# adjacentlink/srsLTE-emane

Hardware: AMD Instinct MI355X
Metric: DL subframes/s (20 MHz, turbo 6-iter) (higher is better)
Workload: dtype f32 (OFDM/chest/eq) + i16 (LLR/turbo)

## Files before the change

include/srslte_hip/phy_hip.h:

```cpp
#ifndef SRSLTE_HIP_PHY_HIP_H
#define SRSLTE_HIP_PHY_HIP_H

#include <stddef.h>
#include <stdint.h>

#ifdef __cplusplus
extern "C" {
#endif

int   srslte_hip_device_count(void);
int   srslte_hip_set_device(int device);
void* srslte_hip_malloc(size_t nbytes);
void  srslte_hip_free(void* d_ptr);
int   srslte_hip_memcpy_h2d(void* d_dst, const void* h_src, size_t nbytes);
int   srslte_hip_memcpy_d2h(void* h_dst, const void* d_src, size_t nbytes);
int   srslte_hip_memset(void* d_dst, int value, size_t nbytes);
int   srslte_hip_sync(void);
void* srslte_hip_stream_create(void);
void  srslte_hip_stream_destroy(void* stream);
int   srslte_hip_stream_sync(void* stream);
void* srslte_hip_event_create(void);
int   srslte_hip_event_record(void* event, void* stream);
float srslte_hip_event_elapsed_ms(void* start, void* stop);
void  srslte_hip_event_destroy(void* event);
// ... 27 lines not shown
  int      filter_type;
  float    filter_coef[2];
  uint16_t mbsfn_area_id;
  uint8_t  interpolate_subframe;
  uint8_t  rsrp_neighbour;
  uint8_t  cfo_estimate_enable;
  uint32_t cfo_estimate_sf_mask;
  uint8_t  sync_error_enable;
} srslte_hip_chest_dl_cfg_t;
typedef struct {
  float noise_estimate, noise_estimate_dbm, snr_db, rsrp, rsrp_dbm, rsrq, rsrq_db, rssi_dbm, cfo, sync_error;
} srslte_hip_chest_dl_res_t;
srslte_hip_chest_dl_t* srslte_hip_chest_dl_create(uint32_t cell_id, uint32_t nof_prb, uint32_t nof_ports, int cp_is_norm);
int srslte_hip_chest_dl_set_tdd(srslte_hip_chest_dl_t* q, int sf_config, int ss_config);
void                   srslte_hip_chest_dl_destroy(srslte_hip_chest_dl_t* q);
int                    srslte_hip_chest_dl_set_symbol_sz(srslte_hip_chest_dl_t* q, int symbol_sz);
const void*            srslte_hip_chest_dl_pilots(const srslte_hip_chest_dl_t* q);
int srslte_hip_chest_dl_estimate_batch(srslte_hip_chest_dl_t* q, const srslte_hip_chest_dl_cfg_t* cfg, uint32_t tti0, const void* d_grid,
                                       void* d_ce, void* d_res, int nof_sf, void* stream);
int srslte_hip_chest_dl_estimate_batch_multi(srslte_hip_chest_dl_t* q, const srslte_hip_chest_dl_cfg_t* cfg, uint32_t tti0, const void* d_grid,
                                             void* d_ce, void* d_res, int nof_sf, int nof_rx, void* stream);
const float* srslte_hip_chest_dl_last_raw(const srslte_hip_chest_dl_t* q);
int         srslte_hip_chest_dl_set_mbsfn_area_id(srslte_hip_chest_dl_t* q, uint16_t mbsfn_area_id);
const void* srslte_hip_chest_dl_mbsfn_pilots(const srslte_hip_chest_dl_t* q, uint16_t mbsfn_area_id);
int srslte_hip_chest_dl_estimate_mbsfn_batch(srslte_hip_chest_dl_t* q, const srslte_hip_chest_dl_cfg_t* cfg, uint32_t tti0, const void* d_grid,
                                             void* d_ce, float* d_noise, int nof_sf, int nof_rx, void* stream);

typedef struct srslte_hip_chest_ul srslte_hip_chest_ul_t;
typedef struct {
  uint32_t cyclic_shift, delta_ss;
  int      group_hopping_en, sequence_hopping_en;
} srslte_hip_dmrs_pusch_cfg_t;
typedef struct {
  float noise_estimate, noise_estimate_dbm, snr, snr_db, cfo;
} srslte_hip_chest_ul_res_t;
srslte_hip_chest_ul_t* srslte_hip_chest_ul_create(uint32_t cell_id, uint32_t nof_prb, int cp_is_norm, const srslte_hip_dmrs_pusch_cfg_t* cfg);
void                   srslte_hip_chest_ul_destroy(srslte_hip_chest_ul_t* q);
int srslte_hip_refsignal_dmrs_pusch_gen(const srslte_hip_chest_ul_t* q, uint32_t L_prb, uint32_t sf_idx, uint32_t n_dmrs, void* r_host);
int srslte_hip_chest_ul_estimate_pusch_batch(srslte_hip_chest_ul_t* q, uint32_t tti0, uint32_t L_prb, uint32_t n_prb, uint32_t n_dmrs,
                                             const void* d_grid, void* d_ce, void* d_res, int nof_sf, void* stream);
int srslte_hip_chest_ul_estimate_pusch_batch_hop(srslte_hip_chest_ul_t* q, uint32_t tti0, uint32_t L_prb, uint32_t n_prb, uint32_t n_prb_slot1,
                                                 uint32_t n_dmrs, const void* d_grid, void* d_ce, void* d_res, int nof_sf, void* stream);

int srslte_hip_demod_soft_demodulate_batch(int mod, const void* d_symbols, float* d_llr, int nsymbols, int ncalls, void* stream);
int srslte_hip_demod_soft_demodulate_s_batch(int mod, const void* d_symbols, short* d_llr, int nsymbols, int ncalls, void* stream);
int srslte_hip_demod_soft_demodulate_b_batch(int mod, const void* d_symbols, int8_t* d_llr, int nsymbols, int ncalls, void* stream);

typedef struct srslte_hip_tdec srslte_hip_tdec_t;
srslte_hip_tdec_t* srslte_hip_tdec_create(uint32_t max_long_cb, uint32_t max_nof_cb);
void               srslte_hip_tdec_destroy(srslte_hip_tdec_t* q);
uint32_t           srslte_hip_tdec_autoimp_get_subblocks(uint32_t long_cb);
uint32_t           srslte_hip_tdec_input_len(uint32_t long_cb, int sb_layout);
int srslte_hip_tdec_run_batch(srslte_hip_tdec_t* q, const int16_t* d_input, uint32_t in_stride, int sb_layout, uint32_t long_cb,
                              uint32_t nof_cb, uint32_t nof_iterations, uint32_t crc_poly, uint32_t crc_nbits, uint8_t* d_output,
                              uint32_t out_stride, uint32_t* d_iters, uint8_t* d_crc_ok, void* stream);

int srslte_hip_tdec_run_batch_manual(srslte_hip_tdec_t* q, const int16_t* d_input, uint32_t in_stride, int sb_layout, uint32_t long_cb,
                                     uint32_t nof_subblocks, uint32_t nof_cb, uint32_t nof_iterations, uint32_t crc_poly, uint32_t crc_nbits,
                                     uint8_t* d_output, uint32_t out_stride, uint32_t* d_iters, uint8_t* d_crc_ok, void* stream);

uint32_t srslte_hip_tdec_autoimp_get_subblocks_8bit(uint32_t long_cb);
int srslte_hip_tdec_run_batch_8bit(srslte_hip_tdec_t* q, const int8_t* d_input, uint32_t in_stride, int sb_layout, uint32_t long_cb,
                                   uint32_t nof_cb, uint32_t nof_iterations, uint32_t crc_poly, uint32_t crc_nbits, uint8_t* d_output,
                                   uint32_t out_stride, uint32_t* d_iters, uint8_t* d_crc_ok, void* stream);

int srslte_hip_tcod_encode_batch(const uint8_t* d_input, uint8_t* d_output, uint32_t long_cb, uint32_t nof_cb, void* stream);
int srslte_hip_tcod_encode_bytes_batch(const uint8_t* d_input, uint32_t in_stride, uint8_t* d_parity, uint32_t par_stride, uint8_t* d_sys_tail,
                                       uint32_t long_cb, uint32_t nof_cb, void* stream);

typedef struct {
  uint32_t F, C, K1, K2, K1_idx, K2_idx, C1, C2, tbs;
} srslte_hip_cbsegm_t;
int srslte_hip_cbsegm(srslte_hip_cbsegm_t* s, uint32_t tbs);
int srslte_hip_cbsegm_cbindex(uint32_t long_cb);
int srslte_hip_cbsegm_cbsize(uint32_t index);
int srslte_hip_tc_interl_LTE_gen_interl(uint16_t* forward, uint16_t* reverse, uint32_t long_cb, uint32_t interl_win);

typedef struct srslte_hip_dl_rx srslte_hip_dl_rx_t;
typedef struct {
  uint32_t cell_id, nof_prb, cfi;
  uint16_t rnti;
  int      mod;
  uint32_t tbs;
  uint32_t max_iterations;
  uint32_t max_batch;
  int      mmse;
  srslte_hip_chest_dl_cfg_t chest_cfg;
  int      llr_8bit;
  uint32_t nof_rx_antennas;
  uint32_t nof_ports;
  int      csi_enable;
  int      power_scale;
  float    p_a;
  int      tx_scheme;
  uint32_t pmi;
  int      mod2;
  uint32_t tbs2;
  int      cp_ext;
  int      tdd;
  uint32_t tdd_sf_config, tdd_ss_config;
  int      mbsfn;
  uint32_t mbsfn_area_id, non_mbsfn_region;
} srslte_hip_dl_rx_cfg_t;
srslte_hip_dl_rx_t* srslte_hip_dl_rx_create(const srslte_hip_dl_rx_cfg_t* cfg);
void                srslte_hip_dl_rx_destroy(srslte_hip_dl_rx_t* q);
int                 srslte_hip_dl_rx_set_iq_format(srslte_hip_dl_rx_t* q, int format, float scale);
uint32_t            srslte_hip_dl_rx_nof_re(const srslte_hip_dl_rx_t* q, uint32_t sf_idx);
int srslte_hip_dl_rx_batch(srslte_hip_dl_rx_t* q, const void* d_iq, uint32_t tti0, uint32_t nof_sf, uint8_t* d_tb, uint32_t tb_stride,
                           uint8_t* d_tb_ok, void* stream);
int srslte_hip_dl_rx_batch_harq(srslte_hip_dl_rx_t* q, const void* d_iq, uint32_t tti0, uint32_t nof_sf, uint32_t rv, int new_data,
                                uint8_t* d_tb, uint32_t tb_stride, uint8_t* d_tb_ok, void* stream);
int srslte_hip_dl_rx_batch_harq2(srslte_hip_dl_rx_t* q, const void* d_iq, uint32_t tti0, uint32_t nof_sf, const uint32_t rv[2], const int new_data[2],
                                 uint8_t* d_tb, uint32_t tb_stride, uint8_t* d_tb_ok, void* stream);
int srslte_hip_dl_rx_grid_batch(srslte_hip_dl_rx_t* q, const void* d_grid, uint32_t tti0, uint32_t nof_sf, uint8_t* d_tb, uint32_t tb_stride,
                                uint8_t* d_tb_ok, void* stream);
typedef struct {
  uint32_t prb_mask[2][4];
  int      mod;
  uint32_t tbs;
  uint32_t rv;
  uint32_t cfi;
  uint16_t rnti;
  int      new_data;
} srslte_hip_dl_grant_t;
int srslte_hip_dl_rx_batch_grants(srslte_hip_dl_rx_t* q, const void* d_iq, uint32_t tti0, uint32_t nof_sf, const srslte_hip_dl_grant_t* grants,
                                  uint8_t* d_tb, uint32_t tb_stride, uint8_t* d_tb_ok, void* stream);
typedef struct {
  srslte_hip_dl_grant_t tb0;
  int      tx_scheme;
  uint32_t pmi;
  int      mod2;
  uint32_t tbs2, rv2;
  int      new_data2;
} srslte_hip_dl_grant2_t;
int srslte_hip_dl_rx_batch_grants2(srslte_hip_dl_rx_t* q, const void* d_iq, uint32_t tti0, uint32_t nof_sf, const srslte_hip_dl_grant2_t* grants,
                                   uint8_t* d_tb, uint32_t tb_stride, uint8_t* d_tb_ok, void* stream);
int srslte_hip_dl_rx_grid_batch_grants2(srslte_hip_dl_rx_t* q, const void* d_grid, uint32_t tti0, uint32_t nof_sf, const srslte_hip_dl_grant2_t* grants,
                                        uint8_t* d_tb, uint32_t tb_stride, uint8_t* d_tb_ok, void* stream);
typedef struct srslte_hip_dl_rx_pool srslte_hip_dl_rx_pool_t;
srslte_hip_dl_rx_pool_t* srslte_hip_dl_rx_pool_create(const srslte_hip_dl_rx_cfg_t* cfg, uint32_t depth);
void                     srslte_hip_dl_rx_pool_destroy(srslte_hip_dl_rx_pool_t* p);
int64_t srslte_hip_dl_rx_pool_submit(srslte_hip_dl_rx_pool_t* p, const void* d_iq, uint32_t tti0, uint32_t nof_sf, const srslte_hip_dl_grant_t* grants,
                                     uint8_t* d_tb, uint32_t tb_stride, uint8_t* d_tb_ok, void* h_record );
int     srslte_hip_dl_rx_pool_wait(srslte_hip_dl_rx_pool_t* p, int64_t ticket);
int     srslte_hip_dl_rx_pool_set_iq_format(srslte_hip_dl_rx_pool_t* p, int format, float scale);
int64_t srslte_hip_dl_rx_pool_submit_host(srslte_hip_dl_rx_pool_t* p, const void* h_iq, uint32_t tti0, uint32_t nof_sf, const srslte_hip_dl_grant_t* grants,
                                          uint8_t* d_tb, uint32_t tb_stride, uint8_t* d_tb_ok, void* h_record );

int srslte_hip_dl_rx_stage(srslte_hip_dl_rx_t* q, int stage, const void* d_iq, uint32_t tti0, uint32_t nof_sf, uint8_t* d_tb,
                           uint32_t tb_stride, uint8_t* d_tb_ok, void* stream);
const void* srslte_hip_dl_rx_debug_buffer(const srslte_hip_dl_rx_t* q, int which);
int         srslte_hip_dl_rx_keep_symbols(srslte_hip_dl_rx_t* q, int enable);
int      srslte_hip_dl_rx_parity_compact(const srslte_hip_dl_rx_t* q);
uint32_t srslte_hip_rm_parity_compact_limit(uint32_t K);

typedef struct srslte_hip_ul_rx srslte_hip_ul_rx_t;
typedef struct {
  uint32_t cell_id, nof_prb;
  uint16_t rnti;
  int      mod;
  uint32_t tbs;
  uint32_t L_prb, n_prb, n_dmrs;
  uint32_t max_iterations, max_batch;
  int      mmse;
  srslte_hip_dmrs_pusch_cfg_t dmrs_cfg;
  int      shortened;
  uint32_t ack_len;
  uint32_t I_offset_ack;
  uint32_t ri_len;
  uint32_t I_offset_ri;
  uint32_t cqi_len, I_offset_cqi;
  uint32_t hopping, n_prb_slot1;
  uint32_t max_grants;
  int      cp_ext;
} srslte_hip_ul_rx_cfg_t;
srslte_hip_ul_rx_t* srslte_hip_ul_rx_create(const srslte_hip_ul_rx_cfg_t* cfg);
void                srslte_hip_ul_rx_destroy(srslte_hip_ul_rx_t* q);
int                 srslte_hip_ul_rx_set_iq_format(srslte_hip_ul_rx_t* q, int format, float scale);
int srslte_hip_ul_rx_batch(srslte_hip_ul_rx_t* q, const void* d_iq, uint32_t tti0, uint32_t nof_sf, uint8_t* d_tb, uint32_t tb_stride,
                           uint8_t* d_tb_ok, void* stream);
int srslte_hip_ul_rx_batch_harq(srslte_hip_ul_rx_t* q, const void* d_iq, uint32_t tti0, uint32_t nof_sf, uint32_t rv, int new_data, uint8_t* d_tb,
                                uint32_t tb_stride, uint8_t* d_tb_ok, void* stream);
typedef struct {
  uint32_t sf;
  uint16_t rnti;
  uint32_t L_prb, n_prb, n_prb_slot1, n_dmrs;
  int      mod;
  uint32_t tbs, rv;
  int      new_data;
  uint32_t ack_len, I_offset_ack;
  uint32_t ri_len, I_offset_ri;
  uint32_t cqi_len, I_offset_cqi;
} srslte_hip_ul_grant_t;
int srslte_hip_ul_rx_batch_grants(srslte_hip_ul_rx_t* q, const void* d_iq, uint32_t tti0, uint32_t nof_sf, const srslte_hip_ul_grant_t* grants,
                                  uint32_t nof_grants, uint8_t* d_tb, uint32_t tb_stride, uint8_t* d_tb_ok, void* stream);
const uint8_t* srslte_hip_ul_rx_grants_ack(const srslte_hip_ul_rx_t* q);
const uint8_t* srslte_hip_ul_rx_grants_ri(const srslte_hip_ul_rx_t* q);
const uint8_t* srslte_hip_ul_rx_grants_cqi(const srslte_hip_ul_rx_t* q);
const uint8_t* srslte_hip_ul_rx_ack(const srslte_hip_ul_rx_t* q);
const uint8_t* srslte_hip_ul_rx_ri(const srslte_hip_ul_rx_t* q);
const uint8_t* srslte_hip_ul_rx_cqi(const srslte_hip_ul_rx_t* q);
const void* srslte_hip_ul_rx_debug_buffer(const srslte_hip_ul_rx_t* q, int which);

typedef struct srslte_hip_ul_tx srslte_hip_ul_tx_t;
typedef struct {
  uint32_t cell_id, nof_prb;
  uint16_t rnti;
  int      mod;
  uint32_t tbs;
  uint32_t L_prb, n_prb, n_dmrs;
  uint32_t max_batch;
  srslte_hip_dmrs_pusch_cfg_t dmrs_cfg;
  int      shortened;
  uint32_t ack_len, I_offset_ack;
  uint32_t ri_len, I_offset_ri;
  uint32_t cqi_len, I_offset_cqi;
  uint32_t hopping, n_prb_slot1;
  uint32_t max_grants;
  int      cp_ext;
} srslte_hip_ul_tx_cfg_t;
srslte_hip_ul_tx_t* srslte_hip_ul_tx_create(const srslte_hip_ul_tx_cfg_t* cfg);
void                srslte_hip_ul_tx_destroy(srslte_hip_ul_tx_t* q);
int                 srslte_hip_ul_tx_set_iq_format(srslte_hip_ul_tx_t* q, int format, float scale);
int srslte_hip_ul_tx_batch(srslte_hip_ul_tx_t* q, const uint8_t* d_tb, uint32_t tb_stride, uint32_t tti0, uint32_t nof_sf, void* d_iq,
                           void* stream);
int srslte_hip_ul_tx_batch_ack(srslte_hip_ul_tx_t* q, const uint8_t* d_tb, uint32_t tb_stride, const uint8_t* d_ack, uint32_t tti0,
                               uint32_t nof_sf, void* d_iq, void* stream);
int srslte_hip_ul_tx_batch_uci(srslte_hip_ul_tx_t* q, const uint8_t* d_tb, uint32_t tb_stride, const uint8_t* d_ack, const uint8_t* d_ri,
                               uint32_t tti0, uint32_t nof_sf, void* d_iq, void* stream);
int srslte_hip_ul_tx_batch_uci_cqi(srslte_hip_ul_tx_t* q, const uint8_t* d_tb, uint32_t tb_stride, const uint8_t* d_ack, const uint8_t* d_ri,
                                   const uint8_t* d_cqi, uint32_t tti0, uint32_t nof_sf, void* d_iq, void* stream);
int srslte_hip_ul_tx_batch_rv(srslte_hip_ul_tx_t* q, const uint8_t* d_tb, uint32_t tb_stride, const uint8_t* d_ack, const uint8_t* d_ri,
                              const uint8_t* d_cqi, uint32_t rv, uint32_t tti0, uint32_t nof_sf, void* d_iq, void* stream);
int srslte_hip_ul_tx_batch_grants(srslte_hip_ul_tx_t* q, const uint8_t* d_tb, uint32_t tb_stride, const uint8_t* d_ack, const uint8_t* d_ri,
                                  const uint8_t* d_cqi, uint32_t tti0, uint32_t nof_sf, const srslte_hip_ul_grant_t* grants, uint32_t nof_grants,
                                  void* d_iq, void* stream);
const void* srslte_hip_ul_tx_debug_buffer(const srslte_hip_ul_tx_t* q, int which);

typedef struct srslte_hip_dl_tx srslte_hip_dl_tx_t;
typedef struct {
  uint32_t cell_id, nof_prb, cfi;
  uint16_t rnti;
  int      mod;
  uint32_t tbs;
  uint32_t max_batch;
  uint32_t nof_ports;
  float    p_a;
  uint32_t max_grants;
  int      cp_ext;
  int      tdd;
  uint32_t tdd_sf_config, tdd_ss_config;
  int      mbsfn;
  uint32_t mbsfn_area_id, non_mbsfn_region;
} srslte_hip_dl_tx_cfg_t;
srslte_hip_dl_tx_t* srslte_hip_dl_tx_create(const srslte_hip_dl_tx_cfg_t* cfg);
void                srslte_hip_dl_tx_destroy(srslte_hip_dl_tx_t* q);
int                 srslte_hip_dl_tx_set_iq_format(srslte_hip_dl_tx_t* q, int format, float scale);
int srslte_hip_dl_tx_batch(srslte_hip_dl_tx_t* q, const uint8_t* d_tb, uint32_t tb_stride, uint32_t tti0, uint32_t nof_sf, uint32_t rv, void* d_iq,
                           void* stream);
typedef struct {
  uint32_t              sf;
  srslte_hip_dl_grant_t grant;
} srslte_hip_dl_tx_grant_t;
int srslte_hip_dl_tx_batch_grants(srslte_hip_dl_tx_t* q, const uint8_t* d_tb, uint32_t tb_stride, uint32_t tti0, uint32_t nof_sf,
                                  const srslte_hip_dl_tx_grant_t* grants, uint32_t nof_grants, void* d_iq, void* stream);
typedef struct {
  uint32_t               sf;
  srslte_hip_dl_grant2_t grant;
} srslte_hip_dl_tx_grant2_t;
int srslte_hip_dl_tx_batch_grants2(srslte_hip_dl_tx_t* q, const uint8_t* d_tb, uint32_t tb_stride, uint32_t tti0, uint32_t nof_sf,
                                   const srslte_hip_dl_tx_grant2_t* grants, uint32_t nof_grants, void* d_iq, void* stream);
const void* srslte_hip_dl_tx_debug_buffer(const srslte_hip_dl_tx_t* q, int which);

typedef struct srslte_hip_sch srslte_hip_sch_t;
srslte_hip_sch_t* srslte_hip_sch_create(uint32_t max_tbs, uint32_t max_e_bits, int llr_8bit);
void              srslte_hip_sch_destroy(srslte_hip_sch_t* q);
int srslte_hip_sch_decode(srslte_hip_sch_t* q, const void* e_bits, uint32_t nof_e_bits, uint32_t tbs, int mod, uint32_t Nl, uint32_t rv,
                          uint32_t max_iterations, int16_t** buffer_f, uint8_t* cb_crc, uint8_t* cb_bytes, uint32_t* sum_passes);
typedef struct {
  int      mod;
  uint32_t tbs, rv, nof_bits, L_prb, nof_symb, max_iterations;
  uint32_t ack_len, ri_len, cqi_len;
  uint32_t I_offset_ack, I_offset_ri, I_offset_cqi;
  uint32_t cqi_len_rank2, cqi_rank2;
} srslte_hip_ulsch_cfg_t;
typedef struct {
  uint8_t  ack[2], ri;
  uint8_t  cqi_bits[64], cqi_crc;
  uint32_t cqi_len;
  uint32_t Q_prime_ack, Q_prime_ri, Q_prime_cqi;
  uint32_t stream_waits;
} srslte_hip_ulsch_res_t;
int srslte_hip_ulsch_decode(srslte_hip_sch_t* q, const int16_t* q_bits, const uint8_t* c_seq, const srslte_hip_ulsch_cfg_t* cfg, int16_t** buffer_f,
                            uint8_t* cb_crc, uint8_t* cb_bytes, uint32_t* sum_passes, srslte_hip_ulsch_res_t* res);
int srslte_hip_ulsch_debug_g(srslte_hip_sch_t* q, int16_t* out, uint32_t n);
typedef struct {
  srslte_hip_ulsch_cfg_t sch;
  uint32_t nof_prb, cell_id, cp_ext;
  uint32_t rnti, sf_idx;
  uint32_t n_prb_tilde[2];
  uint32_t shortened;
  uint32_t nof_re;
} srslte_hip_pusch_cfg_t;
int srslte_hip_pusch_decode(srslte_hip_sch_t* q, const void* sf_symbols, const void* ce, float noise_estimate, const srslte_hip_pusch_cfg_t* cfg,
                            int16_t** buffer_f, uint8_t* cb_crc, uint8_t* cb_bytes, uint32_t* sum_passes, srslte_hip_ulsch_res_t* res);
int srslte_hip_pusch_rows(const srslte_hip_pusch_cfg_t* cfg, uint32_t* rows);
// ... 615 lines not shown
```

srslte-emane_amd/csrc/pdsch_kernels.inc:

```
#include <vector>

namespace {

struct ChestResDev {
  float noise_estimate, noise_estimate_dbm, snr_db, rsrp, rsrp_dbm, rsrq, rsrq_db, rssi_dbm, cfo, sync_error;
};

struct SfClass {
  const uint32_t* idx;
  int             nof_re;
};

struct SfDesc {
  const uint32_t* idx;
  const uint32_t* scr;
  int             nof_re, mod, Qm;
  int             C, K, tbs, rlen;
  const uint32_t* crc_fac;
  int             scheme, codebook, nof_tb;
};
struct CbDesc {
  int             sf, cb;
  int             C, K, Qm, nof_re;
  int             combine;
  int             w_len;
  const uint32_t* tbl;
  int             Nl;
  int             e_off;
};
struct GrantDev {
  uint32_t mask[2][4];
  int      sf_idx, lstart, q_off, rnti;
  int      cw;
  int      tdd;
  int      nss[2];
};

struct PdschGeom {
  const SfDesc* desc;
  SfClass cls[3];
  int     grid_len;
  int      ce_len, ce_nre;
  uint32_t ce_magic;
  int     max_re, max_bits, mod, Qm, mmse, scr_words, tti0, nof_rx, nof_ports;
  float     inv_scaling;
  float*    csi;
  uint32_t* csi_max;
  int             tx_scheme, codebook_idx, nof_tb, mod1, Qm1, max_bits1, scr_words1;
  const uint32_t* scr1;
  float*          csi1;
  uint32_t*       csi_max1;
  int             cw1_off;
};

__device__ __forceinline__ void csi_note_max(uint32_t* dst, float v)
{
  for (int o = 32; o > 0; o >>= 1) v = fmaxf(v, __shfl_xor(v, o, 64));
  if ((threadIdx.x & 63) == 0) atomicMax(dst, __float_as_uint(v));
}

__device__ __forceinline__ int sf_class(int sf_idx) { return sf_idx == 0 ? 0 : (sf_idx == 5 ? 1 : 2); }

template <typename LLR>
__global__ __launch_bounds__(256) void pdsch_demod_kernel(const cf32* __restrict__ grid, const cf32* __restrict__ ce,
                                                          const ChestResDev* __restrict__ res, const uint32_t* __restrict__ scr,
                                                          cf32* __restrict__ d_out, LLR* __restrict__ e_out, PdschGeom g)
{
  __shared__ __attribute__((aligned(16))) LLR stage[256 * 8];
  const int       sf = blockIdx.y, sf_idx = (g.tti0 + sf) % 10;
  SfClass         c  = g.cls[sf_class(sf_idx)];
  int             mod = g.mod, Qm = g.Qm;
  const uint32_t* cs = scr + (size_t)sf_idx * g.scr_words;
  if (g.desc) {
    const SfDesc d = g.desc[sf];
    if (d.scheme >= 2) return;
    c.idx = d.idx; c.nof_re = d.nof_re; mod = d.mod; Qm = d.Qm; cs = d.scr;
  }
  const int     base = blockIdx.x * blockDim.x, i = base + threadIdx.x;
  if (base >= c.nof_re) return;
  const bool     live = i < c.nof_re;
  const uint32_t k  = c.idx[live ? i : c.nof_re - 1];
  const float    n0 = g.mmse ? res[sf].noise_estimate : 0.f;
  cf32           x;
  float          gain;
  const uint32_t kh = g.ce_nre ? k - __umulhi(k, g.ce_magic) * (uint32_t)g.ce_nre : k;
  if (g.nof_rx == 1) {
    const cf32 y = grid[(size_t)sf * g.grid_len + k], h = ce[(size_t)sf * g.ce_len + kh];
    const float re = y.x * h.x + y.y * h.y, im = y.y * h.x - y.x * h.y, csi = h.x * h.x + h.y * h.y + n0;
    x = make_float2(re * g.inv_scaling / csi, im * g.inv_scaling / csi);
    gain = csi;
  } else {
    float re = 0.f, im = 0.f, hh = 0.f;
    for (int a = 0; a < g.nof_rx; a++) {
      const size_t o = ((size_t)sf * g.nof_rx + a) * g.grid_len + k;
      const cf32   y = grid[o], h = ce[((size_t)sf * g.nof_rx + a) * g.ce_len + kh];
      const float  pr = y.x * h.x + y.y * h.y, pi = y.y * h.x - y.x * h.y, ph = h.x * h.x + h.y * h.y;
      re = a ? re + pr : pr;
      im = a ? im + pi : pi;
      hh = a ? hh + ph : ph;
    }
    if (n0 > 0.f) hh += n0;
    x = make_float2(re / hh * g.inv_scaling, im / hh * g.inv_scaling);
    gain = hh;
  }
  if (g.csi) {
    if (live) g.csi[(size_t)sf * g.max_re + i] = gain;
    csi_note_max(g.csi_max + sf, live ? gain : 0.f);
  }
  if (d_out && live) d_out[(size_t)sf * g.max_re + i] = x;
  LLR o[8];
  if constexpr (sizeof(LLR) == 1) {
    demod_dev::demod_b(mod, x, i, c.nof_re, o);
  } else {
    demod_dev::demod_s(mod, x, i, c.nof_re, o);
  }
  const int       bit0 = (live ? i : 0) * Qm;
  const uint32_t  c2   = (uint32_t)((((uint64_t)cs[(bit0 >> 5) + 1] << 32) | cs[bit0 >> 5]) >> (bit0 & 31));
  for (int j = 0; j < Qm; j++) {
    LLR v = o[j];
    if ((c2 >> j) & 1) v = (LLR)-v;
    stage[threadIdx.x * Qm + j] = v;
  }
  __syncthreads();
  const int   nbytes = min(256, c.nof_re - base) * Qm * (int)sizeof(LLR);
  char*       dst    = reinterpret_cast<char*>(e_out + (size_t)sf * g.max_bits + (size_t)base * Qm);
  const char* src    = reinterpret_cast<const char*>(stage);
  for (int o16 = threadIdx.x * 16; o16 + 16 <= nbytes; o16 += 256 * 16) *reinterpret_cast<uint4*>(dst + o16) = *reinterpret_cast<const uint4*>(src + o16);
  const int rem = nbytes & 15;
  if ((int)threadIdx.x < rem) dst[nbytes - rem + threadIdx.x] = src[nbytes - rem + threadIdx.x];
}

template <typename LLR>
__global__ __launch_bounds__(256) void pdsch_demod_div_kernel(const cf32* __restrict__ grid, const cf32* __restrict__ ce,
                                                              const uint32_t* __restrict__ scr, cf32* __restrict__ d_out, LLR* __restrict__ e_out,
                                                              PdschGeom g)
{
  __shared__ __attribute__((aligned(16))) LLR stage[512 * 8];
  const int       sf = blockIdx.y, sf_idx = (g.tti0 + sf) % 10;
  SfClass         c  = g.cls[sf_class(sf_idx)];
  const uint32_t* cs = scr + (size_t)sf_idx * g.scr_words;
  int             mod = g.mod, Qm = g.Qm;
  if (g.desc) {
    const SfDesc d = g.desc[sf];
    if (d.scheme >= 2) return;
    c.idx = d.idx; c.nof_re = d.nof_re; mod = d.mod; Qm = d.Qm; cs = d.scr;
  }
  const int     base = blockIdx.x * 512, i0 = base + 2 * threadIdx.x;
  if (base >= c.nof_re) return;
  const bool     live = i0 < c.nof_re;
  const uint32_t k0 = c.idx[live ? i0 : c.nof_re - 2], k1 = c.idx[live ? i0 + 1 : c.nof_re - 1];
  float          hh = 0.f, x0r = 0.f, x0i = 0.f, x1r = 0.f, x1i = 0.f;
  for (int a = 0; a < g.nof_rx; a++) {
    const cf32* y  = grid + ((size_t)sf * g.nof_rx + a) * g.grid_len;
    const cf32* h0 = ce + (((size_t)sf * 2 + 0) * g.nof_rx + a) * g.grid_len;
    const cf32* h1 = ce + (((size_t)sf * 2 + 1) * g.nof_rx + a) * g.grid_len;
    const cf32  r0 = y[k0], r1 = y[k1], h00 = h0[k0], h01 = h0[k1], h10 = h1[k0], h11 = h1[k1];
    hh += h00.x * h00.x + h00.y * h00.y + h11.x * h11.x + h11.y * h11.y;
    if (hh == 0.f) hh = 1e-4f;
    x0r += h00.x * r0.x + h00.y * r0.y + h11.x * r1.x + h11.y * r1.y;
    x0i += h00.x * r0.y - h00.y * r0.x + h11.y * r1.x - h11.x * r1.y;
    x1r += -(h10.x * r0.x + h10.y * r0.y) + h01.x * r1.x + h01.y * r1.y;
    x1i += -(h10.y * r0.x - h10.x * r0.y) + h01.x * r1.y - h01.y * r1.x;
  }
  if (g.csi) {
    if (live) *reinterpret_cast<float2*>(g.csi + (size_t)sf * g.max_re + i0) = make_float2(hh, hh);
    csi_note_max(g.csi_max + sf, live ? hh : 0.f);
  }
  hh *= 1.0f / g.inv_scaling;
  const cf32 x[2] = {make_float2((float)((double)(x0r / hh) * 1.4142135623730951), (float)((double)(x0i / hh) * 1.4142135623730951)),
                     make_float2((float)((double)(x1r / hh) * 1.4142135623730951), (float)((double)(x1i / hh) * 1.4142135623730951))};
#pragma unroll
  for (int t = 0; t < 2; t++) {
    const int i = (live ? i0 : 0) + t;
    if (d_out && live) d_out[(size_t)sf * g.max_re + i] = x[t];
    LLR o[8];
    if constexpr (sizeof(LLR) == 1) {
      demod_dev::demod_b(mod, x[t], i, c.nof_re, o);
    } else {
      demod_dev::demod_s(mod, x[t], i, c.nof_re, o);
    }
    const int      bit0 = i * Qm;
    const uint32_t c2   = (uint32_t)((((uint64_t)cs[(bit0 >> 5) + 1] << 32) | cs[bit0 >> 5]) >> (bit0 & 31));
    for (int j = 0; j < Qm; j++) stage[(2 * threadIdx.x + t) * Qm + j] = ((c2 >> j) & 1) ? (LLR)-o[j] : o[j];
  }
  __syncthreads();
  const int   nbytes = min(512, c.nof_re - base) * Qm * (int)sizeof(LLR);
  char*       dst    = reinterpret_cast<char*>(e_out + (size_t)sf * g.max_bits + (size_t)base * Qm);
  const char* src    = reinterpret_cast<const char*>(stage);
  for (int o16 = threadIdx.x * 16; o16 + 16 <= nbytes; o16 += 256 * 16) *reinterpret_cast<uint4*>(dst + o16) = *reinterpret_cast<const uint4*>(src + o16);
  const int rem = nbytes & 15;
  if ((int)threadIdx.x < rem) dst[nbytes - rem + threadIdx.x] = src[nbytes - rem + threadIdx.x];
}

template <typename LLR>
__global__ __launch_bounds__(256) void pdsch_demod_div4_kernel(const cf32* __restrict__ grid, const cf32* __restrict__ ce,
                                                               const uint32_t* __restrict__ scr, cf32* __restrict__ d_out, LLR* __restrict__ e_out,
                                                               PdschGeom g)
{
  __shared__ __attribute__((aligned(16))) LLR stage[1024 * 8];
  const int       sf = blockIdx.y, sf_idx = (g.tti0 + sf) % 10;
  SfClass         c  = g.cls[sf_class(sf_idx)];
  const uint32_t* cs = scr + (size_t)sf_idx * g.scr_words;
  int             mod = g.mod, Qm = g.Qm;
  if (g.desc) {
    const SfDesc d = g.desc[sf];
    if (d.scheme >= 2) return;
    c.idx = d.idx; c.nof_re = d.nof_re; mod = d.mod; Qm = d.Qm; cs = d.scr;
  }
  const int     base = blockIdx.x * 1024, i0 = base + 4 * threadIdx.x;
  if (base >= c.nof_re) return;
  const bool live = i0 < c.nof_re;
  uint32_t   k[4];
#pragma unroll
  for (int t = 0; t < 4; t++) k[t] = c.idx[live ? i0 + t : c.nof_re - 4 + t];
  float a[4] = {0.f, 0.f, 0.f, 0.f}, xr[4] = {0.f, 0.f, 0.f, 0.f}, xi[4] = {0.f, 0.f, 0.f, 0.f};
  for (int an = 0; an < g.nof_rx; an++) {
    const cf32* y = grid + ((size_t)sf * g.nof_rx + an) * g.grid_len;
#pragma unroll
    for (int half = 0; half < 2; half++) {
      const cf32* hA = ce + (((size_t)sf * 4 + half) * g.nof_rx + an) * g.grid_len;
      const cf32* hB = ce + (((size_t)sf * 4 + 2 + half) * g.nof_rx + an) * g.grid_len;
      const uint32_t k0 = k[2 * half], k1 = k[2 * half + 1];
      const cf32     h00 = hA[k0], h01 = hB[k0], h10 = hA[k1], h11 = hB[k1], r0 = y[k0], r1 = y[k1];
      a[2 * half] += h00.x * h00.x + h00.y * h00.y + h11.x * h11.x + h11.y * h11.y;
      a[2 * half + 1] += h10.x * h10.x + h10.y * h10.y + h01.x * h01.x + h01.y * h01.y;
      xr[2 * half] += h00.x * r0.x + h00.y * r0.y + h11.x * r1.x + h11.y * r1.y;
      xi[2 * half] += h00.x * r0.y - h00.y * r0.x + h11.y * r1.x - h11.x * r1.y;
      xr[2 * half + 1] += -(h01.x * r0.x + h01.y * r0.y) + h10.x * r1.x + h10.y * r1.y;
      xi[2 * half + 1] += -(h01.y * r0.x - h01.x * r0.y) + h10.x * r1.y - h10.y * r1.x;
    }
  }
  float           gmax = 0.f;
#pragma unroll
  for (int t = 0; t < 4; t++) {
    const int   i  = (live ? i0 : 0) + t;
    const float at = a[t] * (1.0f / g.inv_scaling);
    const cf32  x  = make_float2(xr[t] / at * 1.41421356f, xi[t] / at * 1.41421356f);
    if (g.csi && live) g.csi[(size_t)sf * g.max_re + i] = at / g.nof_rx;
    gmax = fmaxf(gmax, live ? at / g.nof_rx : 0.f);
    if (d_out && live) d_out[(size_t)sf * g.max_re + i] = x;
    LLR o[8];
    if constexpr (sizeof(LLR) == 1) {
      demod_dev::demod_b(mod, x, i, c.nof_re, o);
    } else {
      demod_dev::demod_s(mod, x, i, c.nof_re, o);
    }
    const int      bit0 = i * Qm;
    const uint32_t c2   = (uint32_t)((((uint64_t)cs[(bit0 >> 5) + 1] << 32) | cs[bit0 >> 5]) >> (bit0 & 31));
    for (int j = 0; j < Qm; j++) stage[(4 * threadIdx.x + t) * Qm + j] = ((c2 >> j) & 1) ? (LLR)-o[j] : o[j];
  }
  if (g.csi) csi_note_max(g.csi_max + sf, gmax);
  __syncthreads();
  const int   nbytes = min(1024, c.nof_re - base) * Qm * (int)sizeof(LLR);
  char*       dst    = reinterpret_cast<char*>(e_out + (size_t)sf * g.max_bits + (size_t)base * Qm);
  const char* src    = reinterpret_cast<const char*>(stage);
  for (int o16 = threadIdx.x * 16; o16 + 16 <= nbytes; o16 += 256 * 16) *reinterpret_cast<uint4*>(dst + o16) = *reinterpret_cast<const uint4*>(src + o16);
  const int rem = nbytes & 15;
  if ((int)threadIdx.x < rem) dst[nbytes - rem + threadIdx.x] = src[nbytes - rem + threadIdx.x];
}

__device__ __forceinline__ cf32 cmulc(cf32 a, cf32 b) { return make_float2(a.x * b.x + a.y * b.y, a.y * b.x - a.x * b.y); }

template <typename LLR>
__global__ __launch_bounds__(256) void pdsch_demod_mimo_kernel(const cf32* __restrict__ grid, const cf32* __restrict__ ce,
                                                               const ChestResDev* __restrict__ res, const uint32_t* __restrict__ scr,
                                                               cf32* __restrict__ d_out0, cf32* __restrict__ d_out1, LLR* __restrict__ e_out0,
                                                               LLR* __restrict__ e_out1, PdschGeom g)
{
  __shared__ __attribute__((aligned(16))) LLR stage[2][256 * 8];
  const int       sf = blockIdx.y, sf_idx = (g.tti0 + sf) % 10;
  SfClass         c  = g.cls[sf_class(sf_idx)];
  int             tx_scheme = g.tx_scheme, codebook_idx = g.codebook_idx, nof_tb = g.nof_tb, mods[2] = {g.mod, g.mod1}, Qms[2] = {g.Qm, g.Qm1};
  const uint32_t* css[2] = {scr + (size_t)sf_idx * g.scr_words, g.scr1 ? g.scr1 + (size_t)sf_idx * g.scr_words1 : nullptr};
  if (g.desc) {
    const SfDesc d0 = g.desc[sf];
    if (d0.scheme < 2) return;
    const SfDesc d1 = g.desc[g.cw1_off + sf];
    c.idx = d0.idx; c.nof_re = d0.nof_re; tx_scheme = d0.scheme; codebook_idx = d0.codebook; nof_tb = d0.nof_tb;
    mods[0] = d0.mod; Qms[0] = d0.Qm; css[0] = d0.scr;
    mods[1] = d1.mod; Qms[1] = d1.Qm; css[1] = d1.scr;
  }
  const int     base = blockIdx.x * blockDim.x, i = base + threadIdx.x;
  if (base >= c.nof_re) return;
  const bool     live = i < c.nof_re;
// ... 53 lines not shown
    x[1]   = cadd(cmul(y0, w10), cmul(y1, w11));
    csi[0] = 1.0f / b00.x;
    csi[1] = 1.0f / b11.x;
  }
#pragma unroll
  for (int cw = 0; cw < 2; cw++) {
    if (cw >= nof_tb) break;
    const int       mod = mods[cw], Qm = Qms[cw];
    float*          csi_o = cw ? g.csi1 : g.csi;
    cf32*           d_out = cw ? d_out1 : d_out0;
    if (csi_o) {
      if (live) csi_o[(size_t)sf * g.max_re + i] = csi[cw];
      csi_note_max((cw ? g.csi_max1 : g.csi_max) + sf, live ? csi[cw] : 0.f);
    }
    if (d_out && live) d_out[(size_t)sf * g.max_re + i] = x[cw];
    LLR o[8];
    if constexpr (sizeof(LLR) == 1) {
      demod_dev::demod_b(mod, x[cw], i, c.nof_re, o);
    } else {
      demod_dev::demod_s(mod, x[cw], i, c.nof_re, o);
    }
    const uint32_t* cs   = css[cw];
    const int       bit0 = (live ? i : 0) * Qm;
    const uint32_t  c2   = (uint32_t)((((uint64_t)cs[(bit0 >> 5) + 1] << 32) | cs[bit0 >> 5]) >> (bit0 & 31));
    for (int j = 0; j < Qm; j++) stage[cw][threadIdx.x * Qm + j] = ((c2 >> j) & 1) ? (LLR)-o[j] : o[j];
  }
  __syncthreads();
#pragma unroll
  for (int cw = 0; cw < 2; cw++) {
    if (cw >= nof_tb) break;
    const int   Qm = Qms[cw], nbytes = min(256, c.nof_re - base) * Qm * (int)sizeof(LLR);
    char*       dst = reinterpret_cast<char*>((cw ? e_out1 : e_out0) + (size_t)sf * (cw ? g.max_bits1 : g.max_bits) + (size_t)base * Qm);
    const char* src = reinterpret_cast<const char*>(stage[cw]);
    for (int o16 = threadIdx.x * 16; o16 + 16 <= nbytes; o16 += 256 * 16) *reinterpret_cast<uint4*>(dst + o16) = *reinterpret_cast<const uint4*>(src + o16);
    const int rem = nbytes & 15;
    if ((int)threadIdx.x < rem) dst[nbytes - rem + threadIdx.x] = src[nbytes - rem + threadIdx.x];
  }
}

struct RmGeom {
  const CbDesc* cbd;
  uint8_t*      cb_ok_rst;
  int C, K, Qm, tti0, max_bits, w_stride, out_len;
  int nof_re[3];
  int             max_re, mod;
  int             Nl;
  const float*    csi;
  const uint32_t* csi_max;
  int             combine;
  const uint8_t*  skip;
  int             e_off;
  int             w_len;
};

template <typename LLR>
__device__ __forceinline__ uint32_t add_wrap(uint32_t a, uint32_t b)
{
  if constexpr (sizeof(LLR) == 2) {
    return (((a & 0xffffu) + (b & 0xffffu)) & 0xffffu) | (((a >> 16) + (b >> 16)) << 16);
  } else {
    const uint32_t lo = ((a & 0x00ff00ffu) + (b & 0x00ff00ffu)) & 0x00ff00ffu, hi = ((a & 0xff00ff00u) >> 8) + ((b & 0xff00ff00u) >> 8);
    return lo | ((hi & 0x00ff00ffu) << 8);
  }
}

struct CsiW {
  const float* csi;
  float        scale, inv;
  int          Qm, mod, body_bits, nsym;
};
__device__ __forceinline__ CsiW csi_setup(const RmGeom& g, int sf, int nsym, int Qm)
{
  CsiW c;
  c.csi = g.csi + (size_t)sf * g.max_re;
  const float mx = nsym > 0 ? __uint_as_float(g.csi_max[sf]) : 1.0f;
  c.scale = 32767.0f / mx;
  c.inv   = 1.0f / mx;
  c.Qm = Qm; c.mod = Qm / 2; c.nsym = nsym;
  const int G = c.mod == 3 ? 12 : (c.mod == 4 ? 8 : 4);
  c.body_bits = (nsym * Qm / G) * G;
  return c;
}
template <typename LLR>
__device__ __forceinline__ LLR csi_apply(const CsiW& c, LLR v, int b)
{
  if constexpr (sizeof(LLR) == 1) {
    const int s = min(b / c.Qm, c.nsym - 1);
    return (LLR)demod_dev::trunc_i((float)v * (c.csi[s] * c.inv));
  } else {
    if (b >= c.body_bits) {
      const int s = min(b / c.Qm, c.nsym - 1);
      return (LLR)demod_dev::trunc_i((float)v * (c.csi[s] * c.inv));
    }
    int s;
    if (c.mod == 1) {
      s = 2 * (b >> 2) + (((b & 3) < 2) ? 1 : 0);
    } else if (c.mod == 3) {
      const int r = b % 12;
      s = 2 * (b / 12) + ((r < 4 || r == 6 || r == 7) ? 0 : 1);
    } else {
      s = b / c.Qm;
    }
    const int w = demod_dev::sat16(demod_dev::rne(c.csi[s] * c.scale));
    return (LLR)(((int)v * w) >> 16);
  }
}


template <typename LLR>
__global__ __launch_bounds__(256) void rm_rx_kernel(const LLR* __restrict__ e, LLR* __restrict__ w, const uint32_t* __restrict__ inv, RmGeom g)
{
  constexpr int PER = 4 / (int)sizeof(LLR);
  int             cbg = blockIdx.y, sf = cbg / g.C, cb = cbg - sf * g.C, C = g.C, Qm = g.Qm, out_len = g.out_len, w_len = g.w_len ? g.w_len : g.w_stride, combine = g.combine;
  int             nre = g.nof_re[sf_class((g.tti0 + sf) % 10)], Nl = g.Nl, e_off = g.e_off;
  const uint32_t* tbl = inv;
  if (g.cbd) {
    const CbDesc d = g.cbd[blockIdx.y];
    sf = d.sf; cb = d.cb; cbg = sf * g.C + cb; C = d.C; Qm = d.Qm; out_len = 3 * d.K + 12; w_len = d.w_len; combine = d.combine; nre = d.nof_re; tbl = d.tbl;
    Nl = d.Nl; e_off = d.e_off;
  }
  const int j = PER * (blockIdx.x * blockDim.x + threadIdx.x);
  if (j >= w_len || (g.skip && combine && g.skip[cbg])) return;
  if (g.cb_ok_rst && !combine && j == 0) g.cb_ok_rst[cbg] = 0;
  const int QmL = Qm * Nl, Gp = nre / Nl;
  const int gamma = Gp % C, n_e = QmL * (Gp / C);
  int       rp = cb * n_e, n_e2 = n_e;
  if (cb > C - gamma) {
    n_e2 = n_e + QmL;
    rp   = (C - gamma) * n_e + (cb - (C - gamma)) * n_e2;
  }
  const LLR* src = e + (size_t)sf * g.max_bits + e_off + rp;
  CsiW       cw;
  if (g.csi) cw = csi_setup(g, sf, nre, Qm);
  uint32_t   n[PER], word = 0;
  if constexpr (PER == 2) {
    const uint2 t = *reinterpret_cast<const uint2*>(tbl + j);
    n[0] = t.x; n[1] = t.y;
  } else {
    const uint4 t = *reinterpret_cast<const uint4*>(tbl + j);
    n[0] = t.x; n[1] = t.y; n[2] = t.z; n[3] = t.w;
  }
#pragma unroll
  for (int s = 0; s < PER; s++) {
    int acc = 0;
    if (n[s] != 0xffffffffu) {
      for (int i = (int)n[s]; i < n_e2; i += out_len) acc += g.csi ? csi_apply<LLR>(cw, src[i], rp + i) : src[i];
    }
    word |= ((uint32_t)acc & ((1u << (8 * sizeof(LLR))) - 1u)) << (8 * sizeof(LLR) * s);
  }
  uint32_t* dst = reinterpret_cast<uint32_t*>(w + (size_t)cbg * g.w_stride + j);
  *dst          = combine ? add_wrap<LLR>(*dst, word) : word;
}

template <typename LLR>
__global__ __launch_bounds__(256) void rm_rx_lds_kernel(const LLR* __restrict__ e, LLR* __restrict__ w, const uint32_t* __restrict__ inv, RmGeom g)
{
  extern __shared__ __attribute__((aligned(16))) char seg_raw[];
  constexpr int PER = 16 / (int)sizeof(LLR), NV = PER / 8;
  LLR*          seg = reinterpret_cast<LLR*>(seg_raw);
  int             cbg = blockIdx.x, sf = cbg / g.C, cb = cbg - sf * g.C, C = g.C, Qm = g.Qm, out_len = g.out_len, w_len = g.w_len ? g.w_len : g.w_stride, combine = g.combine;
  int             nre = g.nof_re[sf_class((g.tti0 + sf) % 10)], Nl = g.Nl, e_off = g.e_off;
  const uint32_t* tbl = inv;
  if (g.cbd) {
    const CbDesc d = g.cbd[blockIdx.x];
    sf = d.sf; cb = d.cb; cbg = sf * g.C + cb; C = d.C; Qm = d.Qm; out_len = 3 * d.K + 12; w_len = d.w_len; combine = d.combine; nre = d.nof_re; tbl = d.tbl;
    Nl = d.Nl; e_off = d.e_off;
  }
  if (g.skip && combine && g.skip[cbg]) return;
  if (g.cb_ok_rst && !combine && threadIdx.x == 0) g.cb_ok_rst[cbg] = 0;
  const int QmL = Qm * Nl, Gp = nre / Nl;
  const int gamma = Gp % C, n_e = QmL * (Gp / C);
  int       rp = cb * n_e, n_e2 = n_e;
  if (cb > C - gamma) {
    n_e2 = n_e + QmL;
    rp   = (C - gamma) * n_e + (cb - (C - gamma)) * n_e2;
  }
  const LLR* src = e + (size_t)sf * g.max_bits + e_off + rp;
  const int mis = (int)((reinterpret_cast<uintptr_t>(src) & 15) / sizeof(LLR));
  const int4* s4 = reinterpret_cast<const int4*>(src - mis);
  const int   n16 = (n_e2 + mis + PER - 1) / PER;
  if (g.csi) {
    const CsiW cw = csi_setup(g, sf, nre, Qm);
    for (int i = threadIdx.x; i < n16; i += 256) {
      union {
        int4 v;
        LLR  h[PER];
      } u;
      u.v = s4[i];
#pragma unroll
      for (int j = 0; j < PER; j++) u.h[j] = csi_apply<LLR>(cw, u.h[j], rp - mis + PER * i + j);
      reinterpret_cast<int4*>(seg)[i] = u.v;
    }
  } else {
#pragma unroll 4
    for (int i = threadIdx.x; i < n16; i += 256) reinterpret_cast<int4*>(seg)[i] = s4[i];
  }
  __syncthreads();
  const LLR*   ls    = seg + mis;
  const uint4* inv16 = reinterpret_cast<const uint4*>(reinterpret_cast<const uint16_t*>(tbl + w_len));
  uint4*       dst   = reinterpret_cast<uint4*>(w + (size_t)cbg * g.w_stride);
  const int    ngroups = w_len / PER;
  for (int j0 = threadIdx.x; j0 < ngroups; j0 += 4 * 256) {
    uint4 tt[4][NV];
#pragma unroll
    for (int u = 0; u < 4; u++) {
      const int j = j0 + 256 * u;
#pragma unroll
      for (int v = 0; v < NV; v++) tt[u][v] = j < ngroups ? inv16[j * NV + v] : make_uint4(~0u, ~0u, ~0u, ~0u);
    }
#pragma unroll
    for (int u = 0; u < 4; u++) {
      const int j = j0 + 256 * u;
      if (j >= ngroups) break;
      uint32_t o[4] = {0, 0, 0, 0};
#pragma unroll
      for (int s = 0; s < PER; s++) {
        const uint32_t pair = (&tt[u][s / 8].x)[(s / 2) & 3], n = (s & 1) ? pair >> 16 : pair & 0xffffu;
        int            acc  = 0;
        if (n != 0xffffu) {
          for (int i = (int)n; i < n_e2; i += out_len) acc += ls[i];
        }
        constexpr int BITS = 8 * (int)sizeof(LLR);
        o[s * BITS / 32] |= ((uint32_t)acc & ((1u << BITS) - 1u)) << ((s * BITS) & 31);
      }
      if (combine) {
        const uint4 old = dst[j];
        dst[j] = make_uint4(add_wrap<LLR>(old.x, o[0]), add_wrap<LLR>(old.y, o[1]), add_wrap<LLR>(old.z, o[2]), add_wrap<LLR>(old.w, o[3]));
      } else {
        dst[j] = make_uint4(o[0], o[1], o[2], o[3]);
      }
    }
  }
}

__device__ __forceinline__ uint32_t gf24_mul(uint32_t a, uint32_t b, uint32_t poly)
{
  uint32_t r = 0;
  for (int i = 23; i >= 0; i--) {
    r <<= 1;
    if (r & 0x1000000u) r ^= poly;
    if ((b >> i) & 1) r ^= a;
  }
  return r;
}

template <typename Byte>
__device__ uint32_t block_crc24(Byte byte_at, int nbytes, uint32_t poly, uint32_t* tab, uint32_t* red)
{
  const int t = threadIdx.x;
  {
    uint32_t v = (uint32_t)t << 16;
    for (int i = 0; i < 8; i++) {
      v <<= 1;
      if (v & 0x1000000u) v ^= poly;
    }
    tab[t] = v;
  }
  __syncthreads();
  const int cB = (nbytes + 255) / 256, pad = 256 * cB - nbytes;
  uint32_t  crc = 0;
  for (int i = 0; i < cB; i++) {
    const int v = t * cB + i - pad;
    if (v >= 0) crc = ((crc << 8) & 0xffffffu) ^ tab[((crc >> 16) & 0xff) ^ byte_at(v)];
  }
  uint32_t m = 1;
  for (int i = 0; i < 8 * cB; i++) {
    m <<= 1;
    if (m & 0x1000000u) m ^= poly;
  }
  red[t] = crc;
  __syncthreads();
  for (int s = 1; s < 256; s <<= 1) {
    uint32_t v = 0;
    if ((t & (2 * s - 1)) == 0) v = gf24_mul(red[t], m, poly) ^ red[t + s];
    __syncthreads();
    if ((t & (2 * s - 1)) == 0) red[t] = v;
    m = gf24_mul(m, m, poly);
    __syncthreads();
  }
  return red[0];
}

struct TbGeom {
  const SfDesc* desc;
  int C, K, tbs, rlen, cb_stride, tb_stride;
  int nof_sf, cw1_off;
  const uint32_t* iters;
};
__device__ __forceinline__ bool tb_any_block_decoded(const uint32_t* iters, int first, int C)
{
  if (!iters) return true;
  bool any = false;
  for (int c = 0; c < C; c++) any = any || iters[first + c] != 0;
  return any;
}

__global__ __launch_bounds__(512) void tb_crc_kernel(const uint8_t* __restrict__ cb_bytes, const uint8_t* __restrict__ cb_ok,
                                                     const uint32_t* __restrict__ crc_rem, uint8_t* __restrict__ tb, uint8_t* __restrict__ tb_ok,
                                                     TbGeom g)
{
  __shared__ uint32_t red[8];
  const int C = g.C, K = g.K, tbs = g.tbs, rlen = g.rlen;
  const int sf = blockIdx.x, nbytes = tbs / 8 + 3, rb = rlen / 8;
  uint8_t*  dst = tb + (size_t)sf * g.tb_stride;
  uint32_t  syn = 0;
  for (int b0 = threadIdx.x * 4; b0 < nbytes + 3; b0 += blockDim.x * 4) {
    uint32_t word = 0;
#pragma unroll
    for (int t = 0; t < 4; t++) {
      const int b = b0 + t;
      int       cb = b / rb;
      if (cb > C - 1) cb = C - 1;
      const int     off = b - cb * rb;
      const uint8_t v   = (b < nbytes + 3 && off < K / 8) ? cb_bytes[((size_t)sf * g.C + cb) * g.cb_stride + off] : 0;
      if (b < nbytes + 3) dst[b] = v;
      word |= (uint32_t)(b < nbytes ? v : 0) << (8 * t);
    }
#pragma unroll
    for (int j = 0; j < 32; j++) {
      const int      t = j >> 3, bit = 8 * (b0 + t) + 7 - (j & 7);
      const uint32_t m = 0u - ((word >> j) & 1u);
      syn ^= (bit < 8 * nbytes ? crc_rem[bit] : 0u) & m;
    }
  }
  for (int o = 32; o > 0; o >>= 1) syn ^= __shfl_xor(syn, o, 64);
  if ((threadIdx.x & 63) == 0) red[threadIdx.x >> 6] = syn;
  __syncthreads();
  if (threadIdx.x == 0) {
    syn = 0;
    for (int i = 0; i < (int)blockDim.x / 64; i++) syn ^= red[i];
    bool ok = syn == 0;
    for (int c = 0; c < C; c++) ok = ok && cb_ok[sf * g.C + c];
    const uint8_t* p = dst + tbs / 8;
    ok               = ok && (p[0] | p[1] | p[2]) && tb_any_block_decoded(g.iters, sf * g.C, C);
    tb_ok[sf]        = ok ? 1 : 0;
  }
}

constexpr int TB_MAX_BITS = 105528;
__global__ __launch_bounds__(256) void tb_crc_bytes_kernel(const uint8_t* __restrict__ cb_bytes, const uint8_t* __restrict__ cb_ok, uint8_t* __restrict__ tb,
                                                           uint8_t* __restrict__ tb_ok, TbGeom g)
{
  __shared__ uint32_t tab[256], red[4];
  __shared__ uint8_t  bytes[TB_MAX_BITS / 8 + 8];
  const int    row = blockIdx.x, sf = row < g.nof_sf ? row : g.cw1_off + row - g.nof_sf;
  const SfDesc d   = g.desc[sf];
  const int    C = d.C, K = d.K, nbytes = d.tbs / 8 + 3, rb = d.rlen / 8, t = threadIdx.x;
  uint8_t*     dst = tb + (size_t)row * g.tb_stride;
  if (C == 0) {
    if (t == 0) tb_ok[row] = 0;
    return;
  }
  {
    uint32_t v = (uint32_t)t << 16;
    for (int i = 0; i < 8; i++) {
      v <<= 1;
      if (v & 0x1000000u) v ^= 0x1864CFBu;
    }
    tab[t] = v;
  }
  for (int cb = 0; cb < C; cb++) {
    const uint8_t* src = cb_bytes + ((size_t)sf * g.C + cb) * g.cb_stride;
    const int      n   = cb == C - 1 ? nbytes + 3 - cb * rb : rb;
    for (int i = t; i < n; i += 256) {
      const uint8_t v = i < K / 8 ? src[i] : 0;
      dst[cb * rb + i] = v;
      if (cb * rb + i < nbytes) bytes[cb * rb + i] = v;
    }
  }
  __syncthreads();
  const int cB = (nbytes + 255) / 256, pad = 256 * cB - nbytes;
  uint32_t  crc = 0;
// ... 46 lines not shown
  pdsch_relist_body(gr, idx_out, P, cell_id, max_re, nof_ports, nsl, (int)blockIdx.x);
}
__device__ __forceinline__ void pdsch_relist_body(const GrantDev* __restrict__ gr, uint32_t* __restrict__ idx_out, int P, int cell_id, int max_re,
                                                  int nof_ports, int nsl, int sf)
{
  __shared__ int cnt[14 * 21 + 1];
  const int      nre = 12 * P, cps = (nre + 63) / 64, nsym = 2 * nsl, nchunks = nsym * cps;
  const int      wave = threadIdx.x >> 6, lane = threadIdx.x & 63, nwaves = RELIST_THREADS / 64;
  const GrantDev g  = gr[sf];
  auto           used = [&](int sym, int kc) {
    const int k = kc * 64 + lane, s = sym >= nsl ? 1 : 0, l = sym - nsl * s, p = k / 12;
    if (k >= nre || !((g.mask[s][p >> 5] >> (p & 31)) & 1u)) return false;
    if (g.nss[0] && l >= g.nss[s]) return false;
    return pdsch_re_used(P, cell_id, g.sf_idx, g.q_off, s, l, k, nof_ports, nsl, g.tdd, g.nss[1]);
  };
  __shared__ unsigned long long msk[14 * 21];
  for (int sym = 0; sym < nsym; sym++) {
    const bool on = sym >= nsl || sym >= g.lstart;
    for (int kc = wave; kc < cps; kc += nwaves) {
      const unsigned long long b = on ? __ballot(used(sym, kc)) : 0ull;
      if (lane == 0) {
        cnt[sym * cps + kc] = __popcll(b);
        msk[sym * cps + kc] = b;
      }
    }
  }
  __syncthreads();
  if (wave == 0) {
    constexpr int PL = (14 * 21 + 63) / 64;
    int           v[PL], sum = 0;
#pragma unroll
    for (int j = 0; j < PL; j++) {
      const int c = lane * PL + j;
      v[j]        = c < nchunks ? cnt[c] : 0;
      sum += v[j];
    }
    int incl = sum;
    for (int o = 1; o < 64; o <<= 1) {
      const int t = __shfl_up(incl, o, 64);
      if (lane >= o) incl += t;
    }
    int acc = incl - sum;
#pragma unroll
    for (int j = 0; j < PL; j++) {
      const int c = lane * PL + j;
      if (c < nchunks) cnt[c] = acc;
      acc += v[j];
    }
  }
  __syncthreads();
  uint32_t* o = idx_out + (size_t)sf * max_re;
  for (int sym = (g.lstart < nsl ? g.lstart : nsl); sym < nsym; sym++) {
    for (int kc = wave; kc < cps; kc += nwaves) {
      const unsigned long long b = msk[sym * cps + kc];
      if ((b >> lane) & 1ull) o[cnt[sym * cps + kc] + __popcll(b & ((1ull << lane) - 1ull))] = (uint32_t)(sym * nre + kc * 64 + lane);
    }
  }
}
__device__ __forceinline__ void scr_gen_body(const GrantDev* __restrict__ gr, const uint32_t* __restrict__ basis, uint32_t* __restrict__ out, int words,
                                             int cell_id, int sf, int w)
{
  if (w >= words) return;
  const GrantDev g = gr[sf];
  uint32_t       c_init = ((uint32_t)g.rnti << 14) + ((uint32_t)g.cw << 13) + ((uint32_t)g.sf_idx << 9) + (uint32_t)cell_id, v = basis[w];
  for (int j = 0; j < 31; j++) {
    if ((c_init >> j) & 1u) v ^= basis[(size_t)(1 + j) * words + w];
  }
  out[(size_t)sf * words + w] = v;
}
__global__ __launch_bounds__(256) void scr_gen_kernel(const GrantDev* __restrict__ gr, const uint32_t* __restrict__ basis, uint32_t* __restrict__ out,
                                                      int words, int cell_id)
{
  scr_gen_body(gr, basis, out, words, cell_id, (int)blockIdx.y, (int)(blockIdx.x * 256 + threadIdx.x));
}
__global__ __launch_bounds__(256) void desc_copy_kernel(const uint4* __restrict__ src, uint4* __restrict__ dst, int n16)
{
  const int i = (int)(blockIdx.x * 256 + threadIdx.x);
  if (i < n16) dst[i] = src[i];
}

__global__ __launch_bounds__(RELIST_THREADS) void grants_prep_kernel(const GrantDev* __restrict__ gr, uint32_t* __restrict__ idx_out, int P, int cell_id,
                                                                     int max_re, int nof_ports, int nsl, int nof_sf, const uint32_t* __restrict__ basis,
                                                                     uint32_t* __restrict__ scr0, const GrantDev* __restrict__ gr1,
                                                                     uint32_t* __restrict__ scr1, int words, uint8_t* __restrict__ tb_ok, int nrows,
                                                                     const uint4* __restrict__ desc_src, uint4* __restrict__ desc_dst, int desc_n16,
                                                                     int copy_first)
{
  if ((int)blockIdx.x >= copy_first) {
    const int i = ((int)blockIdx.x - copy_first) * RELIST_THREADS + (int)threadIdx.x;
    if (i < desc_n16) desc_dst[i] = desc_src[i];
    return;
  }
  if ((int)blockIdx.x < nof_sf) {
    if (threadIdx.x == 0) {
      tb_ok[blockIdx.x] = 0;
      if ((int)blockIdx.x + nof_sf < nrows) tb_ok[blockIdx.x + nof_sf] = 0;
    }
    pdsch_relist_body(gr, idx_out, P, cell_id, max_re, nof_ports, nsl, (int)blockIdx.x);
    return;
  }
  const int per = (words + RELIST_THREADS - 1) / RELIST_THREADS;
  int       b = (int)blockIdx.x - nof_sf;
  const int cw = b / (nof_sf * per);
  b -= cw * nof_sf * per;
  const int sf = b / per, w = (b - sf * per) * RELIST_THREADS + (int)threadIdx.x;
  scr_gen_body(cw ? gr1 : gr, basis, cw ? scr1 : scr0, words, cell_id, sf, w);
}

__global__ __launch_bounds__(256) void tb_asm_kernel(const uint8_t* __restrict__ cb_bytes, const uint8_t* __restrict__ cb_ok,
                                                     const uint32_t* __restrict__ cb_syn, uint8_t* __restrict__ tb, uint8_t* __restrict__ tb_ok,
                                                     TbGeom g)
{
  __shared__ __attribute__((aligned(8))) uint8_t cbb[32 * 768];
  const int      sf = blockIdx.x, nbytes = g.tbs / 8 + 3, rb = g.rlen / 8, tot = g.C * g.cb_stride;
  const uint8_t* src0 = cb_bytes + (size_t)sf * tot;
  uint8_t*       dst = tb + (size_t)sf * g.tb_stride;
  if ((reinterpret_cast<uintptr_t>(src0) & 7) == 0) {
    for (int i = threadIdx.x; i < tot / 8; i += blockDim.x) reinterpret_cast<uint64_t*>(cbb)[i] = reinterpret_cast<const uint64_t*>(src0)[i];
    for (int i = tot / 8 * 8 + threadIdx.x; i < tot; i += blockDim.x) cbb[i] = src0[i];
  } else {
    for (int i = threadIdx.x; i < tot; i += blockDim.x) cbb[i] = src0[i];
  }
  __syncthreads();
  auto src = [&](int b) -> uint32_t {
    int cb = b / rb;
    if (cb > g.C - 1) cb = g.C - 1;
    const int off = b - cb * rb;
    return off < g.K / 8 ? cbb[cb * g.cb_stride + off] : 0u;
  };
  const bool a4 = ((reinterpret_cast<uintptr_t>(dst) | (uintptr_t)g.tb_stride) & 3) == 0;
  const int  n  = nbytes + 3, n4 = a4 ? n / 4 : 0;
  for (int w = threadIdx.x; w < n4; w += blockDim.x)
    reinterpret_cast<uint32_t*>(dst)[w] = src(4 * w) | (src(4 * w + 1) << 8) | (src(4 * w + 2) << 16) | (src(4 * w + 3) << 24);
  for (int b = 4 * n4 + threadIdx.x; b < n; b += blockDim.x) dst[b] = (uint8_t)src(b);
  if (threadIdx.x == 0) {
    uint32_t syn = 0;
    bool     ok  = true;
    for (int c = 0; c < g.C; c++) {
      syn ^= cb_syn[sf * g.C + c];
      ok = ok && cb_ok[sf * g.C + c];
    }
    ok        = ok && syn == 0 && (src(g.tbs / 8) | src(g.tbs / 8 + 1) | src(g.tbs / 8 + 2)) && tb_any_block_decoded(g.iters, sf * g.C, g.C);
    tb_ok[sf] = ok ? 1 : 0;
  }
}

int rm_lds_bytes(const RmGeom& g, int llr_bytes)
{
  int mx = g.nof_re[0] > g.nof_re[1] ? g.nof_re[0] : g.nof_re[1];
  mx     = mx > g.nof_re[2] ? mx : g.nof_re[2];
  return ((g.Qm * (mx / g.C) + 2 * g.Qm) * llr_bytes + 32 + 15) & ~15;
}

template <typename T>
int rm_rx_launch(int lds, uint32_t nblk, const void* e, void* w, const uint32_t* tbl, const RmGeom& g, hipStream_t st)
{
  if (lds <= 64 * 1024) {
    hipLaunchKernelGGL(rm_rx_lds_kernel<T>, dim3(nblk), dim3(256), lds, st, (const T*)e, (T*)w, tbl, g);
  } else {
    hipLaunchKernelGGL(rm_rx_kernel<T>, dim3(ceil_div(g.w_stride, 1024 / (int)sizeof(T)), nblk), dim3(256), 0, st, (const T*)e, (T*)w, tbl, g);
  }
  LAUNCH_CHECK();
  return SRSLTE_SUCCESS;
}

std::vector<uint32_t> rm_slot_table(const std::vector<uint32_t>& t, uint32_t w_stride)
{
  std::vector<uint32_t> inv(w_stride + w_stride / 2, 0xffffffffu);
  uint16_t*             inv16 = reinterpret_cast<uint16_t*>(inv.data() + w_stride);
  for (uint32_t n = 0; n < t.size(); n++) {
    if (t[n] == 0xffffffffu) continue;
    inv[t[n]]   = n;
    inv16[t[n]] = (uint16_t)n;
  }
  return inv;
}

void pmch_re_indices(uint32_t nof_prb, uint32_t lstart, std::vector<uint32_t>& idx)
{
  idx.clear();
  for (uint32_t s = 0; s < 2; s++) {
    for (uint32_t l = (s == 0 ? lstart : 0); l < 6; l++) {
      const bool     has_ref = (l == 2 && s == 0) || (l == 0 && s == 1) || (l == 4 && s == 1);
      const uint32_t keep    = (l == 0 && s == 1) ? 0 : 1;
      for (uint32_t k = 0; k < 12 * nof_prb; k++) {
        if (!has_ref || (k & 1) == keep) idx.push_back((6 * s + l) * 12 * nof_prb + k);
      }
    }
  }
}

void pdsch_re_indices(uint32_t cell_id, uint32_t nof_prb, uint32_t nof_ports, uint32_t sf_idx, uint32_t lstart, std::vector<uint32_t>& idx,
                      uint32_t nsl = 7)
{
  const uint32_t nre = 12 * nof_prb, step = nof_ports == 1 ? 6 : 3;
  idx.clear();
  for (uint32_t s = 0; s < 2; s++) {
    for (uint32_t l = (s == 0 ? lstart : 0); l < nsl; l++) {
      const bool     has_ref = l == 0 || l == nsl - 3 || (l == 1 && nof_ports == 4);
      const uint32_t offset  = l == 0 ? cell_id % 6 : (cell_id + 3) % 6;
      const bool     sync    = (s == 0 && (sf_idx == 0 || sf_idx == 5) && l >= nsl - 2) || (s == 1 && sf_idx == 0 && l < 4);
      for (uint32_t k = 0; k < nre; k++) {
        if (sync && k + 36 >= nre / 2 && k < nre / 2 + 36) continue;
        if (has_ref && (k % step) == offset % step) continue;
        idx.push_back((s * nsl + l) * nre + k);
      }
    }
  }
}

template <typename T>
int upload(DevBuf<T>& d, const std::vector<T>& h)
{
  if (h.empty() ? d.alloc(1) : d.upload(h)) {
    hip_log("[srslte_hip] upload of a %zu-byte table to the device failed\n", sizeof(T) * h.size());
    return SRSLTE_ERROR;
  }
  return SRSLTE_SUCCESS;
}

int rm_rx_table_upload(uint32_t K, uint32_t rv, uint32_t W, uint32_t w_stride, DevBuf<uint32_t>& d_tbl)
{
  std::vector<uint32_t> t;
  lte_rm_rx_table(K, rv, t);
  if (W) {
    for (auto& v : t) v = v < 3 * K ? (v % 3) * (K + 32) + ((v / 3) % (K / W)) * W + (v / 3) / (K / W) : (v - 3 * K) + 3 * (K + 32);
  }
  return upload(d_tbl, rm_slot_table(t, w_stride));
}

struct RmParityCompact {
  uint32_t phase[2], len, e_lim;
};
bool rm_parity_compact(uint32_t K, RmParityCompact& c, std::vector<uint32_t>* t_out = nullptr)
{
  if (K % 64 || K / 16 < 4) return false;
  std::vector<uint32_t> t;
  lte_rm_rx_table(K, 0, t);
  const uint32_t Lw = K / 16;
  bool           seen[2] = {false, false};
  c.phase[0] = c.phase[1] = 0;
  c.len   = (K + 32 + K / 2 + 12 + 31) & ~31u;
  c.e_lim = (uint32_t)t.size();
  for (uint32_t n = 0; n < t.size(); n++) {
    const uint32_t v = t[n], s = v % 3, i = v / 3;
    if (v >= 3 * K) {
      t[n] = (v - 3 * K) + K + 32 + K / 2;
    } else if (s == 0) {
      t[n] = (i % Lw) * 16 + i / Lw;
    } else {
      const uint32_t r = i % Lw;
      if (!seen[s - 1]) {
        seen[s - 1]    = true;
        c.phase[s - 1] = r % 4;
      }
      if (r % 4 == c.phase[s - 1]) {
        t[n] = K + 32 + (s - 1) * (K / 4) + (r / 4) * 16 + i / Lw;
      } else {
        if (c.e_lim == t.size()) c.e_lim = n;
        t[n] = 0xffffffffu;
      }
    }
  }
  if (t_out) t_out->swap(t);
  return true;
}
int rm_rx_table_upload_compact(uint32_t K, RmParityCompact& c, DevBuf<uint32_t>& d_tbl)
{
  std::vector<uint32_t> t;
  if (!rm_parity_compact(K, c, &t)) return SRSLTE_ERROR_INVALID_INPUTS;
  return upload(d_tbl, rm_slot_table(t, c.len));
}

__global__ __launch_bounds__(256) void rm_parity_expand_kernel(int16_t* __restrict__ w, int w_stride, int K, int phase0, int phase1)
{
  __shared__ __attribute__((aligned(16))) int16_t cp[6144 / 2 + 16];
  int16_t*  p  = w + (size_t)blockIdx.x * w_stride;
  const int nc = K / 2 + 12, base = K + 32;
  for (int i = threadIdx.x; i < (nc + 7) / 8; i += 256) reinterpret_cast<uint4*>(cp)[i] = reinterpret_cast<const uint4*>(p + base)[i];
  __syncthreads();
  const int per = (K + 32) / 8;
  for (int j = threadIdx.x; j < 2 * per; j += 256) {
    const int s = j >= per, h = j - s * per, r = h >> 1;
    uint4     v = make_uint4(0, 0, 0, 0);
    if (r < K / 16 && (r & 3) == (s ? phase1 : phase0)) v = *reinterpret_cast<const uint4*>(cp + s * (K / 4) + (r >> 2) * 16 + (h & 1) * 8);
    *reinterpret_cast<uint4*>(p + (1 + s) * (K + 32) + h * 8) = v;
  }
  for (int i = 3 * (K + 32) + threadIdx.x; i < w_stride; i += 256) p[i] = i < 3 * (K + 32) + 12 ? cp[K / 2 + i - 3 * (K + 32)] : (int16_t)0;
}

int rm_tx_table_upload(uint32_t K, uint32_t rv, DevBuf<uint32_t>& d_tbl)
{
  std::vector<uint32_t> t;
  lte_rm_rx_table(K, rv, t);
  for (auto& v : t) {
    const uint32_t p = v / 3, s = v % 3;
    v = s == 0 ? (p < K ? p : (1u << 30) | (p - K)) : (2u << 30) | (s == 1 ? p : K + 4 + p);
  }
  return upload(d_tbl, t);
}

void constellation_levels(int mod, float* lvl)
{
  for (uint32_t idx = 0; idx < (1u << mod); idx++) {
    double v = 1.0;
    for (int i = mod - 1; i >= 1; i--) v = (double)(1 << (mod - i)) - (1 - 2 * (int)((idx >> (mod - 1 - i)) & 1)) * v;
    const double norm = mod == 1 ? sqrt(2.0) : (mod == 2 ? sqrt(10.0) : (mod == 3 ? sqrt(42.0) : sqrt(170.0)));
    lvl[idx]          = (float)((1 - 2 * (int)((idx >> (mod - 1)) & 1)) * v / norm);
  }
}
// ... 27 lines not shown
```

srslte-emane_amd/csrc/pdsch_rx.inc:

```
struct GrantsState {
  srslte_hip_tdec_t* tdec = nullptr;
  uint32_t           Cmax = 0, stride = 0, max_re = 0, max_bits = 0, words = 0;
  uint32_t           V = 0;
  DevBuf<uint32_t>   d_relist, d_scr, d_basis, d_cb_iters;
  DevBuf<int16_t>    d_e, d_w;
  DevBuf<uint8_t>    d_cb_bytes, d_cb_ok;
  DevBuf<float>      d_csi;
  DevBuf<uint32_t>   d_csi_max;
  size_t             desc_bytes = 0;
  DescStage          desc;
  bool               tb_direct = false;
  std::map<std::pair<uint32_t, uint32_t>, DevBuf<uint32_t>> rm_tbl;
  std::map<uint32_t, DevBuf<uint32_t>>                      crc_fac;
  ~GrantsState() { srslte_hip_tdec_destroy(tdec); }
};

struct srslte_hip_dl_rx {
  srslte_hip_dl_rx_cfg_t cfg   = {};
  srslte_hip_ofdm_t*     ofdm  = nullptr;
  srslte_hip_chest_dl_t* chest = nullptr;
  PdschGeom              pg    = {};
  DevBuf<uint32_t>       d_idx[3];
  struct Codeword {
    DevBuf<uint32_t> d_scr;
    DevBuf<int16_t>  d_e;
    DevBuf<cf32>     d_d;
    DevBuf<float>    d_csi;
    DevBuf<uint32_t> d_csi_max;
    SchRxFixed       sch;
  } cw[2];
  int                    ncw = 1;
  DevBuf<cf32>           d_grid, d_ce;
  DevBuf<cf32>           d_ce_full;
  DevBuf<ChestResDev>    d_res;
  std::unique_ptr<GrantsState> gs;
  srslte_hip_csi_t*      csi = nullptr;
  uint32_t               est_nof_sf = 0;
  float                  csi_offset = 0.f;
  ~srslte_hip_dl_rx()
  {
    srslte_hip_ofdm_destroy(ofdm);
    srslte_hip_chest_dl_destroy(chest);
    srslte_hip_csi_destroy(csi);
  }
};

struct DlRxCall {
  const cf32* grid = nullptr;
  SchHarq     harq[2];
};

extern "C" void srslte_hip_dl_rx_destroy(srslte_hip_dl_rx_t* q) { delete q; }

extern "C" int srslte_hip_dl_rx_set_iq_format(srslte_hip_dl_rx_t* q, int format, float scale)
{
  return q ? srslte_hip_ofdm_set_sample_format(q->ofdm, format, scale) : SRSLTE_ERROR_INVALID_INPUTS;
}

extern "C" srslte_hip_dl_rx_t* srslte_hip_dl_rx_create(const srslte_hip_dl_rx_cfg_t* cfg)
{
  if (!cfg || cfg->max_batch == 0 || cfg->mod < 1 || cfg->mod > 4 || cfg->max_iterations == 0 || cfg->nof_rx_antennas > 4 || cfg->nof_ports > 4 ||
      cfg->nof_ports == 3) {
    hip_log("[srslte_hip] dl_rx: invalid configuration\n");
    return nullptr;
  }
  const bool mimo = cfg->tx_scheme != 0, two = mimo && cfg->tbs2 != 0;
  if (mimo) {
    const bool ok = (cfg->tx_scheme == 2 || cfg->tx_scheme == 3) && cfg->nof_ports == 2 && cfg->nof_rx_antennas == 2 &&
                    (cfg->tx_scheme == 2 || two) && (two ? cfg->pmi < 2 : cfg->pmi < 4) && (!two || (cfg->mod2 >= 1 && cfg->mod2 <= 4));
    if (!ok) {
      hip_log("[srslte_hip] dl_rx: two-layer modes need a 2-port cell and 2 receive antennas; CDD with two transport blocks, "
              "multiplexing with two (pmi 0-1) or one (pmi 0-3)\n");
      return nullptr;
    }
  }
  std::unique_ptr<srslte_hip_dl_rx> q(new srslte_hip_dl_rx());
  q->cfg = *cfg;
  q->ncw = two ? 2 : 1;
  srslte_hip_cbsegm_t seg;
  if (fixed_grant_segmentation("dl_rx", cfg->tbs, &seg) || (two && fixed_grant_segmentation("dl_rx", cfg->tbs2, &seg))) return nullptr;
  const uint32_t P = cfg->nof_prb, nre = 12 * P, B = cfg->max_batch;
  const uint32_t lstart = cfg->cfi + (P < 10 ? 1 : 0);
  const uint32_t nrx    = cfg->nof_rx_antennas ? cfg->nof_rx_antennas : 1;
  const uint32_t npt    = cfg->nof_ports ? cfg->nof_ports : 1;
  const uint32_t nsl    = (cfg->cp_ext || cfg->mbsfn) ? 6 : 7;
  if (cfg->mbsfn && (npt != 1 || mimo || cfg->tdd || cfg->llr_8bit || cfg->csi_enable || cfg->power_scale || cfg->mbsfn_area_id > 255 ||
                     cfg->non_mbsfn_region < 1 || cfg->non_mbsfn_region > 2)) {
    hip_log("[srslte_hip] dl_rx: an MBSFN pipeline is single-port FDD with 16-bit LLRs, area id 0-255, a non-MBSFN region of 1 or 2 symbols\n");
    return nullptr;
  }
  if (cfg->mbsfn) q->cfg.chest_cfg.interpolate_subframe = 1;
  if (cfg->tdd && (cfg->tdd_sf_config > 6 || cfg->tdd_ss_config > 9)) {
    hip_log("[srslte_hip] dl_rx: TDD uplink-downlink configuration %u / special-subframe configuration %u\n", cfg->tdd_sf_config, cfg->tdd_ss_config);
    return nullptr;
  }
  q->ofdm  = srslte_hip_ofdm_create((int)P, nsl == 6 ? 0 : 1, 1);
  q->chest = srslte_hip_chest_dl_create(cfg->cell_id, P, npt, cfg->cp_ext ? 0 : 1);
  if (q->chest && cfg->tdd) srslte_hip_chest_dl_set_tdd(q->chest, (int)cfg->tdd_sf_config, (int)cfg->tdd_ss_config);
  if (cfg->mbsfn && q->ofdm && q->chest &&
      (srslte_hip_ofdm_set_mbsfn(q->ofdm, 1, (int)cfg->non_mbsfn_region) || srslte_hip_chest_dl_set_mbsfn_area_id(q->chest, (uint16_t)cfg->mbsfn_area_id))) {
    srslte_hip_chest_dl_destroy(q->chest);
    q->chest = nullptr;
  }
  bool ok = q->ofdm && q->chest;
  SchRxFixed::Cfg sc = {};
  const uint32_t  rep_sf[3] = {0, 5, 1};
  for (int c = 0; c < 3 && ok; c++) {
    std::vector<uint32_t> idx;
    if (cfg->mbsfn) pmch_re_indices(P, lstart, idx);
    else pdsch_re_indices(cfg->cell_id, P, npt, rep_sf[c], lstart, idx, nsl);
    q->pg.cls[c].nof_re = (int)idx.size();
    sc.nof_re[c]        = (uint32_t)idx.size();
    sc.max_re           = idx.size() > sc.max_re ? (uint32_t)idx.size() : sc.max_re;
    ok                  = upload(q->d_idx[c], idx) == SRSLTE_SUCCESS;
    q->pg.cls[c].idx    = q->d_idx[c];
  }
  const uint32_t max_re = sc.max_re;
  const size_t   glen   = (size_t)2 * nsl * nre;
  ok = ok && !q->d_grid.alloc(glen * B * nrx) && !q->d_ce.alloc(glen * B * nrx * npt) &&
       hipMemset(q->d_ce, 0, sizeof(cf32) * glen * B * nrx * npt) == hipSuccess &&
       !q->d_res.alloc(B);
  sc.max_batch = B; sc.max_iterations = cfg->max_iterations; sc.llr_8bit = cfg->llr_8bit != 0;
  sc.Nl = (npt > 1 && !mimo) ? 2 : 1;
  uint32_t scr_words[2] = {0, 0};
  for (int c = 0; c < q->ncw && ok; c++) {
    srslte_hip_dl_rx::Codeword& w = q->cw[c];
    sc.mod = c ? cfg->mod2 : cfg->mod; sc.tbs = c ? cfg->tbs2 : cfg->tbs; sc.Qm = 2 * (uint32_t)sc.mod;
    sc.max_bits  = (max_re * sc.Qm + 15) & ~15u;
    scr_words[c] = (max_re * sc.Qm + 31) / 32 + 1;
    std::vector<uint32_t> scr;
    const uint32_t        c_init0 = cfg->mbsfn ? cfg->mbsfn_area_id : ((uint32_t)cfg->rnti << 14) + ((uint32_t)c << 13) + cfg->cell_id;
    lte_scr_table([&](uint32_t sf) { return c_init0 + (sf << 9); }, max_re * sc.Qm, scr_words[c], scr);
    ok = upload(w.d_scr, scr) == SRSLTE_SUCCESS && !w.d_e.alloc((size_t)sc.max_bits * B + 16);
    if (ok && cfg->csi_enable) ok = !w.d_csi.alloc((size_t)max_re * B) && !w.d_csi_max.alloc(B);
    sc.csi = w.d_csi; sc.csi_max = w.d_csi_max;
    sc.may_compact = c == 0; sc.may_direct = !two && !mimo;
    ok = ok && w.sch.init(sc) == SRSLTE_SUCCESS;
  }
  if (!ok) {
    hip_log("[srslte_hip] dl_rx: initialisation failed\n");
    return nullptr;
  }
  const SchRxFixed& s0 = q->cw[0].sch;
  q->pg.grid_len = (int)glen; q->pg.max_re = (int)max_re; q->pg.max_bits = s0.rg.max_bits; q->pg.mod = cfg->mod; q->pg.Qm = s0.rg.Qm;
  q->pg.mmse = cfg->mmse; q->pg.scr_words = (int)scr_words[0]; q->pg.nof_rx = (int)nrx; q->pg.nof_ports = (int)npt;
  q->pg.csi = q->cw[0].d_csi; q->pg.csi_max = q->cw[0].d_csi_max;
  const bool compact = npt == 1 && !q->cfg.chest_cfg.interpolate_subframe;
  q->pg.ce_len = compact ? (int)(12 * P) : (int)glen; q->pg.ce_nre = compact ? (int)(12 * P) : 0;
  q->pg.ce_magic = compact ? (uint32_t)((0x100000000ull + 12 * P - 1) / (12 * P)) : 0;
  q->pg.inv_scaling = cfg->power_scale ? 1.0f / (powf(10.0f, cfg->p_a / 20.0f) * (npt == 1 ? 1.0f : sqrtf(2.0f))) : 1.0f;
  if (mimo) {
    q->pg.tx_scheme = cfg->tx_scheme; q->pg.nof_tb = two ? 2 : 1;
    q->pg.codebook_idx = (int)(two ? cfg->pmi + 1 : cfg->pmi);
    if (two) {
      const SchRxFixed& s1 = q->cw[1].sch;
      q->pg.mod1 = cfg->mod2; q->pg.Qm1 = s1.rg.Qm; q->pg.max_bits1 = s1.rg.max_bits; q->pg.scr_words1 = (int)scr_words[1];
      q->pg.scr1 = q->cw[1].d_scr; q->pg.csi1 = q->cw[1].d_csi; q->pg.csi_max1 = q->cw[1].d_csi_max;
    }
  }
  return q.release();
}

extern "C" int srslte_hip_dl_rx_keep_symbols(srslte_hip_dl_rx_t* q, int enable)
{
  if (!q) return SRSLTE_ERROR_INVALID_INPUTS;
  for (int c = q->ncw - 1; c >= 0; c--) {
    DevBuf<cf32>& d_d = q->cw[c].d_d;
    if (enable && !d_d && d_d.alloc((size_t)q->pg.max_re * q->cfg.max_batch)) {
      hip_log("[srslte_hip] dl_rx: no device memory for the equalised symbols\n");
      return SRSLTE_ERROR;
    }
    if (!enable) d_d = DevBuf<cf32>();
  }
  return SRSLTE_SUCCESS;
}

extern "C" uint32_t srslte_hip_dl_rx_nof_re(const srslte_hip_dl_rx_t* q, uint32_t sf_idx)
{
  return q ? (uint32_t)q->pg.cls[sf_idx % 10 == 0 ? 0 : (sf_idx % 10 == 5 ? 1 : 2)].nof_re : 0;
}

__global__ void ce_expand_kernel(const cf32* __restrict__ row, cf32* __restrict__ full, int nre, int nsym)
{
  const int plane = blockIdx.y;
  for (int k = blockIdx.x * blockDim.x + threadIdx.x; k < nre; k += gridDim.x * blockDim.x) {
    const cf32 v = row[(size_t)plane * nre + k];
    for (int l = 0; l < nsym; l++) full[((size_t)plane * nsym + l) * nre + k] = v;
  }
}
static const void* dl_rx_ce_full(srslte_hip_dl_rx_t* q)
{
  const size_t planes = (size_t)q->cfg.max_batch * q->pg.nof_rx;
  if (hipDeviceSynchronize() != hipSuccess) return nullptr;
  if (!q->d_ce_full && q->d_ce_full.alloc(planes * q->pg.grid_len)) return nullptr;
  hipLaunchKernelGGL(ce_expand_kernel, dim3(ceil_div(q->pg.ce_nre, 256), (unsigned)planes), dim3(256), 0, 0, (const cf32*)q->d_ce, q->d_ce_full, q->pg.ce_nre,
                     q->pg.grid_len / q->pg.ce_nre);
  return hipDeviceSynchronize() == hipSuccess ? q->d_ce_full : nullptr;
}

extern "C" int srslte_hip_dl_rx_parity_compact(const srslte_hip_dl_rx_t* q) { return q ? q->cw[0].sch.last_compact : 0; }

extern "C" uint32_t srslte_hip_rm_parity_compact_limit(uint32_t K)
{
  RmParityCompact c;
  return lte_cb_index(K) >= 0 && lte_qpp_table[lte_cb_index(K)].K == K && rm_parity_compact(K, c) ? c.e_lim : 0;
}

extern "C" const void* srslte_hip_dl_rx_debug_buffer(const srslte_hip_dl_rx_t* q, int which)
{
  if (!q) return nullptr;
  const int c = which >= 100 ? 1 : 0;
  which -= 100 * c;
  if (c && (q->ncw < 2 || which < 3 || which > 10)) return nullptr;
  srslte_hip_dl_rx_t*         m = const_cast<srslte_hip_dl_rx_t*>(q);
  srslte_hip_dl_rx::Codeword& w = m->cw[c];
  switch (which) {
    case 0: return q->d_grid;
    case 1: return q->pg.ce_nre ? dl_rx_ce_full(m) : q->d_ce;
    case 2: return q->d_res;
    case 3: return w.d_d;
    case 4: return w.d_e;
    case 5:
      if (hipDeviceSynchronize() != hipSuccess || w.sch.w_whole(0) || hipDeviceSynchronize() != hipSuccess) return nullptr;
      return w.sch.d_w;
    case 6: return w.sch.d_cb_iters;
    case 7: return w.sch.d_cb_ok;
    case 8: return w.sch.d_cb_bytes;
    case 9: return w.d_csi;
    case 10: return w.d_csi_max;
    case 11: return q->gs ? q->gs->d_e : nullptr;
    case 12: return q->gs ? q->gs->d_w : nullptr;
    case 13: return q->gs ? q->gs->d_cb_iters : nullptr;
    case 14: return q->gs ? q->gs->d_cb_ok : nullptr;
    case 15: return q->gs ? q->gs->d_relist : nullptr;
    case 16: return q->gs ? q->gs->d_scr : nullptr;
    case 17: return q->gs ? q->gs->d_csi : nullptr;
  }
  return nullptr;
}

template <typename LLR>
static void dl_rx_demod_launch(srslte_hip_dl_rx_t* q, const PdschGeom& g, const cf32* grid, uint32_t nof_sf, hipStream_t st)
{
  const cf32*        ce  = q->d_ce;
  const ChestResDev* res = q->d_res;
  const uint32_t*    scr = q->cw[0].d_scr;
  cf32*              d   = q->cw[0].d_d;
  LLR*               e   = reinterpret_cast<LLR*>(q->cw[0].d_e.get());
  if (g.tx_scheme) {
    hipLaunchKernelGGL(pdsch_demod_mimo_kernel<LLR>, dim3(ceil_div(g.max_re, 256), nof_sf), dim3(256), 0, st, grid, ce, res, scr, d, q->cw[1].d_d.get(), e,
                       reinterpret_cast<LLR*>(q->cw[1].d_e.get()), g);
  } else if (g.nof_ports == 4) {
    hipLaunchKernelGGL(pdsch_demod_div4_kernel<LLR>, dim3(ceil_div(g.max_re, 1024), nof_sf), dim3(256), 0, st, grid, ce, scr, d, e, g);
  } else if (g.nof_ports == 2) {
    hipLaunchKernelGGL(pdsch_demod_div_kernel<LLR>, dim3(ceil_div(g.max_re, 512), nof_sf), dim3(256), 0, st, grid, ce, scr, d, e, g);
  } else {
    hipLaunchKernelGGL(pdsch_demod_kernel<LLR>, dim3(ceil_div(g.max_re, 256), nof_sf), dim3(256), 0, st, grid, ce, res, scr, d, e, g);
  }
}

static int dl_rx_stage(srslte_hip_dl_rx_t* q, int stage, const void* d_iq, uint32_t tti0, uint32_t nof_sf, uint8_t* d_tb, uint32_t tb_stride, uint8_t* d_tb_ok,
                       void* stream, const DlRxCall& call)
{
  if (!q || nof_sf > q->cfg.max_batch) return SRSLTE_ERROR_INVALID_INPUTS;
  if (nof_sf == 0) return SRSLTE_SUCCESS;
  hipStream_t st   = (hipStream_t)stream;
  const cf32* grid = call.grid ? call.grid : q->d_grid;
  if (q->cfg.tdd && stage >= 2) {
    hip_log("[srslte_hip] dl_rx: a TDD cell is received through the per-subframe-grant entry points (srslte_hip_dl_rx_batch_grants*)\n");
    return SRSLTE_ERROR;
  }
  uint8_t* const tb[2] = {d_tb, d_tb ? d_tb + (size_t)nof_sf * tb_stride : nullptr};
  uint8_t* const tb_ok[2] = {d_tb_ok, d_tb_ok ? d_tb_ok + nof_sf : nullptr};
  switch (stage) {
    case 0: return srslte_hip_ofdm_rx_sf_batch(q->ofdm, d_iq, q->d_grid, (int)nof_sf * q->pg.nof_rx, stream);
    case 1: {
      q->est_nof_sf = 0;
      int r;
      if (q->cfg.mbsfn) {
        srslte_hip_chest_dl_cfg_t mc = q->cfg.chest_cfg;
        mc.mbsfn_area_id             = (uint16_t)q->cfg.mbsfn_area_id;
        r = chest_dl_estimate_mbsfn_rows(q->chest, &mc, tti0, grid, q->d_ce, (int)nof_sf, q->pg.nof_rx, 6, q->d_res, stream);
      } else {
        r = chest_dl_estimate_batch_rows(q->chest, &q->cfg.chest_cfg, tti0, grid, q->d_ce, q->d_res, (int)nof_sf, q->pg.nof_rx, q->pg.ce_nre != 0, stream);
      }
      if (r == SRSLTE_SUCCESS) q->est_nof_sf = nof_sf;
      return r;
    }
    case 2: {
      PdschGeom g = q->pg;
      g.tti0      = (int)tti0;
      if (g.csi_max) HIP_TRY(hipMemsetAsync(g.csi_max, 0, sizeof(uint32_t) * nof_sf, st));
      if (g.tx_scheme && g.csi_max1) HIP_TRY(hipMemsetAsync(g.csi_max1, 0, sizeof(uint32_t) * nof_sf, st));
      if (q->cfg.llr_8bit) dl_rx_demod_launch<int8_t>(q, g, grid, nof_sf, st);
      else dl_rx_demod_launch<int16_t>(q, g, grid, nof_sf, st);
      LAUNCH_CHECK();
      return SRSLTE_SUCCESS;
    }
    case 3:
    case 4:
    case 5:
      for (int c = 0; c < q->ncw && stage == 5; c++) {
        if (!d_tb || !d_tb_ok || tb_stride < q->cw[c].sch.cfg.tbs / 8 + 6) return SRSLTE_ERROR_INVALID_INPUTS;
      }
      for (int c = q->ncw - 1; c >= 0; c--) {
        SchRxFixed& s = q->cw[c].sch;
        const int   r = stage == 3 ? s.dematch(q->cw[c].d_e, tti0, nof_sf, call.harq[c], st)
                                   : (stage == 4 ? s.decode(nof_sf, call.harq[c], tb[c], tb_stride, tb_ok[c], st) : s.assemble(nof_sf, tb[c], tb_stride, tb_ok[c], st));
        if (r) return r;
      }
      return SRSLTE_SUCCESS;
  }
  return SRSLTE_ERROR_INVALID_INPUTS;
}

extern "C" int srslte_hip_dl_rx_stage(srslte_hip_dl_rx_t* q, int stage, const void* d_iq, uint32_t tti0, uint32_t nof_sf, uint8_t* d_tb,
                                      uint32_t tb_stride, uint8_t* d_tb_ok, void* stream)
{
  return dl_rx_stage(q, stage, d_iq, tti0, nof_sf, d_tb, tb_stride, d_tb_ok, stream, DlRxCall());
}

extern "C" int srslte_hip_dl_rx_batch(srslte_hip_dl_rx_t* q, const void* d_iq, uint32_t tti0, uint32_t nof_sf, uint8_t* d_tb,
                                      uint32_t tb_stride, uint8_t* d_tb_ok, void* stream)
{
  return srslte_hip_dl_rx_batch_harq(q, d_iq, tti0, nof_sf, 0, 1, d_tb, tb_stride, d_tb_ok, stream);
}

extern "C" int srslte_hip_dl_rx_batch_harq(srslte_hip_dl_rx_t* q, const void* d_iq, uint32_t tti0, uint32_t nof_sf, uint32_t rv, int new_data,
                                           uint8_t* d_tb, uint32_t tb_stride, uint8_t* d_tb_ok, void* stream)
{
  if (!q || !d_iq || !d_tb || !d_tb_ok || rv > 3) return SRSLTE_ERROR_INVALID_INPUTS;
  const uint32_t rv2[2] = {rv, rv};
  const int      nd2[2] = {new_data, new_data};
  return srslte_hip_dl_rx_batch_harq2(q, d_iq, tti0, nof_sf, rv2, nd2, d_tb, tb_stride, d_tb_ok, stream);
}

extern "C" int srslte_hip_dl_rx_batch_harq2(srslte_hip_dl_rx_t* q, const void* d_iq, uint32_t tti0, uint32_t nof_sf, const uint32_t rv[2],
                                            const int new_data[2], uint8_t* d_tb, uint32_t tb_stride, uint8_t* d_tb_ok, void* stream)
{
  if (!q || !d_iq || !d_tb || !d_tb_ok || !rv || !new_data || rv[0] > 3 || rv[1] > 3) return SRSLTE_ERROR_INVALID_INPUTS;
  DlRxCall call;
  for (int c = 0; c < q->ncw; c++) {
    call.harq[c] = {rv[c], new_data[c] ? 0 : 1};
    if (int r = q->cw[c].sch.ensure_rv(rv[c])) return r;
  }
  int r = SRSLTE_SUCCESS;
  for (int s = 0; s < 6 && !r; s++) r = dl_rx_stage(q, s, d_iq, tti0, nof_sf, d_tb, tb_stride, d_tb_ok, stream, call);
  return r;
}

extern "C" int srslte_hip_dl_rx_csi_batch(srslte_hip_dl_rx_t* q, uint32_t nof_sf, srslte_hip_csi_res_t* d_out, void* stream)
{
  if (!q || !d_out || nof_sf == 0 || q->est_nof_sf == 0 || nof_sf > q->est_nof_sf) return SRSLTE_ERROR_INVALID_INPUTS;
  if (!q->csi) {
    q->csi = srslte_hip_csi_create(q->cfg.nof_prb, (uint32_t)q->pg.nof_ports, (uint32_t)q->pg.nof_rx, (q->cfg.cp_ext || q->cfg.mbsfn) ? 0 : 1);
    if (!q->csi) return SRSLTE_ERROR_INVALID_INPUTS;
  }
  if (int r = srslte_hip_csi_set_snr_to_cqi_offset(q->csi, q->csi_offset)) return r;
  return srslte_hip_csi_batch(q->csi, q->d_ce, q->d_res, nof_sf, d_out, stream);
}

extern "C" int srslte_hip_dl_rx_set_snr_to_cqi_offset(srslte_hip_dl_rx_t* q, float offset)
{
  if (!q || !(offset == offset)) return SRSLTE_ERROR_INVALID_INPUTS;
  q->csi_offset = offset;
  return SRSLTE_SUCCESS;
}

extern "C" int srslte_hip_dl_rx_grid_batch(srslte_hip_dl_rx_t* q, const void* d_grid, uint32_t tti0, uint32_t nof_sf, uint8_t* d_tb,
                                           uint32_t tb_stride, uint8_t* d_tb_ok, void* stream)
{
  if (!q || !d_grid || !d_tb || !d_tb_ok) return SRSLTE_ERROR_INVALID_INPUTS;
  DlRxCall call;
  call.grid = (const cf32*)d_grid;
  int r     = SRSLTE_SUCCESS;
  for (int s = 1; s < 6 && r == SRSLTE_SUCCESS; s++) r = dl_rx_stage(q, s, nullptr, tti0, nof_sf, d_tb, tb_stride, d_tb_ok, stream, call);
  return r;
}
```

srslte-emane_amd/csrc/pdsch_rx_grants.inc:

```
static int gold_basis_upload(uint32_t words, DevBuf<uint32_t>& d_basis)
{
  const uint32_t         nbits = words * 32, Nc = 1600, tot = nbits + Nc + 31;
  std::vector<uint8_t>   x1(tot);
  std::vector<uint32_t>  x2(tot);
  for (uint32_t n = 0; n < 31; n++) {
    x1[n] = n == 0;
    x2[n] = 1u << n;
  }
  for (uint32_t n = 0; n + 31 < tot; n++) {
    x1[n + 31] = x1[n + 3] ^ x1[n];
    x2[n + 31] = x2[n + 3] ^ x2[n + 2] ^ x2[n + 1] ^ x2[n];
  }
  std::vector<uint32_t> basis((size_t)32 * words, 0);
  for (uint32_t n = 0; n < nbits; n++) {
    const uint32_t w = n >> 5, b = n & 31, v2 = x2[n + Nc];
    basis[w] |= (uint32_t)x1[n + Nc] << b;
    for (uint32_t j = 0; j < 31; j++) basis[(size_t)(1 + j) * words + w] |= ((v2 >> j) & 1u) << b;
  }
  return upload(d_basis, basis);
}

static int grants_alloc(GrantsState* g, uint32_t max_re, uint32_t V, uint32_t Cmax, uint32_t relist_rows, bool csi, size_t extra_desc_bytes)
{
  g->Cmax     = Cmax;
  g->stride   = (srslte_hip_tdec_input_len(6144, 1) + 31) & ~31u;
  g->max_re   = max_re;
  g->max_bits = (g->max_re * 8 + 15) & ~15u;
  g->words    = (g->max_re * 8 + 31) / 32 + 2;
  g->V        = V;
  {
    const char* e = getenv("SRSLTE_HIP_GRANTS_TB_DIRECT");
    g->tb_direct  = !(e && e[0] == '0');
  }
  g->tdec     = srslte_hip_tdec_create(6144, g->V * g->Cmax);
  if (!g->tdec) return SRSLTE_ERROR;
  if (gold_basis_upload(g->words, g->d_basis)) return SRSLTE_ERROR;
  const size_t nblk = (size_t)g->V * g->Cmax;
  g->desc_bytes     = sizeof(GrantDev) * g->V + sizeof(SfDesc) * g->V + sizeof(CbDesc) * nblk + sizeof(uint32_t) * nblk + extra_desc_bytes + ((g->V + 15) & ~15u);
  if (g->desc.init(g->desc_bytes + 16)) return SRSLTE_ERROR;
  if (relist_rows && g->d_relist.alloc((size_t)g->max_re * relist_rows)) return SRSLTE_ERROR;
  if (g->d_scr.alloc((size_t)g->words * g->V) || g->d_e.alloc((size_t)g->max_bits * g->V + 16) || g->d_w.alloc((size_t)g->stride * nblk) ||
      g->d_cb_bytes.alloc((size_t)768 * nblk) || g->d_cb_ok.alloc(nblk) || g->d_cb_iters.alloc(nblk))
    return SRSLTE_ERROR;
  if (csi && (g->d_csi.alloc((size_t)g->max_re * g->V) || g->d_csi_max.alloc(g->V))) return SRSLTE_ERROR;
  HIP_TRY(hipMemset(g->d_cb_ok, 0, nblk));
  HIP_TRY(hipMemset(g->d_w, 0, sizeof(int16_t) * (size_t)g->stride * nblk));
  HIP_TRY(hipMemset(g->d_cb_bytes, 0, (size_t)768 * nblk));
  HIP_TRY(hipDeviceSynchronize());
  return SRSLTE_SUCCESS;
}

struct GrantsDesc {
  GrantDev* gr;
  SfDesc*   sf;
  CbDesc*   cb;
  uint32_t* map;
  uint8_t * extra, *cof;
  GrantsDesc(const GrantsState* g, uint8_t* base)
  {
    const size_t nblk = (size_t)g->V * g->Cmax;
    gr    = reinterpret_cast<GrantDev*>(base);
    sf    = reinterpret_cast<SfDesc*>(gr + g->V);
    cb    = reinterpret_cast<CbDesc*>(sf + g->V);
    map   = reinterpret_cast<uint32_t*>(cb + nblk);
    extra = reinterpret_cast<uint8_t*>(map + nblk);
    cof   = base + g->desc_bytes - ((g->V + 15) & ~15u);
  }
};

template <typename Counts>
static const uint8_t* grants_direct_cof(const GrantsState* g, const GrantsDesc& h, const GrantsDesc& d, uint32_t n, bool l8, Counts counts)
{
  uint32_t max_C = 0;
  for (uint32_t v = 0; v < n; v++) {
    h.cof[v] = (uint8_t)h.sf[v].C;
    if (counts(v)) max_C = std::max(max_C, (uint32_t)h.sf[v].C);
  }
  return !l8 && g->tb_direct && max_C <= TDEC_TB_MAX_C_DIRECT ? d.cof : nullptr;
}

static int grants_init(srslte_hip_dl_rx_t* q)
{
  const uint32_t P = q->cfg.nof_prb, B = q->cfg.max_batch;
  q->gs.reset(new GrantsState());
  return grants_alloc(q->gs.get(), 14 * 12 * P, (q->pg.nof_ports == 2 && q->pg.nof_rx == 2) ? 2 * B : B, q->cw[0].sch.seg.C, B, q->cfg.csi_enable != 0, 0);
}

static int grants_rm_table(GrantsState* g, uint32_t K, uint32_t rv, uint32_t W, uint32_t w_len, const uint32_t** d_tbl)
{
  auto it = g->rm_tbl.find({K, rv});
  if (it == g->rm_tbl.end()) {
    DevBuf<uint32_t> d;
    if (rm_rx_table_upload(K, rv, W, w_len, d)) return SRSLTE_ERROR;
    it = g->rm_tbl.emplace(std::make_pair(K, rv), std::move(d)).first;
  }
  *d_tbl = it->second;
  return SRSLTE_SUCCESS;
}

static int grants_crc_factors(GrantsState* g, uint32_t tbs, const uint32_t** d_fac)
{
  auto it = g->crc_fac.find(tbs);
  if (it == g->crc_fac.end()) {
    const uint32_t poly = 0x1864CFBu, nbytes = tbs / 8 + 3, cB = (nbytes + 255) / 256;
    auto           mul  = [&](uint32_t a, uint32_t b) {
      uint32_t r = 0;
      for (int i = 23; i >= 0; i--) {
        r <<= 1;
        if (r & 0x1000000u) r ^= poly;
        if ((b >> i) & 1) r ^= a;
      }
      return r;
    };
    uint32_t m = 1;
    for (uint32_t i = 0; i < 8 * cB; i++) {
      m <<= 1;
      if (m & 0x1000000u) m ^= poly;
    }
    std::vector<uint32_t> w(256);
    w[255] = 1;
    for (int t = 254; t >= 0; t--) w[t] = mul(w[t + 1], m);
    DevBuf<uint32_t> d;
    if (upload(d, w)) return SRSLTE_ERROR;
    it = g->crc_fac.emplace(tbs, std::move(d)).first;
  }
  *d_fac = it->second;
  return SRSLTE_SUCCESS;
}

static void tdd_grant_symbols(int tdd, uint32_t sf_config, uint32_t ss_config, int nsl, uint32_t sf_idx, GrantDev& gd)
{
  static const int dw[10] = {3, 9, 10, 11, 12, 3, 9, 10, 11, 6};
  gd.tdd = tdd ? 1 : 0;
  gd.nss[0] = gd.nss[1] = 0;
  if (!tdd) return;
  const bool special = sf_idx == 1 || (sf_idx == 6 && (sf_config <= 2 || sf_config == 6));
  const int  n = special ? dw[ss_config % 10] : 2 * nsl;
  gd.nss[0] = n < nsl ? n : nsl;
  gd.nss[1] = n < nsl ? 0 : n - nsl;
}

static uint32_t pdsch_grant_dev(const srslte_hip_dl_grant_t& gr, uint32_t P, uint32_t cell_id, int npt, GrantDev& gd, int nsl = 7)
{
  const uint32_t sf_idx = (uint32_t)gd.sf_idx, lstart = (uint32_t)gd.lstart;
  bool any0 = false, below1 = false;
  for (uint32_t n = 0; n < P; n++) {
    for (int s_ = 0; s_ < 2; s_++) {
      if ((gr.prb_mask[s_][n >> 5] >> (n & 31)) & 1u) {
        gd.mask[s_][n >> 5] |= 1u << (n & 31);
        if (s_ == 0 && nsl - 3 >= (int)lstart) any0 = true;
        if (s_ == 1 && n + 3 < P / 2) below1 = true;
      }
    }
  }
  bool any1_whole = false;
  for (uint32_t n = 0; n < P; n++) {
    if (((gr.prb_mask[1][n >> 5] >> (n & 31)) & 1u) && !(n >= P / 2 - 3 && n < P / 2 + 3 + (P % 2))) any1_whole = true;
  }
  const int q0 = npt == 1 ? (below1 ? (int)(cell_id % 6) : (any0 ? (int)((cell_id + 3) % 6) : 0)) : ((below1 || any0) ? (int)(cell_id % 3) : 0);
  const int q1 = npt == 1 ? 0 : ((below1 || any0 || any1_whole) ? (int)(cell_id % 3) : 0);
  const int q3 = npt == 1 ? (below1 ? (int)((cell_id + 3) % 6) : (any1_whole ? (int)(cell_id % 6) : (any0 ? (int)((cell_id + 3) % 6) : 0)))
                          : ((below1 || any0 || any1_whole) ? (int)(cell_id % 3) : 0);
  gd.q_off = q0 | (q1 << 8) | (q3 << 16);
  auto pop = [](const uint32_t* m, const uint32_t* f) {
    return __builtin_popcount(m[0] & f[0]) + __builtin_popcount(m[1] & f[1]) + __builtin_popcount(m[2] & f[2]) + __builtin_popcount(m[3] & f[3]);
  };
  uint32_t centre[4] = {0, 0, 0, 0}, half[4] = {0, 0, 0, 0}, all[4] = {~0u, ~0u, ~0u, ~0u};
  for (uint32_t n = P / 2 - 3; n < P / 2 + 3 + (P % 2); n++) centre[n >> 5] |= 1u << (n & 31);
  if (P % 2) {
    half[(P / 2 - 3) >> 5] |= 1u << ((P / 2 - 3) & 31);
    half[(P / 2 + 3) >> 5] |= 1u << ((P / 2 + 3) & 31);
  }
  uint32_t nre = 0;
  const int nss[2] = {gd.nss[0] ? gd.nss[0] : nsl, gd.nss[0] ? gd.nss[1] : nsl};
  for (int sym = 0; sym < 2 * nsl; sym++) {
    const int s_ = sym / nsl, l = sym % nsl;
    if ((s_ == 0 && l < (int)lstart) || l >= nss[s_]) continue;
    const bool ref = l == 0 || l == nsl - 3 || (l == 1 && npt == 4);
    const bool ss  = gd.tdd ? ((s_ == 1 && (sf_idx == 0 || sf_idx == 5) && l >= nss[1] - 1) || (s_ == 0 && (sf_idx == 1 || sf_idx == 6) && l == 2))
                            : (s_ == 0 && (sf_idx == 0 || sf_idx == 5) && l >= nsl - 2);
    const bool sync = ss || (s_ == 1 && sf_idx == 0 && l < 4);
    const int  per = ref ? (npt == 1 ? 10 : 8) : 12;
    nre += per * pop(gd.mask[s_], all);
    if (sync) nre += (per / 2) * pop(gd.mask[s_], half) - per * pop(gd.mask[s_], centre);
  }
  return nre;
}

struct GrantsBuild {
  struct Group { uint32_t K, single; std::vector<uint32_t> slots; };
  GrantsState*       g;
  SfDesc*            h_sf;
  CbDesc*            h_cb;
  bool               l8;
  uint32_t           max_tbs;
  int                npt, max_mod;
  const char*        who;
  std::vector<Group> groups;
  uint32_t           ncb = 0, max_seg = 0;
  int add_tb(uint32_t b, uint32_t v, int mod, uint32_t tbs, uint32_t rv, int new_data, uint32_t nre, uint32_t Nl, uint32_t e_off = 0)
  {
    SfDesc& sd = h_sf[v];
    srslte_hip_cbsegm_t seg;
    if (mod < 1 || mod > max_mod || rv > 3 || tbs > max_tbs || tbs > (uint32_t)TB_MAX_BITS || (tbs % 8) || srslte_hip_cbsegm(&seg, tbs) || seg.F || seg.C2 ||
        seg.C == 0  || seg.C > g->Cmax) {
      hip_log("[srslte_hip] %s grants: entry %u: unsupported transport block (mod %d, tbs %u, rv %u)\n", who, b, mod, tbs, rv);
      return SRSLTE_ERROR_INVALID_INPUTS;
    }
    const uint32_t Qm = 2 * (uint32_t)mod, K = seg.K1, C = seg.C;
    if (nre == 0 || nre < C * Nl) {
      hip_log("[srslte_hip] %s grants: entry %u: empty allocation\n", who, b);
      return SRSLTE_ERROR_INVALID_INPUTS;
    }
    sd.nof_re = (int)nre; sd.mod = mod; sd.Qm = (int)Qm; sd.C = (int)C; sd.K = (int)K; sd.tbs = (int)tbs; sd.rlen = (int)(C == 1 ? K : K - 24);
    if (grants_crc_factors(g, tbs, &sd.crc_fac)) return SRSLTE_ERROR;
    const uint32_t W = l8 ? srslte_hip_tdec_autoimp_get_subblocks_8bit(K) : srslte_hip_tdec_autoimp_get_subblocks(K);
    const uint32_t w_len = (srslte_hip_tdec_input_len(K, W != 0) + 31) & ~31u;
    const uint32_t* tbl = nullptr;
    if (grants_rm_table(g, K, rv, W, w_len, &tbl)) return SRSLTE_ERROR;
    Group* grp = nullptr;
    for (auto& x : groups) {
      if (x.K == K && x.single == (C == 1 ? tbs : 0)) grp = &x;
    }
    if (!grp) {
      groups.push_back(Group{K, C == 1 ? tbs : 0, {}});
      grp = &groups.back();
    }
    for (uint32_t c = 0; c < C; c++) {
      CbDesc& cd = h_cb[ncb++];
      cd.sf = (int)v; cd.cb = (int)c; cd.C = (int)C; cd.K = (int)K; cd.Qm = (int)Qm; cd.nof_re = (int)nre; cd.combine = new_data ? 0 : 1;
      cd.w_len = (int)w_len; cd.tbl = tbl; cd.Nl = (int)Nl; cd.e_off = (int)e_off;
      grp->slots.push_back(v * g->Cmax + c);
    }
    const uint32_t seg_bytes = (Qm * (nre / C) + 2 * Qm * (uint32_t)npt) * (l8 ? 1 : 2) + 32;
    max_seg = seg_bytes > max_seg ? seg_bytes : max_seg;
    return SRSLTE_SUCCESS;
  }
  uint32_t fill_map(uint32_t* h_map) const
  {
    uint32_t n = 0;
    for (auto& x : groups) {
      for (uint32_t v : x.slots) h_map[n++] = v;
    }
    return n;
  }
};

static int grants_back_end(GrantsState* g, const GrantsBuild& bd, const SfDesc* d_sf, const CbDesc* d_cb, const uint32_t* d_map, uint32_t tti0,
                           uint32_t max_iterations, uint32_t nrows, uint32_t nof_rows0, uint32_t cw1_off, uint8_t* d_tb, uint32_t tb_stride,
                           uint8_t* d_tb_ok, hipStream_t st, const uint8_t* d_cof = nullptr)
{
  const bool l8 = bd.l8;
  const bool direct = d_cof != nullptr && !l8;
  if (bd.ncb) {
    RmGeom rg;
    memset(&rg, 0, sizeof(rg));
    rg.cbd = d_cb; rg.cb_ok_rst = g->d_cb_ok; rg.C = (int)g->Cmax; rg.tti0 = (int)tti0; rg.max_bits = (int)g->max_bits; rg.w_stride = (int)g->stride;
    rg.Nl = 1; rg.skip = g->d_cb_ok; rg.max_re = (int)g->max_re; rg.csi = g->d_csi; rg.csi_max = g->d_csi_max;
    const int lds = (int)((bd.max_seg + 15) & ~15u);
    if (int r = l8 ? rm_rx_launch<int8_t>(lds, bd.ncb, g->d_e, g->d_w, nullptr, rg, st) : rm_rx_launch<int16_t>(lds, bd.ncb, g->d_e, g->d_w, nullptr, rg, st))
      return r;
    TdecOpts o;
    o.skip = g->d_cb_ok;
    if (direct) {
      o.tb_out = d_tb; o.tb_out_stride = tb_stride; o.tb_ok_out = d_tb_ok;
      o.tb_Cof = d_cof; o.tb_width = g->Cmax; o.tb_B = cw1_off; o.tb_rows0 = nof_rows0;
    }
    std::vector<srslte_hip_tdec_group_t> gv;
    gv.reserve(bd.groups.size());
    for (auto& x : bd.groups) gv.push_back({x.K, (uint32_t)x.slots.size(), x.single ? 0x1864CFBu : 0x1800063u, x.single ? x.single + 24 : x.K});
    int rc = SRSLTE_SUCCESS;
    for (size_t first = 0, off = 0; first < gv.size() && rc == SRSLTE_SUCCESS;) {
      const size_t cnt = gv.size() - first < 24 ? gv.size() - first : 24;
      o.cb_map = d_map + off;
      rc = tdec_run_groups(g->tdec, g->d_w, l8 ? 1 : 0, g->stride, gv.data() + first, (uint32_t)cnt, max_iterations, g->d_cb_bytes, 768, g->d_cb_iters, g->d_cb_ok, st, o);
      for (size_t i = first; i < first + cnt; i++) off += gv[i].nof_cb;
      first += cnt;
    }
    if (rc) return rc;
  }
  if (direct || !d_tb) return SRSLTE_SUCCESS;
  TbGeom tg;
  memset(&tg, 0, sizeof(tg));
  tg.desc = d_sf; tg.C = (int)g->Cmax; tg.cb_stride = 768; tg.tb_stride = (int)tb_stride; tg.nof_sf = (int)nof_rows0; tg.cw1_off = (int)cw1_off;
  tg.iters = g->d_cb_iters;
  hipLaunchKernelGGL(tb_crc_bytes_kernel, dim3(nrows), dim3(256), 0, st, (const uint8_t*)g->d_cb_bytes, (const uint8_t*)g->d_cb_ok, d_tb, d_tb_ok, tg);
  LAUNCH_CHECK();
  return SRSLTE_SUCCESS;
}

static int grants_run(srslte_hip_dl_rx_t* q, const void* d_iq, uint32_t tti0, uint32_t nof_sf, const srslte_hip_dl_grant2_t* grants, uint8_t* d_tb,
                      uint32_t tb_stride, uint8_t* d_tb_ok, void* stream, bool second_rows, const cf32* grid_in = nullptr);

extern "C" int srslte_hip_dl_rx_batch_grants(srslte_hip_dl_rx_t* q, const void* d_iq, uint32_t tti0, uint32_t nof_sf, const srslte_hip_dl_grant_t* grants,
                                             uint8_t* d_tb, uint32_t tb_stride, uint8_t* d_tb_ok, void* stream)
{
  if (!q || !grants || nof_sf > q->cfg.max_batch) return SRSLTE_ERROR_INVALID_INPUTS;
  std::vector<srslte_hip_dl_grant2_t> g2(nof_sf);
  for (uint32_t b = 0; b < nof_sf; b++) {
    memset(&g2[b], 0, sizeof(g2[b]));
    g2[b].tb0 = grants[b];
  }
  return grants_run(q, d_iq, tti0, nof_sf, g2.data(), d_tb, tb_stride, d_tb_ok, stream, false);
}

extern "C" int srslte_hip_dl_rx_batch_grants2(srslte_hip_dl_rx_t* q, const void* d_iq, uint32_t tti0, uint32_t nof_sf, const srslte_hip_dl_grant2_t* grants,
                                              uint8_t* d_tb, uint32_t tb_stride, uint8_t* d_tb_ok, void* stream)
{
  return grants_run(q, d_iq, tti0, nof_sf, grants, d_tb, tb_stride, d_tb_ok, stream, true);
}

extern "C" int srslte_hip_dl_rx_grid_batch_grants2(srslte_hip_dl_rx_t* q, const void* d_grid, uint32_t tti0, uint32_t nof_sf, const srslte_hip_dl_grant2_t* grants,
                                                   uint8_t* d_tb, uint32_t tb_stride, uint8_t* d_tb_ok, void* stream)
{
  if (!q || !d_grid) return SRSLTE_ERROR_INVALID_INPUTS;
  return grants_run(q, d_grid, tti0, nof_sf, grants, d_tb, tb_stride, d_tb_ok, stream, true, (const cf32*)d_grid);
}

static int grants_run(srslte_hip_dl_rx_t* q, const void* d_iq, uint32_t tti0, uint32_t nof_sf, const srslte_hip_dl_grant2_t* grants, uint8_t* d_tb,
                      uint32_t tb_stride, uint8_t* d_tb_ok, void* stream, bool second_rows, const cf32* grid_in)
{
  if (!q || !d_iq || !grants || !d_tb || !d_tb_ok || nof_sf > q->cfg.max_batch || tb_stride < q->cfg.tbs / 8 + 6) return SRSLTE_ERROR_INVALID_INPUTS;
  if (q->cfg.tx_scheme) {
    hip_log("[srslte_hip] dl_rx grants mode: create the object without a fixed two-layer scheme; the grants carry it\n");
    return SRSLTE_ERROR;
  }
  if (q->cfg.mbsfn) {
    hip_log("[srslte_hip] dl_rx grants mode: an MBSFN pipeline has one PMCH configuration, no per-subframe grants\n");
    return SRSLTE_ERROR;
  }
  if (nof_sf == 0) return SRSLTE_SUCCESS;
  if (!q->gs && grants_init(q)) {
    hip_log("[srslte_hip] dl_rx grants: initialisation failed\n");
    q->gs.reset();
    return SRSLTE_ERROR;
  }
  GrantsState*   g  = q->gs.get();
  hipStream_t    st = (hipStream_t)stream;
  const uint32_t P = q->cfg.nof_prb, cell_id = q->cfg.cell_id, B = q->cfg.max_batch, V = g->V;
  const int      npt = q->pg.nof_ports;
  uint8_t*       h_pin = nullptr;
  if (int r = g->desc.begin(&h_pin)) return r;
  const GrantsDesc h(g, h_pin), d(g, g->desc.dev_bytes());
  GrantDev*        h_gr = h.gr;
  SfDesc*          h_sf = h.sf;
  const bool         l8 = q->cfg.llr_8bit != 0;
  bool               any_mimo = false;
  GrantsBuild        bd;
  bd.g = g; bd.h_sf = h_sf; bd.h_cb = h.cb; bd.l8 = l8; bd.max_tbs = q->cfg.tbs; bd.npt = npt; bd.max_mod = 4; bd.who = "dl_rx";
  auto add_tb = [&](uint32_t b, uint32_t v, int mod, uint32_t tbs, uint32_t rv, int new_data, uint32_t nre, uint32_t Nl) -> int {
    return bd.add_tb(b, v, mod, tbs, rv, new_data, nre, Nl);
  };
  for (uint32_t b = 0; b < nof_sf; b++) {
    const srslte_hip_dl_grant2_t& g2 = grants[b];
    const srslte_hip_dl_grant_t&  gr = g2.tb0;
    GrantDev&                     gd = h_gr[b];
    SfDesc&                       sd = h_sf[b];
    memset(&gd, 0, sizeof(gd));
    memset(&sd, 0, sizeof(sd));
    if (V > B) {
      memset(&h_gr[B + b], 0, sizeof(gd));
      memset(&h_sf[B + b], 0, sizeof(sd));
    }
    const uint32_t sf_idx = (tti0 + b) % 10, lstart = gr.cfi + (P < 10 ? 1 : 0);
    gd.sf_idx = (int)sf_idx; gd.lstart = (int)lstart; gd.rnti = gr.rnti;
    tdd_grant_symbols(q->cfg.tdd, q->cfg.tdd_sf_config, q->cfg.tdd_ss_config, q->cfg.cp_ext ? 6 : 7, sf_idx, gd);
    sd.idx = g->d_relist + (size_t)b * g->max_re;
    sd.scr = g->d_scr + (size_t)b * g->words;
    if (gr.tbs == 0) continue;
    const bool two_layer = g2.tx_scheme >= 2;
    if (gr.cfi < 1 || gr.cfi > 3 || g2.tx_scheme < 0 || g2.tx_scheme > 3 ||
        (two_layer && (V == B || (g2.tx_scheme == 3 && g2.tbs2 == 0) || (g2.tbs2 ? g2.pmi > 1 : g2.pmi > 3))) || (!two_layer && g2.tbs2)) {
      hip_log("[srslte_hip] dl_rx grants: subframe %u: unsupported grant (cfi %u, tx_scheme %d, pmi %u, second transport block %u bits)\n", b, gr.cfi, g2.tx_scheme,
              g2.pmi, g2.tbs2);
      return SRSLTE_ERROR_INVALID_INPUTS;
    }
    const uint32_t nre = pdsch_grant_dev(gr, P, cell_id, npt, gd, q->cfg.cp_ext ? 6 : 7);
    if (!two_layer && (nre % (uint32_t)npt)) {
      hip_log("[srslte_hip] dl_rx grants: subframe %u: %u REs are not a multiple of the %d ports\n", b, nre, npt);
      return SRSLTE_ERROR_INVALID_INPUTS;
    }
    if (int r = add_tb(b, b, gr.mod, gr.tbs, gr.rv, gr.new_data, nre, (!two_layer && npt > 1) ? 2 : 1)) return r;
    sd.scheme = g2.tx_scheme; sd.nof_tb = g2.tbs2 ? 2 : 1; sd.codebook = (int)(g2.tbs2 ? g2.pmi + 1 : g2.pmi);
    if (two_layer) any_mimo = true;
    if (g2.tbs2) {
      GrantDev& gd1 = h_gr[B + b];
      SfDesc&   sd1 = h_sf[B + b];
      gd1 = gd; gd1.cw = 1;
      sd1.idx = sd.idx;
      sd1.scr = g->d_scr + (size_t)(B + b) * g->words;
      if (int r = add_tb(b, B + b, g2.mod2, g2.tbs2, g2.rv2, g2.new_data2, nre, 1)) return r;
      sd1.scheme = g2.tx_scheme; sd1.nof_tb = 2; sd1.codebook = sd.codebook;
    }
  }
  bd.fill_map(h.map);
  const uint8_t* d_cof = grants_direct_cof(g, h, d, V, l8, [&](uint32_t v) { return v % B < nof_sf; });
  const DlRxCall call = {grid_in, {}};
  int r = grid_in ? SRSLTE_SUCCESS : dl_rx_stage(q, 0, d_iq, tti0, nof_sf, d_tb, tb_stride, d_tb_ok, stream, call);
  if (!r) r = dl_rx_stage(q, 1, d_iq, tti0, nof_sf, d_tb, tb_stride, d_tb_ok, stream, call);
  if (r) return r;
  const uint32_t nrows = (second_rows && V > B) ? 2 * nof_sf : nof_sf;
  {
    const int       per = ceil_div((int)g->words, RELIST_THREADS), work = (int)(nof_sf + (any_mimo ? 2 : 1) * nof_sf * per);
    const int       n16 = (int)((g->desc_bytes + 15) / 16);
    const GrantDev* src = h_gr;
    hipLaunchKernelGGL(grants_prep_kernel, dim3(work + ceil_div(n16, RELIST_THREADS)), dim3(RELIST_THREADS), 0, st, src, g->d_relist, (int)P,
                       (int)cell_id, (int)g->max_re, q->pg.nof_ports, q->cfg.cp_ext ? 6 : 7, (int)nof_sf, (const uint32_t*)g->d_basis, g->d_scr,
                       any_mimo ? src + B : nullptr, g->d_scr + (size_t)B * g->words, (int)g->words, d_tb_ok,
                       (int)nrows, (const uint4*)h_pin, (uint4*)g->desc.dev_bytes(), n16, work);
  }
  LAUNCH_CHECK();
  if (int r = g->desc.committed(st)) return r;
  {
    PdschGeom pg = q->pg;
    pg.desc = d.sf; pg.tti0 = (int)tti0; pg.max_re = (int)g->max_re; pg.max_bits = (int)g->max_bits; pg.csi = g->d_csi; pg.csi_max = g->d_csi_max;
    if (g->d_csi_max) HIP_TRY(hipMemsetAsync(g->d_csi_max, 0, sizeof(uint32_t) * V, st));
    const cf32* grid = grid_in ? grid_in : q->d_grid;
    if (pg.nof_ports == 4) {
      if (l8) {
        hipLaunchKernelGGL(pdsch_demod_div4_kernel<int8_t>, dim3(ceil_div((int)g->max_re, 1024), nof_sf), dim3(256), 0, st, grid, (const cf32*)q->d_ce,
                           (const uint32_t*)g->d_scr, (cf32*)nullptr, (int8_t*)g->d_e.get(), pg);
      } else {
        hipLaunchKernelGGL(pdsch_demod_div4_kernel<int16_t>, dim3(ceil_div((int)g->max_re, 1024), nof_sf), dim3(256), 0, st, grid, (const cf32*)q->d_ce,
                           (const uint32_t*)g->d_scr, (cf32*)nullptr, g->d_e, pg);
      }
    } else if (pg.nof_ports == 2) {
      if (l8) {
        hipLaunchKernelGGL(pdsch_demod_div_kernel<int8_t>, dim3(ceil_div((int)g->max_re, 512), nof_sf), dim3(256), 0, st, grid, (const cf32*)q->d_ce,
                           (const uint32_t*)g->d_scr, (cf32*)nullptr, (int8_t*)g->d_e.get(), pg);
      } else {
        hipLaunchKernelGGL(pdsch_demod_div_kernel<int16_t>, dim3(ceil_div((int)g->max_re, 512), nof_sf), dim3(256), 0, st, grid, (const cf32*)q->d_ce,
                           (const uint32_t*)g->d_scr, (cf32*)nullptr, g->d_e, pg);
      }
      if (any_mimo) {
        pg.cw1_off  = (int)B;
        pg.max_bits1 = pg.max_bits;
        pg.csi1     = g->d_csi ? g->d_csi + (size_t)B * g->max_re : nullptr;
        pg.csi_max1 = g->d_csi_max ? g->d_csi_max + B : nullptr;
        if (l8) {
          hipLaunchKernelGGL(pdsch_demod_mimo_kernel<int8_t>, dim3(ceil_div((int)g->max_re, 256), nof_sf), dim3(256), 0, st, grid, (const cf32*)q->d_ce,
                             (const ChestResDev*)q->d_res, (const uint32_t*)g->d_scr, (cf32*)nullptr, (cf32*)nullptr, (int8_t*)g->d_e.get(),
                             (int8_t*)g->d_e.get() + (size_t)B * g->max_bits, pg);
        } else {
          hipLaunchKernelGGL(pdsch_demod_mimo_kernel<int16_t>, dim3(ceil_div((int)g->max_re, 256), nof_sf), dim3(256), 0, st, grid, (const cf32*)q->d_ce,
                             (const ChestResDev*)q->d_res, (const uint32_t*)g->d_scr, (cf32*)nullptr, (cf32*)nullptr, g->d_e, g->d_e + (size_t)B * g->max_bits, pg);
        }
      }
    } else if (l8) {
      hipLaunchKernelGGL(pdsch_demod_kernel<int8_t>, dim3(ceil_div((int)g->max_re, 256), nof_sf), dim3(256), 0, st, grid, (const cf32*)q->d_ce,
                         (const ChestResDev*)q->d_res, (const uint32_t*)g->d_scr, (cf32*)nullptr, (int8_t*)g->d_e.get(), pg);
    } else {
      hipLaunchKernelGGL(pdsch_demod_kernel<int16_t>, dim3(ceil_div((int)g->max_re, 256), nof_sf), dim3(256), 0, st, grid, (const cf32*)q->d_ce,
                         (const ChestResDev*)q->d_res, (const uint32_t*)g->d_scr, (cf32*)nullptr, g->d_e, pg);
    }
    LAUNCH_CHECK();
  }
  return grants_back_end(g, bd, d.sf, d.cb, d.map, tti0, q->cfg.max_iterations, nrows, nof_sf, B, d_tb, tb_stride, d_tb_ok, st, d_cof);
}

struct srslte_hip_dl_rx_pool {
  std::vector<srslte_hip_dl_rx_t*> rx;
  std::vector<hipStream_t>         st;
  std::vector<hipEvent_t>          ev;
  std::vector<int64_t>             last;
  std::vector<DevBuf<uint8_t>>     iq;
  int64_t                          next = 0;
  ~srslte_hip_dl_rx_pool()
  {
    for (size_t i = 0; i < rx.size(); i++) {
      if (st[i]) (void)hipStreamSynchronize(st[i]);
      srslte_hip_dl_rx_destroy(rx[i]);
      if (ev[i]) (void)hipEventDestroy(ev[i]);
      if (st[i]) (void)hipStreamDestroy(st[i]);
    }
  }
};

extern "C" void srslte_hip_dl_rx_pool_destroy(srslte_hip_dl_rx_pool_t* p) { delete p; }

extern "C" srslte_hip_dl_rx_pool_t* srslte_hip_dl_rx_pool_create(const srslte_hip_dl_rx_cfg_t* cfg, uint32_t depth)
{
  if (!cfg || depth == 0 || depth > 16) return nullptr;
  std::unique_ptr<srslte_hip_dl_rx_pool> p(new srslte_hip_dl_rx_pool());
  p->rx.assign(depth, nullptr);
  p->st.assign(depth, nullptr);
  p->ev.assign(depth, nullptr);
  p->last.assign(depth, -1);
  p->iq.resize(depth);
  for (uint32_t i = 0; i < depth; i++) {
    p->rx[i] = srslte_hip_dl_rx_create(cfg);
    if (!p->rx[i] || hipStreamCreateWithFlags(&p->st[i], hipStreamNonBlocking) != hipSuccess ||
        hipEventCreateWithFlags(&p->ev[i], hipEventDisableTiming) != hipSuccess)
      return nullptr;
  }
  return p.release();
}

extern "C" int64_t srslte_hip_dl_rx_pool_submit(srslte_hip_dl_rx_pool_t* p, const void* d_iq, uint32_t tti0, uint32_t nof_sf, const srslte_hip_dl_grant_t* grants,
                                                uint8_t* d_tb, uint32_t tb_stride, uint8_t* d_tb_ok, void* h_record)
{
  if (!p || !d_iq || !d_tb || !d_tb_ok) return SRSLTE_ERROR_INVALID_INPUTS;
  const size_t i = (size_t)(p->next % (int64_t)p->rx.size());
  if (p->last[i] >= 0 && hipEventSynchronize(p->ev[i]) != hipSuccess) return SRSLTE_ERROR;
  const int r = grants ? srslte_hip_dl_rx_batch_grants(p->rx[i], d_iq, tti0, nof_sf, grants, d_tb, tb_stride, d_tb_ok, p->st[i])
                       : srslte_hip_dl_rx_batch(p->rx[i], d_iq, tti0, nof_sf, d_tb, tb_stride, d_tb_ok, p->st[i]);
  if (r) return r < 0 ? r : SRSLTE_ERROR;
  if (h_record) {
    if (hipMemcpyAsync(h_record, d_tb, (size_t)nof_sf * tb_stride, hipMemcpyDeviceToHost, p->st[i]) != hipSuccess ||
        hipMemcpyAsync((uint8_t*)h_record + (size_t)nof_sf * tb_stride, d_tb_ok, nof_sf, hipMemcpyDeviceToHost, p->st[i]) != hipSuccess)
      return SRSLTE_ERROR;
  }
  if (hipEventRecord(p->ev[i], p->st[i]) != hipSuccess) return SRSLTE_ERROR;
  p->last[i] = p->next;
  return p->next++;
}

extern "C" int srslte_hip_dl_rx_pool_set_iq_format(srslte_hip_dl_rx_pool_t* p, int format, float scale)
{
  if (!p || p->next != 0) return SRSLTE_ERROR_INVALID_INPUTS;
  for (auto* rx : p->rx)
    if (int r = srslte_hip_dl_rx_set_iq_format(rx, format, scale)) return r;
  return SRSLTE_SUCCESS;
}

extern "C" int64_t srslte_hip_dl_rx_pool_submit_host(srslte_hip_dl_rx_pool_t* p, const void* h_iq, uint32_t tti0, uint32_t nof_sf, const srslte_hip_dl_grant_t* grants,
                                                     uint8_t* d_tb, uint32_t tb_stride, uint8_t* d_tb_ok, void* h_record)
{
  if (!p || !h_iq || !d_tb || !d_tb_ok || nof_sf > p->rx[0]->cfg.max_batch) return SRSLTE_ERROR_INVALID_INPUTS;
  const size_t          i  = (size_t)(p->next % (int64_t)p->rx.size());
  srslte_hip_dl_rx_t*   rx = p->rx[i];
  const size_t          sf_bytes = ofdm_sample_bytes(rx->ofdm) * (size_t)rx->pg.nof_rx * (size_t)srslte_hip_ofdm_sf_len(rx->ofdm);
  if (!p->iq[0]) {
    for (auto& b : p->iq)
      if (b.alloc(sizeof(cf32) * (size_t)rx->pg.nof_rx * (size_t)srslte_hip_ofdm_sf_len(rx->ofdm) * rx->cfg.max_batch)) {
        for (auto& c : p->iq) c = DevBuf<uint8_t>();
        hip_log("[srslte_hip] dl_rx_pool: device allocation failed\n");
        return SRSLTE_ERROR;
      }
  }
  if (p->last[i] >= 0 && hipEventSynchronize(p->ev[i]) != hipSuccess) return SRSLTE_ERROR;
  if (nof_sf && hipMemcpyAsync(p->iq[i], h_iq, sf_bytes * nof_sf, hipMemcpyHostToDevice, p->st[i]) != hipSuccess) return SRSLTE_ERROR;
  return srslte_hip_dl_rx_pool_submit(p, p->iq[i], tti0, nof_sf, grants, d_tb, tb_stride, d_tb_ok, h_record);
}

extern "C" int srslte_hip_dl_rx_pool_wait(srslte_hip_dl_rx_pool_t* p, int64_t ticket)
{
  if (!p || ticket < 0 || ticket >= p->next) return SRSLTE_ERROR_INVALID_INPUTS;
  const size_t i = (size_t)(ticket % (int64_t)p->rx.size());
  if (p->last[i] > ticket) return SRSLTE_SUCCESS;
  return hipEventSynchronize(p->ev[i]) == hipSuccess ? SRSLTE_SUCCESS : SRSLTE_ERROR;
}
```

srslte-emane_amd/csrc/sch_fixed.inc:

```

static int fixed_grant_segmentation(const char* who, uint32_t tbs, srslte_hip_cbsegm_t* seg)
{
  if (srslte_hip_cbsegm(seg, tbs) == 0 && !seg->F && !seg->C2 && (tbs % 8) == 0) return SRSLTE_SUCCESS;
  hip_log("[srslte_hip] %s: TBS %u needs filler bits or two code-block sizes; not supported on device yet\n", who, tbs);
  return SRSLTE_ERROR;
}

struct SchHarq { uint32_t rv = 0; int combine = 0; };

struct SchRxFixed {
  struct Cfg {
    uint32_t        tbs, max_batch, max_iterations;
    bool            llr_8bit;
    uint32_t        nof_re[3], Qm, Nl, e_off, max_bits, max_re;
    int             mod;
    const float*    csi;
    const uint32_t* csi_max;
    bool            may_compact, may_direct;
  };
  Cfg                 cfg = {};
  srslte_hip_tdec_t*  tdec = nullptr;
  srslte_hip_cbsegm_t seg  = {};
  RmGeom              rg   = {};
  TbGeom              tg   = {};
  uint32_t            W = 0, in_stride = 0;
  DevBuf<uint32_t>    d_rm_tbl_rv[4];
  bool                pc_ok = false;
  RmParityCompact     pc    = {};
  DevBuf<uint32_t>    d_rm_tbl_pc;
  uint32_t            w_compact_n  = 0;
  int                 last_compact = 0;
  const uint8_t*      direct_tb = nullptr;
  const uint8_t*      direct_ok = nullptr;
  uint32_t            direct_stride = 0, direct_nof_sf = 0;
  DevBuf<int16_t>     d_w;
  DevBuf<uint8_t>     d_cb_bytes, d_cb_ok;
  DevBuf<uint32_t>    d_cb_iters, d_tbcrc;
  DevBuf<uint32_t>    d_tb_rem, d_cb_syn;
  ~SchRxFixed() { srslte_hip_tdec_destroy(tdec); }

  int init(const Cfg& c)
  {
    cfg = c;
    if (srslte_hip_cbsegm(&seg, c.tbs)) return SRSLTE_ERROR;
    const uint32_t B = c.max_batch, C = seg.C, K = seg.K1;
    if (!(tdec = srslte_hip_tdec_create(K, B * C))) return SRSLTE_ERROR;
    W         = c.llr_8bit ? srslte_hip_tdec_autoimp_get_subblocks_8bit(K) : srslte_hip_tdec_autoimp_get_subblocks(K);
    in_stride = (srslte_hip_tdec_input_len(K, W != 0) + 31) & ~31u;
    if (rm_rx_table_upload(K, 0, W, in_stride, d_rm_tbl_rv[0])) return SRSLTE_ERROR;
    std::vector<uint32_t> rem, t;
    lte_tbcrc_rem_table(c.tbs, rem);
    if (upload(d_tbcrc, rem)) return SRSLTE_ERROR;
    if (W) {
      lte_tbcrc_win_table(rem, C, K, W, t);
      if (upload(d_tb_rem, t) || d_cb_syn.alloc((size_t)B * C)) return SRSLTE_ERROR;
    }
    if (d_w.alloc((size_t)in_stride * B * C) || d_cb_bytes.alloc((size_t)(K / 8) * B * C) || d_cb_ok.alloc((size_t)B * C) || d_cb_iters.alloc((size_t)B * C))
      return SRSLTE_ERROR;
    HIP_TRY(hipMemset(d_cb_ok, 0, (size_t)B * C));
    HIP_TRY(hipMemset(d_w, 0, sizeof(int16_t) * (size_t)in_stride * B * C));
    HIP_TRY(hipMemset(d_cb_bytes, 0, (size_t)(K / 8) * B * C));
    HIP_TRY(hipDeviceSynchronize());
    rg.csi = c.csi; rg.csi_max = c.csi_max; rg.max_re = (int)c.max_re; rg.mod = c.mod; rg.Nl = (int)c.Nl; rg.e_off = (int)c.e_off;
    rg.C = (int)C; rg.K = (int)K; rg.Qm = (int)c.Qm; rg.max_bits = (int)c.max_bits; rg.w_stride = (int)in_stride; rg.out_len = (int)(3 * K + 12);
    for (int i = 0; i < 3; i++) rg.nof_re[i] = (int)c.nof_re[i];
    tg.C = (int)C; tg.K = (int)K; tg.tbs = (int)c.tbs; tg.rlen = (int)(C == 1 ? K : K - 24); tg.cb_stride = (int)(K / 8);
    if (c.may_compact && !c.llr_8bit && W == 16 && K % 64 == 0 && ((reinterpret_cast<uintptr_t>(d_w.get()) | (in_stride * sizeof(int16_t))) & 15) == 0) {
      const char*     e = getenv("SRSLTE_HIP_PARITY_COMPACT");
      RmParityCompact lim;
      if (!(e && atoi(e) == 0) && rm_parity_compact(K, lim)) {
        uint32_t mx = 0;
        for (int i = 0; i < 3; i++) {
          const uint32_t Gp = c.nof_re[i] / c.Nl, n_e = c.Qm * c.Nl * (Gp / C) + (Gp % C > 1 ? c.Qm * c.Nl : 0);
          mx = n_e > mx ? n_e : mx;
        }
        if (mx <= lim.e_lim) {
          if (rm_rx_table_upload_compact(K, pc, d_rm_tbl_pc)) return SRSLTE_ERROR;
          pc_ok = true;
        }
      }
    }
    return SRSLTE_SUCCESS;
  }

  int w_whole(hipStream_t st)
  {
    if (!w_compact_n) return SRSLTE_SUCCESS;
    hipLaunchKernelGGL(rm_parity_expand_kernel, dim3(w_compact_n * seg.C), dim3(256), 0, st, d_w.get(), (int)in_stride, (int)seg.K1, (int)pc.phase[0],
                       (int)pc.phase[1]);
    LAUNCH_CHECK();
    w_compact_n = 0;
    return SRSLTE_SUCCESS;
  }

  int ensure_rv(uint32_t rv) { return d_rm_tbl_rv[rv] ? SRSLTE_SUCCESS : rm_rx_table_upload(seg.K1, rv, W, in_stride, d_rm_tbl_rv[rv]); }

  int dematch(const void* d_e, uint32_t tti0, uint32_t nof_sf, SchHarq h, hipStream_t st)
  {
    RmGeom g  = rg;
    g.tti0    = (int)tti0;
    g.combine = h.combine;
    g.skip    = h.combine ? d_cb_ok : nullptr;
    const uint32_t* tbl = d_rm_tbl_rv[h.rv];
    last_compact = pc_ok && h.rv == 0 && !h.combine;
    if (last_compact) {
      tbl         = d_rm_tbl_pc;
      g.w_len     = (int)pc.len;
      w_compact_n = nof_sf > w_compact_n ? nof_sf : w_compact_n;
    } else if (h.combine || nof_sf < w_compact_n) {
      if (int r = w_whole(st)) return r;
    } else {
      w_compact_n = 0;
    }
    if (cfg.llr_8bit) return rm_rx_launch<int8_t>(rm_lds_bytes(g, 1), nof_sf * seg.C, d_e, d_w, tbl, g, st);
    return rm_rx_launch<int16_t>(rm_lds_bytes(g, 2), nof_sf * seg.C, d_e, d_w, tbl, g, st);
  }

  int decode(uint32_t nof_sf, SchHarq h, uint8_t* d_tb, uint32_t tb_stride, uint8_t* d_tb_ok, hipStream_t st)
  {
    const uint32_t C = seg.C, K = seg.K1;
    TdecOpts       o;
    o.tb_rem = d_tb_rem; o.tb_C = C; o.tb_syn = d_cb_syn;
    o.skip   = h.combine ? d_cb_ok.get() : nullptr;
    if (w_compact_n && w_compact_n < nof_sf) {
      if (int r = w_whole(st)) return r;
    }
    if (w_compact_n) {
      o.pc = 1; o.pc_phase[0] = pc.phase[0]; o.pc_phase[1] = pc.phase[1];
    }
    direct_tb = nullptr;
    if (cfg.may_direct && d_tb_rem && (cfg.llr_8bit ? W >= 16 : W == 16) && !h.combine && d_tb && d_tb_ok && tb_stride >= cfg.tbs / 8 + 6) {
      o.tb_out = d_tb; o.tb_out_stride = tb_stride; o.tb_rb = tg.rlen / 8; o.tb_ok_out = d_tb_ok;
      direct_tb = d_tb; direct_ok = d_tb_ok; direct_stride = tb_stride; direct_nof_sf = nof_sf;
    }
    return tdec_run_batch_w(tdec, d_w, cfg.llr_8bit ? 1 : 0, in_stride, W != 0, K, -1, nof_sf * C, cfg.max_iterations, C > 1 ? 0x1800063u : 0x1864CFBu,
                            C > 1 ? K : cfg.tbs + 24, d_cb_bytes, K / 8, d_cb_iters, d_cb_ok, st, o);
  }

  int assemble(uint32_t nof_sf, uint8_t* d_tb, uint32_t tb_stride, uint8_t* d_tb_ok, hipStream_t st)
  {
    if (direct_tb && direct_tb == d_tb && direct_ok == d_tb_ok && direct_stride == tb_stride && direct_nof_sf == nof_sf) return SRSLTE_SUCCESS;
    TbGeom g    = tg;
    g.tb_stride = (int)tb_stride;
    g.iters     = d_cb_iters;
    if (d_tb_rem) {
      hipLaunchKernelGGL(tb_asm_kernel, dim3(nof_sf), dim3(256), 0, st, (const uint8_t*)d_cb_bytes, (const uint8_t*)d_cb_ok, (const uint32_t*)d_cb_syn, d_tb,
                         d_tb_ok, g);
    } else {
      hipLaunchKernelGGL(tb_crc_kernel, dim3(nof_sf), dim3(512), 0, st, (const uint8_t*)d_cb_bytes, (const uint8_t*)d_cb_ok, (const uint32_t*)d_tbcrc, d_tb,
                         d_tb_ok, g);
    }
    LAUNCH_CHECK();
    return SRSLTE_SUCCESS;
  }
};
```

srslte-emane_amd/pipelines.py:

```python
import ctypes as C

import numpy as np

from ._native import (IQ_CF32, IQ_SC16, SRSLTE_SUCCESS, DevBuf, DevView, Handle, P, _check, cint, f32, host_copy, i64, lib, read_structs,
                      result_structs, struct_array, symbol_sz, sync, u32, void, vp)
from .core import ChestDlCfg, DmrsPuschCfg
from .csi import CsiRes
from .dl_ctrl import _ctrl_tx_in
from .ul_ctrl import SRS_MAX_CE, PucchReq, PucchRes, Srs, SrsRes, SrsUe


class DlRxCfg(C.Structure):
    C_TYPE = "srslte_hip_dl_rx_cfg_t"
    _fields_ = [("cell_id", C.c_uint32), ("nof_prb", C.c_uint32), ("cfi", C.c_uint32), ("rnti", C.c_uint16), ("mod", C.c_int),
                ("tbs", C.c_uint32), ("max_iterations", C.c_uint32), ("max_batch", C.c_uint32), ("mmse", C.c_int), ("chest_cfg", ChestDlCfg),
                ("llr_8bit", C.c_int), ("nof_rx_antennas", C.c_uint32), ("nof_ports", C.c_uint32), ("csi_enable", C.c_int), ("power_scale", C.c_int), ("p_a", C.c_float),
                ("tx_scheme", C.c_int), ("pmi", C.c_uint32), ("mod2", C.c_int), ("tbs2", C.c_uint32), ("cp_ext", C.c_int),
                ("tdd", C.c_int), ("tdd_sf_config", C.c_uint32), ("tdd_ss_config", C.c_uint32),
                ("mbsfn", C.c_int), ("mbsfn_area_id", C.c_uint32), ("non_mbsfn_region", C.c_uint32)]


class DlGrant(C.Structure):
    C_TYPE = "srslte_hip_dl_grant_t"
    _fields_ = [("prb_mask", (C.c_uint32 * 4) * 2), ("mod", C.c_int), ("tbs", C.c_uint32), ("rv", C.c_uint32), ("cfi", C.c_uint32), ("rnti", C.c_uint16),
                ("new_data", C.c_int)]

    @classmethod
    def make(cls, nof_prb, mod, tbs, rnti, cfi=1, rv=0, new_data=True, prb_mask=None):
        g = cls()
        g.mod, g.tbs, g.rv, g.cfi, g.rnti, g.new_data = mod, tbs, rv, cfi, rnti, 1 if new_data else 0
        for s in range(2):
            for n in range(nof_prb):
                if prb_mask is None or prb_mask[s][n]:
                    g.prb_mask[s][n >> 5] |= 1 << (n & 31)
        return g


class DlGrant2(C.Structure):
    C_TYPE = "srslte_hip_dl_grant2_t"
    _fields_ = [("tb0", DlGrant), ("tx_scheme", C.c_int), ("pmi", C.c_uint32), ("mod2", C.c_int), ("tbs2", C.c_uint32), ("rv2", C.c_uint32), ("new_data2", C.c_int)]


class UlRxCfg(C.Structure):
    C_TYPE = "srslte_hip_ul_rx_cfg_t"
    _fields_ = [("cell_id", C.c_uint32), ("nof_prb", C.c_uint32), ("rnti", C.c_uint16), ("mod", C.c_int), ("tbs", C.c_uint32), ("L_prb", C.c_uint32),
                ("n_prb", C.c_uint32), ("n_dmrs", C.c_uint32), ("max_iterations", C.c_uint32), ("max_batch", C.c_uint32), ("mmse", C.c_int),
                ("dmrs_cfg", DmrsPuschCfg), ("shortened", C.c_int), ("ack_len", C.c_uint32), ("I_offset_ack", C.c_uint32),
                ("ri_len", C.c_uint32), ("I_offset_ri", C.c_uint32), ("cqi_len", C.c_uint32), ("I_offset_cqi", C.c_uint32),
                ("hopping", C.c_uint32), ("n_prb_slot1", C.c_uint32), ("max_grants", C.c_uint32), ("cp_ext", C.c_int)]


class UlGrant(C.Structure):
    C_TYPE = "srslte_hip_ul_grant_t"
    _fields_ = [("sf", C.c_uint32), ("rnti", C.c_uint16), ("L_prb", C.c_uint32), ("n_prb", C.c_uint32), ("n_prb_slot1", C.c_uint32), ("n_dmrs", C.c_uint32),
                ("mod", C.c_int), ("tbs", C.c_uint32), ("rv", C.c_uint32), ("new_data", C.c_int), ("ack_len", C.c_uint32), ("I_offset_ack", C.c_uint32),
                ("ri_len", C.c_uint32), ("I_offset_ri", C.c_uint32), ("cqi_len", C.c_uint32), ("I_offset_cqi", C.c_uint32)]

    @classmethod
    def make(cls, sf, rnti, L_prb, n_prb, mod, tbs, n_dmrs=0, n_prb_slot1=None, rv=0, new_data=True, ack_len=0, I_offset_ack=0, ri_len=0, I_offset_ri=0,
             cqi_len=0, I_offset_cqi=0):
        return cls(sf, rnti, L_prb, n_prb, n_prb if n_prb_slot1 is None else n_prb_slot1, n_dmrs, mod, tbs, rv, 1 if new_data else 0, ack_len, I_offset_ack,
                   ri_len, I_offset_ri, cqi_len, I_offset_cqi)


class UlTxCfg(C.Structure):
    C_TYPE = "srslte_hip_ul_tx_cfg_t"
    _fields_ = [("cell_id", C.c_uint32), ("nof_prb", C.c_uint32), ("rnti", C.c_uint16), ("mod", C.c_int), ("tbs", C.c_uint32), ("L_prb", C.c_uint32),
                ("n_prb", C.c_uint32), ("n_dmrs", C.c_uint32), ("max_batch", C.c_uint32), ("dmrs_cfg", DmrsPuschCfg), ("shortened", C.c_int),
                ("ack_len", C.c_uint32), ("I_offset_ack", C.c_uint32), ("ri_len", C.c_uint32), ("I_offset_ri", C.c_uint32),
                ("cqi_len", C.c_uint32), ("I_offset_cqi", C.c_uint32), ("hopping", C.c_uint32), ("n_prb_slot1", C.c_uint32), ("max_grants", C.c_uint32),
                ("cp_ext", C.c_int)]


class DlTxCfg(C.Structure):
    C_TYPE = "srslte_hip_dl_tx_cfg_t"
    _fields_ = [("cell_id", C.c_uint32), ("nof_prb", C.c_uint32), ("cfi", C.c_uint32), ("rnti", C.c_uint16), ("mod", C.c_int), ("tbs", C.c_uint32),
                ("max_batch", C.c_uint32), ("nof_ports", C.c_uint32), ("p_a", C.c_float), ("max_grants", C.c_uint32), ("cp_ext", C.c_int),
                ("tdd", C.c_int), ("tdd_sf_config", C.c_uint32), ("tdd_ss_config", C.c_uint32),
                ("mbsfn", C.c_int), ("mbsfn_area_id", C.c_uint32), ("non_mbsfn_region", C.c_uint32)]


class DlTxGrant(C.Structure):
    C_TYPE = "srslte_hip_dl_tx_grant_t"
    _fields_ = [("sf", C.c_uint32), ("grant", DlGrant)]


class DlTxGrant2(C.Structure):
    C_TYPE = "srslte_hip_dl_tx_grant2_t"
    _fields_ = [("sf", C.c_uint32), ("grant", DlGrant2)]


_RX_BATCH = [vp, vp, u32, u32, vp, u32, vp, vp]
_RX_HARQ = [vp, vp, u32, u32, u32, cint, vp, u32, vp, vp]
_DL_RX_GRANTS = [vp, vp, u32, u32, vp, vp, u32, vp, vp]
_DL_TX_GRANTS = [vp, vp, u32, u32, u32, vp, u32, vp, vp]

SIGNATURES = {
    "srslte_hip_dl_rx_create": (vp, [P(DlRxCfg)]),
    "srslte_hip_dl_rx_destroy": (void, [vp]),
    "srslte_hip_dl_rx_set_iq_format": (None, [vp, cint, f32]),
    "srslte_hip_dl_rx_nof_re": (u32, [vp, u32]),
    "srslte_hip_dl_rx_batch": (None, _RX_BATCH),
    "srslte_hip_dl_rx_batch_harq": (None, _RX_HARQ),
    "srslte_hip_dl_rx_batch_harq2": (None, [vp, vp, u32, u32, vp, vp, vp, u32, vp, vp]),
    "srslte_hip_dl_rx_grid_batch": (None, _RX_BATCH),
    "srslte_hip_dl_rx_batch_grants": (None, _DL_RX_GRANTS),
    "srslte_hip_dl_rx_batch_grants2": (None, _DL_RX_GRANTS),
    "srslte_hip_dl_rx_grid_batch_grants2": (None, _DL_RX_GRANTS),
    "srslte_hip_dl_rx_pool_create": (vp, [vp, u32]),
    "srslte_hip_dl_rx_pool_destroy": (void, [vp]),
    "srslte_hip_dl_rx_pool_submit": (i64, [vp, vp, u32, u32, vp, vp, u32, vp, vp]),
    "srslte_hip_dl_rx_pool_wait": (None, [vp, i64]),
    "srslte_hip_dl_rx_pool_set_iq_format": (None, [vp, cint, f32]),
    "srslte_hip_dl_rx_pool_submit_host": (i64, [vp, vp, u32, u32, vp, vp, u32, vp, vp]),
    "srslte_hip_dl_rx_stage": (None, [vp, cint, vp, u32, u32, vp, u32, vp, vp]),
    "srslte_hip_dl_rx_debug_buffer": (vp, [vp, cint]),
    "srslte_hip_dl_rx_keep_symbols": (None, [vp, cint]),
    "srslte_hip_dl_rx_parity_compact": (None, [vp]),
    "srslte_hip_rm_parity_compact_limit": (u32, [u32]),
    "srslte_hip_ul_rx_create": (vp, [P(UlRxCfg)]),
    "srslte_hip_ul_rx_destroy": (void, [vp]),
    "srslte_hip_ul_rx_set_iq_format": (None, [vp, cint, f32]),
    "srslte_hip_ul_rx_batch": (None, _RX_BATCH),
    "srslte_hip_ul_rx_batch_harq": (None, _RX_HARQ),
    "srslte_hip_ul_rx_batch_grants": (None, [vp, vp, u32, u32, vp, u32, vp, u32, vp, vp]),
    "srslte_hip_ul_rx_grants_ack": (vp, [vp]),
    "srslte_hip_ul_rx_grants_ri": (vp, [vp]),
    "srslte_hip_ul_rx_grants_cqi": (vp, [vp]),
    "srslte_hip_ul_rx_ack": (vp, [vp]),
    "srslte_hip_ul_rx_ri": (vp, [vp]),
    "srslte_hip_ul_rx_cqi": (vp, [vp]),
    "srslte_hip_ul_rx_debug_buffer": (vp, [vp, cint]),
    "srslte_hip_ul_tx_create": (vp, [P(UlTxCfg)]),
    "srslte_hip_ul_tx_destroy": (void, [vp]),
    "srslte_hip_ul_tx_set_iq_format": (None, [vp, cint, f32]),
    "srslte_hip_ul_tx_batch": (None, [vp, vp, u32, u32, u32, vp, vp]),
    "srslte_hip_ul_tx_batch_ack": (None, [vp, vp, u32, vp, u32, u32, vp, vp]),
    "srslte_hip_ul_tx_batch_uci": (None, [vp, vp, u32, vp, vp, u32, u32, vp, vp]),
    "srslte_hip_ul_tx_batch_uci_cqi": (None, [vp, vp, u32, vp, vp, vp, u32, u32, vp, vp]),
    "srslte_hip_ul_tx_batch_rv": (None, [vp, vp, u32, vp, vp, vp, u32, u32, u32, vp, vp]),
    "srslte_hip_ul_tx_batch_grants": (None, [vp, vp, u32, vp, vp, vp, u32, u32, vp, u32, vp, vp]),
    "srslte_hip_ul_tx_debug_buffer": (vp, [vp, cint]),
    "srslte_hip_dl_tx_create": (vp, [P(DlTxCfg)]),
    "srslte_hip_dl_tx_destroy": (void, [vp]),
    "srslte_hip_dl_tx_set_iq_format": (None, [vp, cint, f32]),
    "srslte_hip_dl_tx_batch": (None, [vp, vp, u32, u32, u32, u32, vp, vp]),
    "srslte_hip_dl_tx_batch_grants": (None, _DL_TX_GRANTS),
    "srslte_hip_dl_tx_batch_grants2": (None, _DL_TX_GRANTS),
    "srslte_hip_dl_tx_debug_buffer": (vp, [vp, cint]),
}


class Pipeline(Handle):

    DEBUG = IQ_FORMAT = None
    iq_format = IQ_CF32

    def debug(self, which, dtype, count):
        return host_copy(getattr(lib(), self.DEBUG)(self.h, which), dtype, count)

    def set_iq_format(self, fmt, scale=1.0):
        rc = getattr(lib(), self.IQ_FORMAT)(self.h, fmt, scale)
        if rc == SRSLTE_SUCCESS:
            self.iq_format = fmt
        return rc

    def _iq_in(self, iq, width):
        if self.iq_format == IQ_SC16:
            return np.ascontiguousarray(iq, np.int16).reshape(-1, 2 * width)
        return np.ascontiguousarray(iq, np.complex64).reshape(-1, width)

    def _iq_out(self, *shape):
        if self.iq_format == IQ_SC16:
            return self.d_iq.to_host(np.int16, 2 * int(np.prod(shape))).reshape(shape + (2,))
        return self.d_iq.to_host(np.complex64).reshape(shape)


def _tb_rows(d_tb, d_ok, stride, n, nbytes=None):
    return d_tb.to_host(np.uint8).reshape(-1, stride)[:n, :nbytes], d_ok.to_host(np.uint8)[:n]


def _tb_rows2(d_tb, d_ok, stride, n, nbytes=(None, None)):
    tb, ok = _tb_rows(d_tb, d_ok, stride, 2 * n)
    return [tb[:n, :nbytes[0]], tb[n:, :nbytes[1]]], [ok[:n], ok[n:]]


class DlRx(Pipeline):
    DESTROY, DEBUG, IQ_FORMAT = "srslte_hip_dl_rx_destroy", "srslte_hip_dl_rx_debug_buffer", "srslte_hip_dl_rx_set_iq_format"

    def __init__(self, cell_id, nof_prb, cfi, rnti, mod, tbs, max_iterations, max_batch, mmse=True, chest_cfg=None, llr_8bit=False, nof_rx=1,
                 nof_ports=1, csi=False, power_scale=False, p_a=0.0, out_ptrs=None, tx_scheme=0, pmi=0, mod2=0, tbs2=0, cp_ext=False, tdd=None,
                 mbsfn=None):
        self.cfg = DlRxCfg(cell_id, nof_prb, cfi, rnti, mod, tbs, max_iterations, max_batch, 1 if mmse else 0, chest_cfg or ChestDlCfg(),
                           1 if llr_8bit else 0, nof_rx, nof_ports, 1 if csi else 0, 1 if power_scale else 0, p_a, tx_scheme, pmi, mod2, tbs2, 1 if cp_ext else 0,
                           1 if tdd else 0, tdd[0] if tdd else 0, tdd[1] if tdd else 0, 1 if mbsfn else 0, mbsfn[0] if mbsfn else 0, mbsfn[1] if mbsfn else 0)
        self.nof_rx = nof_rx
        self._create("srslte_hip_dl_rx_create", C.byref(self.cfg))
        self.tbs, self.max_batch, self.tbs2 = tbs, max_batch, tbs2
        self.tb_stride = (max(tbs, tbs2) // 8 + 6 + 15) & ~15
        self.sf_len = 15 * symbol_sz(nof_prb)
        if out_ptrs is None:
            self.d_tb, self.d_ok = DevBuf(self.tb_stride * max_batch * (2 if tbs2 else 1)), DevBuf(max_batch * (2 if tbs2 else 1))
        else:
            self.d_tb, self.d_ok = DevView(out_ptrs[0], self.tb_stride * max_batch), DevView(out_ptrs[1], max_batch)
        self.e_stride = (max(self.nof_re(s) for s in (0, 1, 5)) * {1: 2, 2: 4, 3: 6, 4: 8}[mod] + 15) & ~15

    def nof_re(self, sf_idx):
        return lib().srslte_hip_dl_rx_nof_re(self.h, sf_idx)

    def keep_symbols(self, enable=True):
        _check(lib().srslte_hip_dl_rx_keep_symbols(self.h, 1 if enable else 0), "dl_rx_keep_symbols")

    def parity_compact(self):
        return bool(lib().srslte_hip_dl_rx_parity_compact(self.h))

    def run_device(self, d_iq_ptr, tti0, nof_sf, stream=None):
        return lib().srslte_hip_dl_rx_batch(self.h, d_iq_ptr, tti0, nof_sf, self.d_tb.ptr, self.tb_stride, self.d_ok.ptr, stream)

    def stage(self, stage, d_iq_ptr, tti0, nof_sf, stream=None):
        return lib().srslte_hip_dl_rx_stage(self.h, stage, d_iq_ptr, tti0, nof_sf, self.d_tb.ptr, self.tb_stride, self.d_ok.ptr, stream)

    def _rows(self, n):
        return _tb_rows(self.d_tb, self.d_ok, self.tb_stride, n, self.tbs // 8 + 3)

    def _rows2(self, n):
        return _tb_rows2(self.d_tb, self.d_ok, self.tb_stride, n, (self.tbs // 8 + 3, self.tbs2 // 8 + 3))

    def decode(self, iq, tti0=0):
        x = self._iq_in(iq, self.nof_rx * self.sf_len)
        din = DevBuf.from_host(x)
        _check(self.run_device(din.ptr, tti0, x.shape[0]), "dl_rx_batch")
        sync()
        return self._rows2(x.shape[0]) if self.tbs2 else self._rows(x.shape[0])

    def decode_harq2(self, iq, tti0, rv, new_data):
        x = self._iq_in(iq, self.nof_rx * self.sf_len)
        din = DevBuf.from_host(x)
        n = x.shape[0]
        _check(lib().srslte_hip_dl_rx_batch_harq2(self.h, din.ptr, tti0, n, (C.c_uint32 * 2)(*rv), (C.c_int * 2)(*[1 if v else 0 for v in new_data]),
                                                  self.d_tb.ptr, self.tb_stride, self.d_ok.ptr, None), "dl_rx_batch_harq2")
        sync()
        return self._rows2(n)

    def decode_grants(self, iq, tti0, grants):
        x = self._iq_in(iq, self.nof_rx * self.sf_len)
        assert len(grants) == x.shape[0]
        arr = (DlGrant * len(grants))(*grants)
        din = DevBuf.from_host(x)
        rc = lib().srslte_hip_dl_rx_batch_grants(self.h, din.ptr, tti0, x.shape[0], arr, self.d_tb.ptr, self.tb_stride, self.d_ok.ptr, None)
        if rc != SRSLTE_SUCCESS:
            return rc, None, None
        sync()
        return (rc,) + self._rows(x.shape[0])

    def decode_grants2(self, iq, tti0, grants, from_grid=False):
        if from_grid:
            x = np.ascontiguousarray(iq, np.complex64).reshape(-1, self.nof_rx * 14 * 12 * self.cfg.nof_prb)
        else:
            x = self._iq_in(iq, self.nof_rx * self.sf_len)
        n = x.shape[0]
        assert len(grants) == n
        arr = (DlGrant2 * n)(*grants)
        din, dtb, dok = DevBuf.from_host(x), DevBuf(self.tb_stride * n * 2), DevBuf(2 * n)
        fn = lib().srslte_hip_dl_rx_grid_batch_grants2 if from_grid else lib().srslte_hip_dl_rx_batch_grants2
        rc = fn(self.h, din.ptr, tti0, n, arr, dtb.ptr, self.tb_stride, dok.ptr, None)
        if rc != SRSLTE_SUCCESS:
            return rc, None, None
        sync()
        tb, ok = _tb_rows2(dtb, dok, self.tb_stride, n)
        if not (self.cfg.nof_ports == 2 and self.cfg.nof_rx_antennas == 2):
            tb[1] = ok[1] = None
        return rc, tb, ok

    def decode_harq(self, iq, tti0, rv, new_data):
        x = self._iq_in(iq, self.nof_rx * self.sf_len)
        din = DevBuf.from_host(x)
        _check(lib().srslte_hip_dl_rx_batch_harq(self.h, din.ptr, tti0, x.shape[0], rv, 1 if new_data else 0, self.d_tb.ptr, self.tb_stride,
                                                 self.d_ok.ptr, None), "dl_rx_batch_harq")
        sync()
        return self._rows(x.shape[0])

    def decode_grid(self, grid, tti0=0):
        x = np.ascontiguousarray(grid, np.complex64)
        x = x.reshape(-1, x.shape[-1])
        din = DevBuf.from_host(x)
        _check(lib().srslte_hip_dl_rx_grid_batch(self.h, din.ptr, tti0, x.shape[0], self.d_tb.ptr, self.tb_stride, self.d_ok.ptr, None), "dl_rx_grid_batch")
        sync()
        return self._rows(x.shape[0])

    def csi(self, nof_sf, snr_to_cqi_offset=None):
        if snr_to_cqi_offset is not None:
            _check(lib().srslte_hip_dl_rx_set_snr_to_cqi_offset(self.h, snr_to_cqi_offset), "dl_rx_set_snr_to_cqi_offset")
        dout = DevBuf(max(1, nof_sf) * C.sizeof(CsiRes))
        return result_structs(lib().srslte_hip_dl_rx_csi_batch(self.h, nof_sf, dout.ptr, None), dout.ptr, CsiRes, nof_sf)


class DlRxPool(Handle):
    DESTROY = "srslte_hip_dl_rx_pool_destroy"

    def __init__(self, cfg, depth):
        self._create("srslte_hip_dl_rx_pool_create", C.byref(cfg), depth)

    def set_iq_format(self, fmt, scale=1.0):
        return lib().srslte_hip_dl_rx_pool_set_iq_format(self.h, fmt, scale)

    def submit(self, d_iq, tti0, nof_sf, d_tb, tb_stride, d_tb_ok, grants=None, h_record=None):
        arr = (DlGrant * len(grants))(*grants) if grants else None
        return lib().srslte_hip_dl_rx_pool_submit(self.h, d_iq, tti0, nof_sf, arr, d_tb, tb_stride, d_tb_ok, h_record)

    def submit_host(self, h_iq, tti0, nof_sf, d_tb, tb_stride, d_tb_ok, grants=None, h_record=None):
        arr = (DlGrant * len(grants))(*grants) if grants else None
        return lib().srslte_hip_dl_rx_pool_submit_host(self.h, h_iq, tti0, nof_sf, arr, d_tb, tb_stride, d_tb_ok, h_record)

    def wait(self, ticket):
        return lib().srslte_hip_dl_rx_pool_wait(self.h, ticket)


class UlRx(Pipeline):
    DESTROY, DEBUG, IQ_FORMAT = "srslte_hip_ul_rx_destroy", "srslte_hip_ul_rx_debug_buffer", "srslte_hip_ul_rx_set_iq_format"

    def __init__(self, cell_id, nof_prb, rnti, mod, tbs, L_prb, n_prb, n_dmrs, max_iterations, max_batch, cyclic_shift=0, delta_ss=0,
                 group_hopping=False, sequence_hopping=False, mmse=True, shortened=False, ack_len=0, I_offset_ack=0, ri_len=0, I_offset_ri=0,
                 cqi_len=0, I_offset_cqi=0, n_prb_slot1=None, max_grants=0, cp_ext=False):
        self.cfg = UlRxCfg(cell_id, nof_prb, rnti, mod, tbs, L_prb, n_prb, n_dmrs, max_iterations, max_batch, 1 if mmse else 0,
                           DmrsPuschCfg(cyclic_shift, delta_ss, 1 if group_hopping else 0, 1 if sequence_hopping else 0), 1 if shortened else 0,
                           ack_len, I_offset_ack, ri_len, I_offset_ri, cqi_len, I_offset_cqi, 0 if n_prb_slot1 is None else 1, n_prb_slot1 or 0,
                           max_grants, 1 if cp_ext else 0)
        self._create("srslte_hip_ul_rx_create", C.byref(self.cfg))
        self.tbs, self.max_batch = tbs, max_batch
        self.tb_stride = (tbs // 8 + 6 + 15) & ~15
        self.sf_len = 15 * symbol_sz(nof_prb)
        self.rows = max(max_batch, max_grants)
        self.rows_grants = max_grants or max_batch
        self.d_tb, self.d_ok = DevBuf(self.tb_stride * self.rows), DevBuf(self.rows)

    def _rows(self, n, nbytes=None):
        return _tb_rows(self.d_tb, self.d_ok, self.tb_stride, n, nbytes)

    def decode_grants(self, iq, tti0, grants):
        x = self._iq_in(iq, self.sf_len)
        din = DevBuf.from_host(x)
        arr = (UlGrant * len(grants))(*grants)
        _check(lib().srslte_hip_ul_rx_batch_grants(self.h, din.ptr, tti0, x.shape[0], arr, len(grants), self.d_tb.ptr, self.tb_stride, self.d_ok.ptr, None),
               "ul_rx_batch_grants")
        sync()
        self.last_nof_grants = len(grants)
        return self._rows(len(grants))

    def decode_grants_pucch(self, iq, tti0, grants, ctrl, reqs):
        x = self._iq_in(iq, self.sf_len)
        din = DevBuf.from_host(x)
        dres = DevBuf(C.sizeof(PucchRes) * max(1, len(reqs)))
        rc = lib().srslte_hip_ul_rx_batch_grants_pucch(self.h, din.ptr, tti0, x.shape[0], struct_array(UlGrant, grants), len(grants), self.d_tb.ptr,
                                                       self.tb_stride, self.d_ok.ptr, ctrl.h, struct_array(PucchReq, reqs), len(reqs), dres.ptr, None)
        if rc != SRSLTE_SUCCESS:
            return rc, None, None, None
        sync()
        self.last_nof_grants = len(grants)
        return (rc,) + self._rows(len(grants)) + (read_structs(dres.ptr, PucchRes, len(reqs)),)

    def decode_grants_pucch_srs(self, iq, tti0, grants, ctrl, reqs, srs, ues):
        x = self._iq_in(iq, self.sf_len)
        din = DevBuf.from_host(x)
        dres = DevBuf(C.sizeof(PucchRes) * max(1, len(reqs)))
        dsr, dsc = DevBuf(C.sizeof(SrsRes) * max(1, len(ues))), DevBuf(8 * SRS_MAX_CE * max(1, len(ues)))
        rc = lib().srslte_hip_ul_rx_batch_grants_pucch_srs(self.h, din.ptr, tti0, x.shape[0], struct_array(UlGrant, grants), len(grants), self.d_tb.ptr,
                                                           self.tb_stride, self.d_ok.ptr, ctrl.h if ctrl is not None else None,
                                                           struct_array(PucchReq, reqs), len(reqs), dres.ptr, srs.h if srs is not None else None,
# ... 192 lines not shown
```

Measured before the change: 563,300.

## Add lean PDSCH demod kernel (4 REs/thread) and single-wrap rate-match specialization

Adds a specialized single-port PDSCH demod kernel that processes four REs per thread, with modulation and MRC as template parameters. It packs the LLRs in registers and writes them with wide vector stores, without the LDS staging pass. It also adds a ONE_WRAP variant of the LDS rate-dematch kernel that replaces the circular accumulation loop with a single clamped load when the encoded length never wraps the circular buffer. Both paths are on by default and can be turned off through an env var. The risk is more template instantiations and edge-case handling for tail REs and unaligned index tables.

Result: no change. 567,400 (median of 2 runs) (+0.7%).

```diff
diff --git a/include/srslte_hip/phy_hip.h b/include/srslte_hip/phy_hip.h
--- a/include/srslte_hip/phy_hip.h
+++ b/include/srslte_hip/phy_hip.h
@@ -203,6 +203,7 @@
 const void* srslte_hip_dl_rx_debug_buffer(const srslte_hip_dl_rx_t* q, int which);
 int         srslte_hip_dl_rx_keep_symbols(srslte_hip_dl_rx_t* q, int enable);
 int      srslte_hip_dl_rx_parity_compact(const srslte_hip_dl_rx_t* q);
+int      srslte_hip_dl_rx_lean_kernels(const srslte_hip_dl_rx_t* q);
 uint32_t srslte_hip_rm_parity_compact_limit(uint32_t K);
 
 typedef struct srslte_hip_ul_rx srslte_hip_ul_rx_t;
diff --git a/srslte-emane_amd/csrc/pdsch_kernels.inc b/srslte-emane_amd/csrc/pdsch_kernels.inc
--- a/srslte-emane_amd/csrc/pdsch_kernels.inc
+++ b/srslte-emane_amd/csrc/pdsch_kernels.inc
@@ -130,6 +130,135 @@
   if ((int)threadIdx.x < rem) dst[nbytes - rem + threadIdx.x] = src[nbytes - rem + threadIdx.x];
 }
 
+template <typename LLR, int MOD, bool MRC>
+__global__ __launch_bounds__(256) void pdsch_demod_kernel_re4(const cf32* __restrict__ grid, const cf32* __restrict__ ce,
+                                                              const ChestResDev* __restrict__ res, const uint32_t* __restrict__ scr,
+                                                              LLR* __restrict__ e_out, PdschGeom g)
+{
+  constexpr int   Qm = 2 * MOD, BITS = 8 * (int)sizeof(LLR), NW = 4 * Qm * BITS / 32;
+  const int       sf = blockIdx.y, sf_idx = (g.tti0 + sf) % 10;
+  SfClass         c  = g.cls[sf_class(sf_idx)];
+  const uint32_t* cs = scr + (size_t)sf_idx * g.scr_words;
+  if (g.desc) {
+    const SfDesc d = g.desc[sf];
+    c.idx = d.idx; c.nof_re = d.nof_re; cs = d.scr;
+  }
+  const int i0 = 4 * (blockIdx.x * blockDim.x + threadIdx.x);
+  if (i0 >= c.nof_re) return;
+  const bool whole = i0 + 4 <= c.nof_re;
+  uint32_t   k[4], kh[4];
+  if (whole && (reinterpret_cast<uintptr_t>(c.idx) & 15) == 0) {
+    const uint4 t = *reinterpret_cast<const uint4*>(c.idx + i0);
+    k[0] = t.x; k[1] = t.y; k[2] = t.z; k[3] = t.w;
+  } else {
+#pragma unroll
+    for (int t = 0; t < 4; t++) k[t] = c.idx[min(i0 + t, c.nof_re - 1)];
+  }
+#pragma unroll
+  for (int t = 0; t < 4; t++) {
+    kh[t] = 8u * (g.ce_nre ? k[t] - __umulhi(k[t], g.ce_magic) * (uint32_t)g.ce_nre : k[t]);
+    k[t] *= 8u;
+  }
+  auto at = [](const cf32* base, uint32_t off) { return *reinterpret_cast<const cf32*>(reinterpret_cast<const char*>(base) + off); };
+  const float n0 = g.mmse ? res[sf].noise_estimate : 0.f;
+  cf32        x[4];
+  const cf32* yb = grid + (size_t)sf * g.nof_rx * g.grid_len;
+  const cf32* hb = ce + (size_t)sf * g.nof_rx * g.ce_len;
+  float       re[4], im[4], hh[4];
+  {
+    cf32 y[4], h[4];
+#pragma unroll
+    for (int t = 0; t < 4; t++) {
+      y[t] = at(yb, k[t]);
+      h[t] = at(hb, kh[t]);
+    }
+#pragma unroll
+    for (int t = 0; t < 4; t++) {
+      re[t] = y[t].x * h[t].x + y[t].y * h[t].y;
+      im[t] = y[t].y * h[t].x - y[t].x * h[t].y;
+      hh[t] = h[t].x * h[t].x + h[t].y * h[t].y;
+    }
+  }
+  if constexpr (!MRC) {
+#pragma unroll
+    for (int t = 0; t < 4; t++) {
+      const float csi = hh[t] + n0;
+      x[t] = make_float2(re[t] * g.inv_scaling / csi, im[t] * g.inv_scaling / csi);
+    }
+  } else {
+#pragma unroll 1
+    for (int a = 1; a < g.nof_rx; a++) {
+      cf32 y[4], h[4];
+#pragma unroll
+      for (int t = 0; t < 4; t++) {
+        k[t] += 8u * (uint32_t)g.grid_len;
+        kh[t] += 8u * (uint32_t)g.ce_len;
+        y[t] = at(yb, k[t]);
+        h[t] = at(hb, kh[t]);
+      }
+#pragma unroll
+      for (int t = 0; t < 4; t++) {
+        re[t] += y[t].x * h[t].x + y[t].y * h[t].y;
+        im[t] += y[t].y * h[t].x - y[t].x * h[t].y;
+        hh[t] += h[t].x * h[t].x + h[t].y * h[t].y;
+      }
+    }
+#pragma unroll
+    for (int t = 0; t < 4; t++) {
+      if (n0 > 0.f) hh[t] += n0;
+      x[t] = make_float2(re[t] / hh[t] * g.inv_scaling, im[t] / hh[t] * g.inv_scaling);
+    }
+  }
+  const int      bit0 = i0 * Qm;
+  const uint32_t c2   = (uint32_t)((((uint64_t)cs[(bit0 >> 5) + 1] << 32) | cs[bit0 >> 5]) >> (bit0 & 31));
+  LLR*           row  = e_out + (size_t)sf * g.max_bits;
+  const int lim = MOD == demod_dev::MOD_256QAM ? c.nof_re : ((sizeof(LLR) == 1 || MOD == demod_dev::MOD_QPSK) ? 8 * (c.nof_re / 8) : 4 * (c.nof_re / 4));
+  if (whole && i0 + 4 <= lim) {
+    uint32_t w[NW];
+#pragma unroll
+    for (int n = 0; n < NW; n++) w[n] = 0;
+#pragma unroll
+    for (int t = 0; t < 4; t++) {
+      LLR o[8];
+      if constexpr (sizeof(LLR) == 1) {
+        demod_dev::demod_b(MOD, x[t], 0, 8, o);
+      } else {
+        demod_dev::demod_s(MOD, x[t], 0, 8, o);
+      }
+#pragma unroll
+      for (int j = 0; j < Qm; j++) {
+        const int s = t * Qm + j;
+        LLR       v = o[j];
+        if ((c2 >> s) & 1) v = (LLR)-v;
+        w[s * BITS / 32] |= ((uint32_t)v & ((1u << BITS) - 1u)) << ((s * BITS) & 31);
+      }
+    }
+    if constexpr (sizeof(LLR) == 1) {
+      uint2* dst = reinterpret_cast<uint2*>(row + (size_t)i0 * Qm);
+#pragma unroll
+      for (int n = 0; n < NW / 2; n++) dst[n] = make_uint2(w[2 * n], w[2 * n + 1]);
+    } else {
+      uint4* dst = reinterpret_cast<uint4*>(row + (size_t)i0 * Qm);
+#pragma unroll
+      for (int n = 0; n < NW / 4; n++) dst[n] = make_uint4(w[4 * n], w[4 * n + 1], w[4 * n + 2], w[4 * n + 3]);
+    }
+  } else {
+#pragma unroll
+    for (int t = 0; t < 4; t++) {
+      const int i = i0 + t;
+      if (i >= c.nof_re) break;
+      LLR o[8];
+      if constexpr (sizeof(LLR) == 1) {
+        demod_dev::demod_b(MOD, x[t], i, c.nof_re, o);
+      } else {
+        demod_dev::demod_s(MOD, x[t], i, c.nof_re, o);
+      }
+#pragma unroll
+      for (int j = 0; j < Qm; j++) row[(size_t)i * Qm + j] = ((c2 >> (t * Qm + j)) & 1) ? (LLR)-o[j] : o[j];
+    }
+  }
+}
+
 template <typename LLR>
 __global__ __launch_bounds__(256) void pdsch_demod_div_kernel(const cf32* __restrict__ grid, const cf32* __restrict__ ce,
                                                               const uint32_t* __restrict__ scr, cf32* __restrict__ d_out, LLR* __restrict__ e_out,
@@ -489,7 +618,7 @@
   *dst          = combine ? add_wrap<LLR>(*dst, word) : word;
 }
 
-template <typename LLR>
+template <typename LLR, bool ONE_WRAP = false>
 __global__ __launch_bounds__(256) void rm_rx_lds_kernel(const LLR* __restrict__ e, LLR* __restrict__ w, const uint32_t* __restrict__ inv, RmGeom g)
 {
   extern __shared__ __attribute__((aligned(16))) char seg_raw[];
@@ -554,7 +683,10 @@
       for (int s = 0; s < PER; s++) {
         const uint32_t pair = (&tt[u][s / 8].x)[(s / 2) & 3], n = (s & 1) ? pair >> 16 : pair & 0xffffu;
         int            acc  = 0;
-        if (n != 0xffffu) {
+        if constexpr (ONE_WRAP) {
+          const int v = ls[min(n, (uint32_t)(n_e2 - 1))];
+          acc         = n < (uint32_t)n_e2 ? v : 0;
+        } else if (n != 0xffffu) {
           for (int i = (int)n; i < n_e2; i += out_len) acc += ls[i];
         }
         constexpr int BITS = 8 * (int)sizeof(LLR);
@@ -907,10 +1039,47 @@
   return ((g.Qm * (mx / g.C) + 2 * g.Qm) * llr_bytes + 32 + 15) & ~15;
 }
 
+enum { LEAN_DEMOD = 1, LEAN_RM = 2 };
+int pdsch_lean_env()
+{
+  const char* e = getenv("SRSLTE_HIP_PDSCH_LEAN");
+  return e ? atoi(e) & (LEAN_DEMOD | LEAN_RM) : (LEAN_DEMOD | LEAN_RM);
+}
+
+template <typename LLR>
+bool pdsch_demod_re4_launch(int mod, const PdschGeom& g, const cf32* grid, const cf32* ce, const ChestResDev* res, const uint32_t* scr, LLR* e,
+                            uint32_t nof_sf, hipStream_t st)
+{
+  if (g.tx_scheme || g.nof_ports != 1 || g.csi) return false;
+  const dim3 grd(ceil_div(g.max_re, 1024), nof_sf), blk(256);
+  const bool mrc = g.nof_rx > 1;
+#define RE4(M)                                                                                                                   \
+  case M:                                                                                                                        \
+    if (mrc) hipLaunchKernelGGL((pdsch_demod_kernel_re4<LLR, M, true>), grd, blk, 0, st, grid, ce, res, scr, e, g);              \
+    else hipLaunchKernelGGL((pdsch_demod_kernel_re4<LLR, M, false>), grd, blk, 0, st, grid, ce, res, scr, e, g);                 \
+    return true;
+  switch (mod) {
+    RE4(1)
+    RE4(2)
+    RE4(3)
+    RE4(4)
+  }
+#undef RE4
+  return false;
+}
+
+bool rm_one_wrap(uint32_t nre, uint32_t Qm, uint32_t Nl, uint32_t C, uint32_t K)
+{
+  const uint32_t Gp = nre / Nl, n_e2 = Qm * Nl * (Gp / C) + (Gp % C > 1 ? Qm * Nl : 0);
+  return n_e2 <= 3 * K + 12;
+}
+
 template <typename T>
-int rm_rx_launch(int lds, uint32_t nblk, const void* e, void* w, const uint32_t* tbl, const RmGeom& g, hipStream_t st)
-{
-  if (lds <= 64 * 1024) {
+int rm_rx_launch(int lds, uint32_t nblk, const void* e, void* w, const uint32_t* tbl, const RmGeom& g, hipStream_t st, bool one_wrap = false)
+{
+  if (lds <= 64 * 1024 && one_wrap) {
+    hipLaunchKernelGGL((rm_rx_lds_kernel<T, true>), dim3(nblk), dim3(256), lds, st, (const T*)e, (T*)w, tbl, g);
+  } else if (lds <= 64 * 1024) {
     hipLaunchKernelGGL(rm_rx_lds_kernel<T>, dim3(nblk), dim3(256), lds, st, (const T*)e, (T*)w, tbl, g);
   } else {
     hipLaunchKernelGGL(rm_rx_kernel<T>, dim3(ceil_div(g.w_stride, 1024 / (int)sizeof(T)), nblk), dim3(256), 0, st, (const T*)e, (T*)w, tbl, g);
diff --git a/srslte-emane_amd/csrc/pdsch_rx.inc b/srslte-emane_amd/csrc/pdsch_rx.inc
--- a/srslte-emane_amd/csrc/pdsch_rx.inc
+++ b/srslte-emane_amd/csrc/pdsch_rx.inc
@@ -9,6 +9,8 @@
   DevBuf<uint32_t>   d_csi_max;
   size_t             desc_bytes = 0;
   DescStage          desc;
+  int                lean = 0;
+  int                last_one_wrap = 0;
   bool               tb_direct = false;
   std::map<std::pair<uint32_t, uint32_t>, DevBuf<uint32_t>> rm_tbl;
   std::map<uint32_t, DevBuf<uint32_t>>                      crc_fac;
@@ -37,6 +39,8 @@
   srslte_hip_csi_t*      csi = nullptr;
   uint32_t               est_nof_sf = 0;
   float                  csi_offset = 0.f;
+  int                    lean = 0;
+  int                    last_lean = 0;
   ~srslte_hip_dl_rx()
   {
     srslte_hip_ofdm_destroy(ofdm);
@@ -75,8 +79,9 @@
     }
   }
   std::unique_ptr<srslte_hip_dl_rx> q(new srslte_hip_dl_rx());
-  q->cfg = *cfg;
-  q->ncw = two ? 2 : 1;
+  q->cfg  = *cfg;
+  q->ncw  = two ? 2 : 1;
+  q->lean = pdsch_lean_env();
   srslte_hip_cbsegm_t seg;
   if (fixed_grant_segmentation("dl_rx", cfg->tbs, &seg) || (two && fixed_grant_segmentation("dl_rx", cfg->tbs2, &seg))) return nullptr;
   const uint32_t P = cfg->nof_prb, nre = 12 * P, B = cfg->max_batch;
@@ -199,6 +204,8 @@
 }
 
 extern "C" int srslte_hip_dl_rx_parity_compact(const srslte_hip_dl_rx_t* q) { return q ? q->cw[0].sch.last_compact : 0; }
+
+extern "C" int srslte_hip_dl_rx_lean_kernels(const srslte_hip_dl_rx_t* q) { return q ? q->last_lean : 0; }
 
 extern "C" uint32_t srslte_hip_rm_parity_compact_limit(uint32_t K)
 {
@@ -254,6 +261,8 @@
     hipLaunchKernelGGL(pdsch_demod_div4_kernel<LLR>, dim3(ceil_div(g.max_re, 1024), nof_sf), dim3(256), 0, st, grid, ce, scr, d, e, g);
   } else if (g.nof_ports == 2) {
     hipLaunchKernelGGL(pdsch_demod_div_kernel<LLR>, dim3(ceil_div(g.max_re, 512), nof_sf), dim3(256), 0, st, grid, ce, scr, d, e, g);
+  } else if ((q->lean & LEAN_DEMOD) && !d && pdsch_demod_re4_launch<LLR>(g.mod, g, grid, ce, res, scr, e, nof_sf, st)) {
+    q->last_lean |= LEAN_DEMOD;
   } else {
     hipLaunchKernelGGL(pdsch_demod_kernel<LLR>, dim3(ceil_div(g.max_re, 256), nof_sf), dim3(256), 0, st, grid, ce, res, scr, d, e, g);
   }
@@ -292,6 +301,7 @@
       g.tti0      = (int)tti0;
       if (g.csi_max) HIP_TRY(hipMemsetAsync(g.csi_max, 0, sizeof(uint32_t) * nof_sf, st));
       if (g.tx_scheme && g.csi_max1) HIP_TRY(hipMemsetAsync(g.csi_max1, 0, sizeof(uint32_t) * nof_sf, st));
+      q->last_lean &= ~LEAN_DEMOD;
       if (q->cfg.llr_8bit) dl_rx_demod_launch<int8_t>(q, g, grid, nof_sf, st);
       else dl_rx_demod_launch<int16_t>(q, g, grid, nof_sf, st);
       LAUNCH_CHECK();
@@ -309,6 +319,7 @@
                                    : (stage == 4 ? s.decode(nof_sf, call.harq[c], tb[c], tb_stride, tb_ok[c], st) : s.assemble(nof_sf, tb[c], tb_stride, tb_ok[c], st));
         if (r) return r;
       }
+      if (stage == 3) q->last_lean = (q->last_lean & ~LEAN_RM) | (q->cw[0].sch.last_one_wrap ? LEAN_RM : 0);
       return SRSLTE_SUCCESS;
   }
   return SRSLTE_ERROR_INVALID_INPUTS;
diff --git a/srslte-emane_amd/csrc/pdsch_rx_grants.inc b/srslte-emane_amd/csrc/pdsch_rx_grants.inc
--- a/srslte-emane_amd/csrc/pdsch_rx_grants.inc
+++ b/srslte-emane_amd/csrc/pdsch_rx_grants.inc
@@ -32,6 +32,7 @@
     const char* e = getenv("SRSLTE_HIP_GRANTS_TB_DIRECT");
     g->tb_direct  = !(e && e[0] == '0');
   }
+  g->lean     = pdsch_lean_env();
   g->tdec     = srslte_hip_tdec_create(6144, g->V * g->Cmax);
   if (!g->tdec) return SRSLTE_ERROR;
   if (gold_basis_upload(g->words, g->d_basis)) return SRSLTE_ERROR;
@@ -83,7 +84,9 @@
 {
   const uint32_t P = q->cfg.nof_prb, B = q->cfg.max_batch;
   q->gs.reset(new GrantsState());
-  return grants_alloc(q->gs.get(), 14 * 12 * P, (q->pg.nof_ports == 2 && q->pg.nof_rx == 2) ? 2 * B : B, q->cw[0].sch.seg.C, B, q->cfg.csi_enable != 0, 0);
+  const int r = grants_alloc(q->gs.get(), 14 * 12 * P, (q->pg.nof_ports == 2 && q->pg.nof_rx == 2) ? 2 * B : B, q->cw[0].sch.seg.C, B, q->cfg.csi_enable != 0, 0);
+  q->gs->lean = q->lean;
+  return r;
 }
 
 static int grants_rm_table(GrantsState* g, uint32_t K, uint32_t rv, uint32_t W, uint32_t w_len, const uint32_t** d_tbl)
@@ -198,6 +201,7 @@
   const char*        who;
   std::vector<Group> groups;
   uint32_t           ncb = 0, max_seg = 0;
+  bool               one_wrap = true;
   int add_tb(uint32_t b, uint32_t v, int mod, uint32_t tbs, uint32_t rv, int new_data, uint32_t nre, uint32_t Nl, uint32_t e_off = 0)
   {
     SfDesc& sd = h_sf[v];
@@ -233,7 +237,8 @@
       grp->slots.push_back(v * g->Cmax + c);
     }
     const uint32_t seg_bytes = (Qm * (nre / C) + 2 * Qm * (uint32_t)npt) * (l8 ? 1 : 2) + 32;
-    max_seg = seg_bytes > max_seg ? seg_bytes : max_seg;
+    max_seg  = seg_bytes > max_seg ? seg_bytes : max_seg;
+    one_wrap = one_wrap && rm_one_wrap(nre, Qm, Nl, C, K);
     return SRSLTE_SUCCESS;
   }
   uint32_t fill_map(uint32_t* h_map) const
@@ -258,7 +263,9 @@
     rg.cbd = d_cb; rg.cb_ok_rst = g->d_cb_ok; rg.C = (int)g->Cmax; rg.tti0 = (int)tti0; rg.max_bits = (int)g->max_bits; rg.w_stride = (int)g->stride;
     rg.Nl = 1; rg.skip = g->d_cb_ok; rg.max_re = (int)g->max_re; rg.csi = g->d_csi; rg.csi_max = g->d_csi_max;
     const int lds = (int)((bd.max_seg + 15) & ~15u);
-    if (int r = l8 ? rm_rx_launch<int8_t>(lds, bd.ncb, g->d_e, g->d_w, nullptr, rg, st) : rm_rx_launch<int16_t>(lds, bd.ncb, g->d_e, g->d_w, nullptr, rg, st))
+    const bool ow = (g->lean & LEAN_RM) && bd.one_wrap;
+    g->last_one_wrap = ow && lds <= 64 * 1024;
+    if (int r = l8 ? rm_rx_launch<int8_t>(lds, bd.ncb, g->d_e, g->d_w, nullptr, rg, st, ow) : rm_rx_launch<int16_t>(lds, bd.ncb, g->d_e, g->d_w, nullptr, rg, st, ow))
       return r;
     TdecOpts o;
     o.skip = g->d_cb_ok;
@@ -346,6 +353,7 @@
   SfDesc*          h_sf = h.sf;
   const bool         l8 = q->cfg.llr_8bit != 0;
   bool               any_mimo = false;
+  int                one_mod  = -1;
   GrantsBuild        bd;
   bd.g = g; bd.h_sf = h_sf; bd.h_cb = h.cb; bd.l8 = l8; bd.max_tbs = q->cfg.tbs; bd.npt = npt; bd.max_mod = 4; bd.who = "dl_rx";
   auto add_tb = [&](uint32_t b, uint32_t v, int mod, uint32_t tbs, uint32_t rv, int new_data, uint32_t nre, uint32_t Nl) -> int {
@@ -383,6 +391,7 @@
     if (int r = add_tb(b, b, gr.mod, gr.tbs, gr.rv, gr.new_data, nre, (!two_layer && npt > 1) ? 2 : 1)) return r;
     sd.scheme = g2.tx_scheme; sd.nof_tb = g2.tbs2 ? 2 : 1; sd.codebook = (int)(g2.tbs2 ? g2.pmi + 1 : g2.pmi);
     if (two_layer) any_mimo = true;
+    one_mod = (two_layer || (one_mod >= 0 && one_mod != gr.mod)) ? 0 : gr.mod;
     if (g2.tbs2) {
       GrantDev& gd1 = h_gr[B + b];
       SfDesc&   sd1 = h_sf[B + b];
@@ -416,6 +425,7 @@
     pg.desc = d.sf; pg.tti0 = (int)tti0; pg.max_re = (int)g->max_re; pg.max_bits = (int)g->max_bits; pg.csi = g->d_csi; pg.csi_max = g->d_csi_max;
     if (g->d_csi_max) HIP_TRY(hipMemsetAsync(g->d_csi_max, 0, sizeof(uint32_t) * V, st));
     const cf32* grid = grid_in ? grid_in : q->d_grid;
+    q->last_lean &= ~LEAN_DEMOD;
     if (pg.nof_ports == 4) {
       if (l8) {
         hipLaunchKernelGGL(pdsch_demod_div4_kernel<int8_t>, dim3(ceil_div((int)g->max_re, 1024), nof_sf), dim3(256), 0, st, grid, (const cf32*)q->d_ce,
@@ -446,6 +456,12 @@
                              (const ChestResDev*)q->d_res, (const uint32_t*)g->d_scr, (cf32*)nullptr, (cf32*)nullptr, g->d_e, g->d_e + (size_t)B * g->max_bits, pg);
         }
       }
+    } else if ((g->lean & LEAN_DEMOD) && one_mod > 0 &&
+               (l8 ? pdsch_demod_re4_launch<int8_t>(one_mod, pg, grid, (const cf32*)q->d_ce, (const ChestResDev*)q->d_res, (const uint32_t*)g->d_scr,
+                                                  (int8_t*)g->d_e.get(), nof_sf, st)
+                   : pdsch_demod_re4_launch<int16_t>(one_mod, pg, grid, (const cf32*)q->d_ce, (const ChestResDev*)q->d_res, (const uint32_t*)g->d_scr,
+                                                   g->d_e.get(), nof_sf, st))) {
+      q->last_lean |= LEAN_DEMOD;
     } else if (l8) {
       hipLaunchKernelGGL(pdsch_demod_kernel<int8_t>, dim3(ceil_div((int)g->max_re, 256), nof_sf), dim3(256), 0, st, grid, (const cf32*)q->d_ce,
                          (const ChestResDev*)q->d_res, (const uint32_t*)g->d_scr, (cf32*)nullptr, (int8_t*)g->d_e.get(), pg);
@@ -455,7 +471,9 @@
     }
     LAUNCH_CHECK();
   }
-  return grants_back_end(g, bd, d.sf, d.cb, d.map, tti0, q->cfg.max_iterations, nrows, nof_sf, B, d_tb, tb_stride, d_tb_ok, st, d_cof);
+  const int rb = grants_back_end(g, bd, d.sf, d.cb, d.map, tti0, q->cfg.max_iterations, nrows, nof_sf, B, d_tb, tb_stride, d_tb_ok, st, d_cof);
+  q->last_lean = (q->last_lean & ~LEAN_RM) | (bd.ncb && g->last_one_wrap ? LEAN_RM : 0);
+  return rb;
 }
 
 struct srslte_hip_dl_rx_pool {
diff --git a/srslte-emane_amd/csrc/sch_fixed.inc b/srslte-emane_amd/csrc/sch_fixed.inc
--- a/srslte-emane_amd/csrc/sch_fixed.inc
+++ b/srslte-emane_amd/csrc/sch_fixed.inc
@@ -30,6 +30,8 @@
   DevBuf<uint32_t>    d_rm_tbl_pc;
   uint32_t            w_compact_n  = 0;
   int                 last_compact = 0;
+  bool                one_wrap      = false;
+  int                 last_one_wrap = 0;
   const uint8_t*      direct_tb = nullptr;
   const uint8_t*      direct_ok = nullptr;
   uint32_t            direct_stride = 0, direct_nof_sf = 0;
@@ -65,6 +67,8 @@
     rg.C = (int)C; rg.K = (int)K; rg.Qm = (int)c.Qm; rg.max_bits = (int)c.max_bits; rg.w_stride = (int)in_stride; rg.out_len = (int)(3 * K + 12);
     for (int i = 0; i < 3; i++) rg.nof_re[i] = (int)c.nof_re[i];
     tg.C = (int)C; tg.K = (int)K; tg.tbs = (int)c.tbs; tg.rlen = (int)(C == 1 ? K : K - 24); tg.cb_stride = (int)(K / 8);
+    one_wrap = (pdsch_lean_env() & LEAN_RM) != 0;
+    for (int i = 0; i < 3; i++) one_wrap = one_wrap && rm_one_wrap(c.nof_re[i], c.Qm, c.Nl, C, K);
     if (c.may_compact && !c.llr_8bit && W == 16 && K % 64 == 0 && ((reinterpret_cast<uintptr_t>(d_w.get()) | (in_stride * sizeof(int16_t))) & 15) == 0) {
       const char*     e = getenv("SRSLTE_HIP_PARITY_COMPACT");
       RmParityCompact lim;
@@ -112,8 +116,10 @@
     } else {
       w_compact_n = 0;
     }
-    if (cfg.llr_8bit) return rm_rx_launch<int8_t>(rm_lds_bytes(g, 1), nof_sf * seg.C, d_e, d_w, tbl, g, st);
-    return rm_rx_launch<int16_t>(rm_lds_bytes(g, 2), nof_sf * seg.C, d_e, d_w, tbl, g, st);
+    const int lds = rm_lds_bytes(g, cfg.llr_8bit ? 1 : 2);
+    last_one_wrap = one_wrap && lds <= 64 * 1024;
+    if (cfg.llr_8bit) return rm_rx_launch<int8_t>(lds, nof_sf * seg.C, d_e, d_w, tbl, g, st, one_wrap);
+    return rm_rx_launch<int16_t>(lds, nof_sf * seg.C, d_e, d_w, tbl, g, st, one_wrap);
   }
 
   int decode(uint32_t nof_sf, SchHarq h, uint8_t* d_tb, uint32_t tb_stride, uint8_t* d_tb_ok, hipStream_t st)
diff --git a/srslte-emane_amd/pipelines.py b/srslte-emane_amd/pipelines.py
--- a/srslte-emane_amd/pipelines.py
+++ b/srslte-emane_amd/pipelines.py
@@ -117,6 +117,7 @@
     "srslte_hip_dl_rx_debug_buffer": (vp, [vp, cint]),
     "srslte_hip_dl_rx_keep_symbols": (None, [vp, cint]),
     "srslte_hip_dl_rx_parity_compact": (None, [vp]),
+    "srslte_hip_dl_rx_lean_kernels": (None, [vp]),
     "srslte_hip_rm_parity_compact_limit": (u32, [u32]),
     "srslte_hip_ul_rx_create": (vp, [P(UlRxCfg)]),
     "srslte_hip_ul_rx_destroy": (void, [vp]),
@@ -214,6 +215,9 @@
     def parity_compact(self):
         return bool(lib().srslte_hip_dl_rx_parity_compact(self.h))
 
+    def lean_kernels(self):
+        return int(lib().srslte_hip_dl_rx_lean_kernels(self.h))
+
     def run_device(self, d_iq_ptr, tti0, nof_sf, stream=None):
         return lib().srslte_hip_dl_rx_batch(self.h, d_iq_ptr, tti0, nof_sf, self.d_tb.ptr, self.tb_stride, self.d_ok.ptr, stream)
 
```
